# SparklingH/BloomScene

Hardware: AMD Instinct MI355X
Metric: Msplats/s fwd+bwd @1M Gaussians 1920x1080 SH3; fraction of HBM roofline (higher is better)
Workload: dtype f32; 1 GPU; c3: 1000000 Gaussians, SH deg 3, 1920x1080, fwd+bwd colour+depth targets, synthetic scene A seed 0; gaussians=1000000, width=1920, height=1080, sh_degree=3, num_rendered=4386625, visible=1000000, parallelism=view-parallel x1, exact_exp=0, strict_gradients=0, prewarm_steps=282

## Files before the change

### bloomscene_amd/_capi.py

```python
from __future__ import annotations

import ctypes as C
import os
import subprocess

_HERE = os.path.dirname(os.path.abspath(__file__))
LIB_PATH = os.path.join(_HERE, "libbloomscene_rast.so")
CSRC = os.path.join(_HERE, "csrc")

ALLOC_FN = C.CFUNCTYPE(C.c_void_p, C.c_void_p, C.c_size_t)

_F = C.c_void_p
ABI_VERSION = 4
OLDER_ABI_ACCEPTED = frozenset({2, 3})


class StageProfile(C.Structure):
    _fields_ = [("name", C.c_char_p), ("total_ms", C.c_double), ("launches", C.c_int)]


SIGNATURES = {
    "bsr_version": (C.c_int, []),
    "bsr_last_error": (C.c_char_p, []),
    "bsr_mark_visible": (C.c_int, [C.c_int, _F, _F, _F, _F, C.c_void_p]),
    "bsr_forward": (C.c_int, [ALLOC_FN, C.c_void_p, ALLOC_FN, C.c_void_p, ALLOC_FN, C.c_void_p,
                              C.c_int, C.c_int, C.c_int, _F, C.c_int, C.c_int, _F, _F, _F, _F, _F, C.c_float, _F, _F,
                              _F, _F, _F, C.c_float, C.c_float, C.c_int, _F, _F, _F, C.c_int, C.c_void_p,
                              C.POINTER(C.c_int)]),
    "bsr_forward_ex": (C.c_int, [ALLOC_FN, C.c_void_p, ALLOC_FN, C.c_void_p, ALLOC_FN, C.c_void_p,
                                 C.c_int, C.c_int, C.c_int, _F, C.c_int, C.c_int, _F, _F, _F, _F, _F, C.c_float, _F, _F,
                                 _F, _F, _F, C.c_float, C.c_float, C.c_int, _F, _F, _F, C.c_int, C.c_void_p,
                                 C.POINTER(C.c_int)] + [C.c_uint]),
    "bsr_forward_views": (C.c_int, [ALLOC_FN, C.c_void_p, ALLOC_FN, C.c_void_p, ALLOC_FN, C.c_void_p,
                                    C.c_int, C.c_int, C.c_int, C.c_int, _F, C.c_int, C.c_int, _F, _F, _F, _F, _F,
                                    C.c_float, _F, _F, _F, _F, _F, C.c_float, C.c_float, C.c_int, _F, _F, _F, C.c_int,
                                    C.c_void_p, C.POINTER(C.c_int), C.c_uint]),
    "bsr_visible_filter": (C.c_int, [C.c_int, C.c_int, C.c_int, C.c_int, _F, _F, C.c_float, _F, _F, _F, _F,
                                     C.c_float, C.c_float, C.c_int, _F, C.c_int, C.c_void_p]),
    "bsr_visible_scratch_bytes": (C.c_size_t, [C.c_int]),
    "bsr_visible_filter_indices": (C.c_int, [C.c_int, C.c_int, C.c_int, C.c_int, _F, _F, C.c_float, _F, _F, _F, _F,
                                             C.c_float, C.c_float, C.c_int, _F, _F, _F, C.POINTER(C.c_int), C.c_int,
                                             C.c_void_p]),
    "bsr_visible_filter_views": (C.c_int, [C.c_int, C.c_int, C.c_int, C.c_int, _F, _F, C.c_float, _F, _F, _F, _F,
                                           C.c_float, C.c_float, _F, C.c_int, C.c_void_p]),
    "bsr_visible_groups_scratch_bytes": (C.c_size_t, [C.c_int, C.c_int]),
    "bsr_visible_filter_groups": (C.c_int, [C.c_int, C.c_int, C.c_int, C.c_int, C.c_int, _F, _F, C.c_float, _F, _F, _F, _F,
                                            C.c_float, C.c_float, _F, _F, _F, _F, C.c_int, C.c_void_p]),
    "bsr_pack_rows": (C.c_int, [C.c_int, C.c_int, C.c_int, C.POINTER(C.c_void_p), C.POINTER(C.c_int), _F, C.c_int, _F, C.c_int,
                                C.c_void_p]),
    "bsr_gather_rows": (C.c_int, [C.c_int, C.c_int, C.c_int, C.POINTER(C.c_void_p), C.POINTER(C.c_int), _F, C.c_int,
                                  C.POINTER(C.c_void_p), C.c_int, C.c_void_p]),
    "bsr_backward": (C.c_int, [C.c_int, C.c_int, C.c_int, C.c_int, _F, C.c_int, C.c_int, _F, _F, _F, _F, C.c_float,
                               _F, _F, _F, _F, _F, C.c_float, C.c_float, _F, _F, _F, _F, _F, _F, _F, _F, _F, _F, _F,
                               _F, _F, _F, _F, C.c_int, C.c_void_p]),
    "bsr_backward_depth": (C.c_int, [C.c_int, C.c_int, C.c_int, C.c_int, _F, C.c_int, C.c_int, _F, _F, _F, _F, C.c_float,
                                     _F, _F, _F, _F, _F, C.c_float, C.c_float, _F, _F, _F, _F, _F, _F, _F, _F, _F, _F,
                                     _F, _F, _F, _F, _F, _F, C.c_int, C.c_void_p]),
    "bsr_backward_ex": (C.c_int, [C.c_int, C.c_int, C.c_int, C.c_int, _F, C.c_int, C.c_int, _F, _F, _F, _F, C.c_float,
                                  _F, _F, _F, _F, _F, C.c_float, C.c_float, _F, _F, _F, _F, _F, _F, _F, _F, _F, _F,
                                  _F, _F, _F, _F, _F, _F, C.c_int, C.c_void_p, C.c_uint]),
    "bsr_read_counts": (C.c_int, [_F, C.c_int, C.c_int, C.c_void_p, C.POINTER(C.c_int), C.POINTER(C.c_int)]),
    "bsr_check_deferred": (C.c_int, []),
    "bsr_geometry_bytes": (C.c_size_t, [C.c_int]),
    "bsr_binning_bytes": (C.c_size_t, [C.c_int]),
    "bsr_image_bytes": (C.c_size_t, [C.c_int, C.c_int]),
    "bsr_transmittance_offset": (C.c_size_t, [C.c_void_p]),
    "bsr_profile_enable": (C.c_int, [C.c_int]),
    "bsr_profile_only": (C.c_int, [C.c_char_p]),
    "bsr_profile_reset": (C.c_int, []),
    "bsr_profile_read": (C.c_int, [C.POINTER(StageProfile), C.c_int]),
    "bsr_anchor_scratch_bytes": (C.c_size_t, [C.c_int, C.c_int]),
    "bsr_anchor_select": (C.c_int, [C.c_int, C.c_int, _F, _F, _F, C.POINTER(C.c_int), C.c_void_p]),
    "bsr_anchor_expand": (C.c_int, [C.c_int, C.c_int, C.c_int] + [_F] * 12 + [C.c_void_p]),
    "bsr_anchor_expand_backward": (C.c_int, [C.c_int, C.c_int, C.c_int] + [_F] * 16 + [C.c_void_p]),
    "bsr_anchor_gaussian_bytes": (C.c_size_t, [C.c_int]),
    "bsr_anchor_gradient_bytes": (C.c_size_t, [C.c_int]),
    "bsr_anchor_render_forward": (C.c_int, [C.c_int, C.c_int] + [_F] * 8 + [ALLOC_FN, C.c_void_p] * 4
                                  + [_F, C.c_int, C.c_int, C.c_float, _F, _F, _F, C.c_float, C.c_float, _F, _F, C.c_int,
                                     C.c_void_p, C.POINTER(C.c_int), C.POINTER(C.c_int), C.c_uint]),
    "bsr_anchor_render_backward": (C.c_int, [C.c_int, C.c_int, C.c_int, C.c_int] + [_F] * 6 + [_F, _F, _F]
                                   + [_F, C.c_int, C.c_int, C.c_float, _F, _F, _F, C.c_float, C.c_float]
                                   + [_F] * 3 + [_F] * 5 + [_F] + [_F] * 6 + [C.c_int, C.c_void_p, C.c_uint]),
    "bsr_grid_backward_scratch_bytes": (C.c_size_t, [C.c_int, C.c_int, C.c_int]),
    "bsr_grid_encode_forward": (C.c_int, [C.c_int] * 5 + [_F] * 6 + [C.c_void_p]),
    "bsr_grid_encode_backward": (C.c_int, [C.c_int] * 5 + [_F] * 7 + [C.c_void_p, C.c_void_p]),
    "bsr_knn_scratch_bytes": (C.c_size_t, [C.c_int]),
    "bsr_knn_mean_dist": (C.c_int, [C.c_int, _F, _F, C.c_void_p, C.c_void_p]),
    "bsr_scatter_max": (C.c_int, [C.c_int] * 4 + [_F, _F, _F, C.c_longlong, C.c_longlong, _F, _F, C.c_void_p]),
    "bsr_voxel_isin_scratch_bytes": (C.c_size_t, [C.c_int]),
    "bsr_voxel_isin": (C.c_int, [C.c_int, C.c_int, _F, _F, _F, C.c_void_p, C.c_void_p]),
    "bsr_entropy_scratch_bytes": (C.c_size_t, [C.c_int] * 3),
    "bsr_entropy_forward": (C.c_int, [C.c_int] * 3 + [_F, C.c_longlong] * 3 + [_F, C.c_int, _F, _F, _F] + [_F] * 4
                            + [C.c_void_p, C.c_void_p]),
    "bsr_entropy_backward": (C.c_int, [C.c_int] * 3 + [_F, C.c_longlong] * 3 + [_F, C.c_int, _F, _F, _F] + [_F, C.c_int]
                             + [_F] * 5 + [C.c_void_p, C.c_void_p]),
    "bsr_photometric_scratch_bytes": (C.c_size_t, [C.c_int] * 4),
    "bsr_photometric_forward": (C.c_int, [C.c_int] * 4 + [_F, _F, C.c_float, _F, _F, _F, C.c_void_p, C.c_void_p]),
    "bsr_photometric_backward": (C.c_int, [C.c_int] * 4 + [_F, _F, _F, C.c_float, _F, _F, C.c_void_p]),
    "bsr_depth_prior_scratch_bytes": (C.c_size_t, [C.c_int] * 2),
    "bsr_depth_prior_forward": (C.c_int, [C.c_int] * 2 + [_F] * 3 + [C.c_longlong] * 3 + [C.c_int] + [C.c_float] * 3 + [C.c_int]
                                + [_F] * 4 + [C.c_void_p]),
    "bsr_depth_prior_backward": (C.c_int, [C.c_int] * 2 + [_F] * 3 + [C.c_longlong] * 3 + [C.c_int] + [C.c_float] * 3 + [C.c_int]
                                 + [_F] * 4 + [C.c_void_p]),
    "bsr_anchor_heads_scratch_bytes": (C.c_size_t, [C.c_int] * 3),
    "bsr_anchor_heads_forward": (C.c_int, [C.c_int] * 3 + [_F, C.c_longlong, _F, _F, _F, C.c_void_p] + [_F] * 4 + [C.c_void_p]),
    "bsr_anchor_heads_backward": (C.c_int, [C.c_int] * 3 + [_F, C.c_longlong, _F, _F, _F, C.c_void_p] + [_F] * 7
                                  + [C.c_void_p, C.c_void_p, C.c_void_p]),
    "bsr_context_scratch_bytes": (C.c_size_t, [C.c_int] * 5),
    "bsr_context_head_forward": (C.c_int, [C.c_int] * 5 + [_F, C.c_longlong, C.c_void_p] + [C.c_float] * 3 + [_F, C.c_longlong] * 3
                                 + [_F] * 3 + [_F] * 2 + [_F] * 3 + [_F, C.c_void_p]),
    "bsr_context_head_backward": (C.c_int, [C.c_int] * 5 + [_F, C.c_longlong, C.c_void_p] + [C.c_float] * 3 + [_F] * 3 + [_F] * 5
                                  + [_F, C.c_void_p, C.c_void_p, C.c_void_p]),
    "bsr_context_quantise_forward": (C.c_int, [C.c_int] * 5 + [_F, C.c_longlong, C.c_void_p] + [C.c_float] * 3
                                     + [_F, C.c_longlong] * 3 + [_F] * 3 + [_F] + [_F] * 3 + [C.c_void_p]),
    "bsr_anchor_visible_forward": (C.c_int, [C.c_int] * 4 + [_F] * 5 + [C.c_longlong] + [_F] * 3 + [_F] * 7 + [C.c_void_p]),
    "bsr_anchor_visible_backward": (C.c_int, [C.c_int] * 4 + [_F] * 3 + [_F] * 5 + [_F] * 5 + [C.c_void_p]),
    "bsr_anchor_accumulate_scratch_bytes": (C.c_size_t, [C.c_int] * 2),
    "bsr_anchor_accumulate": (C.c_int, [C.c_int] * 4 + [_F] * 4 + [C.c_int] + [_F] * 5 + [C.c_void_p, C.c_void_p]),
    "bsr_codec_stream_bound": (C.c_size_t, [C.c_longlong, C.c_int]),
    "bsr_codec_scratch_bytes": (C.c_size_t, [C.c_longlong, C.c_int]),
    "bsr_codec_encode_gaussian": (C.c_int, [C.c_int] * 3 + [_F, C.c_longlong] * 3 + [_F, C.c_int, _F, C.c_float, C.c_int]
                                  + [_F, C.c_size_t, _F, C.c_void_p, C.c_void_p]),
    "bsr_codec_decode_gaussian": (C.c_int, [C.c_int] * 3 + [_F, C.c_size_t] + [_F, C.c_longlong] * 2
                                  + [_F, C.c_int, _F, C.c_float, _F, _F, C.c_void_p]),
    "bsr_codec_encode_table": (C.c_int, [C.c_int] * 2 + [_F, _F, C.c_longlong, C.c_int, _F, C.c_size_t, _F, C.c_void_p,
                                                         C.c_void_p]),
    "bsr_codec_decode_table": (C.c_int, [C.c_int] * 2 + [_F, C.c_size_t, _F, C.c_longlong, _F, _F, C.c_void_p]),
}

HeadsPointers = C.c_void_p * 12
ContextPointers = C.c_void_p * 4

_lib = None
_allow_older_abi = False


def build(force: bool = False) -> str:
    cmd = ["make", "-C", CSRC, "-j8"] + (["-B"] if force else [])
    subprocess.check_call(cmd, stdout=subprocess.DEVNULL)
    return LIB_PATH


def lib():
    global _lib
    if _lib is None:
        if not os.path.exists(LIB_PATH):
            raise RuntimeError(
                f"{LIB_PATH} not found: build it with `make -C {CSRC}` (or __graft_entry__.build()). "
                "bloomscene_amd has no CPU fallback.")
        handle = C.CDLL(LIB_PATH)
        handle.bsr_version.restype = C.c_int
        older = handle.bsr_version() in OLDER_ABI_ACCEPTED and _allow_older_abi
        if handle.bsr_version() != ABI_VERSION and not older:
            raise RuntimeError(f"{LIB_PATH} is ABI version {handle.bsr_version()}, this binding needs {ABI_VERSION}: "
                               f"rebuild it (make -C {CSRC})")
        for name, (res, args) in SIGNATURES.items():
            if older and not hasattr(handle, name):
                continue
            fn = getattr(handle, name)
            fn.restype = res
            fn.argtypes = args
        _lib = handle
    return _lib


def use_library(path: str, allow_older_abi: bool = False):
    global LIB_PATH, _allow_older_abi
    if _lib is not None:
        raise RuntimeError("use_library() must be called before the library is first used")
    LIB_PATH = os.path.abspath(path)
    _allow_older_abi = bool(allow_older_abi)


def last_error() -> str:
    return lib().bsr_last_error().decode("utf-8", "replace")


def check(rc: int, what: str):
    if rc != 0:
        raise RuntimeError(f"{what} failed: {last_error()}")


def profile_enable(on):
    lib().bsr_profile_enable(int(on))


def profile_only(stage=None):
    lib().bsr_profile_only(stage.encode() if stage else None)


def profile_reset():
    lib().bsr_profile_reset()


def profile_read():
    arr = (StageProfile * 16)()
    n = lib().bsr_profile_read(arr, 16)
    return {arr[i].name.decode(): (arr[i].total_ms, arr[i].launches) for i in range(n)}
```

### bloomscene_amd/csrc/api.hip

```cpp
#include "../../include/bloomscene_rast.h"
#include "common.h"
#include "errors.h"
#include "host_state.h"
#include "launch.h"
#include "profiler.h"
#include "scratch.h"

#include <cstring>

using namespace bsr;

static constexpr unsigned BSR_KNOWN_FLAGS = BSR_FLAG_EXACT_EXP | BSR_FLAG_EXACT_GRAD | BSR_FLAG_NO_READBACK | BSR_FLAG_TEST_MASK;

static bool is_capturing(hipStream_t s)
{
	hipStreamCaptureStatus cs = hipStreamCaptureStatusNone;
	if (hipStreamIsCapturing(s, &cs) != hipSuccess) { (void)hipGetLastError(); cs = hipStreamCaptureStatusNone; }
	return cs != hipStreamCaptureStatusNone;
}

static int check_common(int P, int width, int height, const float* means3D, const float* scales, const float* rotations,
                        const float* cov3D_precomp, const float* viewmatrix, const float* projmatrix)
{
	if (P < 0 || width <= 0 || height <= 0) return fail("invalid sizes: P=%d width=%d height=%d", P, width, height);
	if ((width + BSR_TILE - 1) / BSR_TILE > 65535 || (height + BSR_TILE - 1) / BSR_TILE > 65535)
		return fail("image too large for 16-bit tile coordinates");
	if (P > 0 && !means3D) return fail("means3D is null");
	if (!viewmatrix || !projmatrix) return fail("viewmatrix/projmatrix is null");
	const bool has_sr = scales != nullptr && rotations != nullptr;
	const bool has_any_sr = scales != nullptr || rotations != nullptr;
	if (P > 0 && ((!has_sr && !cov3D_precomp) || (has_any_sr && cov3D_precomp)))
		return fail("Please provide exactly one of either scale/rotation pair or precomputed 3D covariance!");
	return 0;
}

static int check_forward_args(bsr_alloc_fn geometryBuffer, bsr_alloc_fn binningBuffer, bsr_alloc_fn imageBuffer, int P,
                              int D, int M, const float* background, int width, int height, const float* means3D,
                              const float* shs, const float* colors_precomp, const float* opacities, const float* scales,
                              const float* rotations, const float* cov3D_precomp, const float* viewmatrix,
                              const float* projmatrix, const float* cam_pos, const float* out_color,
                              const float* out_depth)
{
	if (check_common(P, width, height, means3D, scales, rotations, cov3D_precomp, viewmatrix, projmatrix)) return 1;
	if (!geometryBuffer || !binningBuffer || !imageBuffer) return fail("scratch allocation callback is null");
	if (!out_color || !out_depth || !background) return fail("out_color/out_depth/background is null");
	if (!opacities) return fail("opacities is null");
	if ((shs == nullptr) == (colors_precomp == nullptr))
		return fail("Please provide excatly one of either SHs or precomputed colors!");
	if (shs && (!cam_pos || M <= 0)) return fail("SH colours need cam_pos and M > 0");
	if (shs && D >= 0 && (D + 1) * (D + 1) > M && D <= 3)
		return fail("sh_degree %d needs %d coefficients per Gaussian, shs holds %d", D, (D + 1) * (D + 1), M);
	return 0;
}

struct ForwardCall {
	hipStream_t s;
	unsigned flags;
	int debug;
	bool no_readback;
	int V, P, width, height, gx, gy, T, n_wg;
	size_t P_rows;
	GeomState geom;
	ImgState img;
	bsr_alloc_fn binningBuffer;
	void* binning_user;
	const float* background;
	float *out_color, *out_depth;
	size_t cap;
};

static int run_tail(ForwardCall& c, size_t capacity, bool rerun, long long kept_hint)
{
	hipStream_t s = c.s;
	const unsigned flags = c.flags;
	const int V = c.V, T = c.T, debug = c.debug;
	const GeomState& geom = c.geom;
	const ImgState& img = c.img;
	char* bin_p = c.binningBuffer(c.binning_user, BinState::bytes(capacity, V == 1));
	if (!bin_p) return fail("scratch allocation callback returned null");
	const BinState bin = BinState::carve(bin_p, capacity, V == 1);
	c.cap = capacity;
	if (rerun) {
		HIP_TRY(hipMemsetAsync(img.flags + 1, 0, sizeof(int), s));
		HIP_TRY(hipMemsetAsync(img.flags + 4, 0, 2 * sizeof(int), s));
	}
	const int* n_ptr = img.flags + 2;
	const BinPlan plan = binning_plan((int)c.P_rows, T, (int)capacity, kept_hint);
	BinElem* elems_sorted = nullptr;
	BinElem* elems_free = nullptr;
	{
		StageTimer t("binning", s);
		launch_binning(plan, (int)c.P_rows, T, c.gx, n_ptr, (int)capacity, geom, bin.elems_a, bin.elems_b, bin.hist, BSR_HIST_BLOCKS_MAX,
		               img.tile_range, img.big_tiles, img.flags, &elems_sorted, &elems_free, s);
	}
	STAGE_CHECK("binning", debug, s);
	{
		StageTimer t("sort_tiles", s);
		const uint32_t* digit_total1 = geom.hist1 + BSR_RADIX_BINS_ * hist1_columns((size_t)c.n_wg);
		launch_sort_tiles(plan, T, (int)capacity, n_ptr, (int)capacity, img.tile_range, img.big_tiles, img.flags,
		                  digit_total1, elems_sorted, elems_free, bin.point_list,
		                  ((flags & BSR_FLAG_TEST_SORT_INT) ? 1 : 0) | ((flags & BSR_FLAG_TEST_SORT_NETWORK) ? 2 : 0),
		                  (flags & BSR_FLAG_TEST_SMALL_GRIDS) != 0, s);
	}
	STAGE_CHECK("sort_tiles", debug, s);
	{
		StageTimer t("render_fwd", s);
		int* const masks_flag = (V == 1 && c.P <= (1 << 24) && !(flags & BSR_FLAG_TEST_NO_HALF_MASKS)) ? img.flags + 6 : nullptr;
		launch_render_fwd(c.gx, c.gy, V, c.width, c.height, n_ptr, (int)capacity, img.tile_range, bin.point_list, masks_flag, geom.rec,
		                  c.background, V > 1 ? nullptr : img.final_T, V > 1 ? nullptr : img.n_contrib, c.out_color, c.out_depth,
		                  (flags & BSR_FLAG_EXACT_EXP) != 0, c.no_readback, img.flags + BSR_POOL_FWD, s);
	}
	return 0;
}

static int forward_impl(int V, bsr_alloc_fn geometryBuffer, void* geometry_user, bsr_alloc_fn binningBuffer,
                        void* binning_user, bsr_alloc_fn imageBuffer, void* image_user, int P, int D, int M,
                        const float* background, int width,
                int height, const float* means3D, const float* shs, const float* colors_precomp,
                const float* opacities, const float* scales, float scale_modifier, const float* rotations,
                const float* cov3D_precomp, const float* viewmatrix, const float* projmatrix, const float* cam_pos,
                float tan_fovx, float tan_fovy, int prefiltered, float* out_color, float* out_depth, int* radii,
                int debug, void* stream, int* num_rendered, unsigned flags)
{
	g_err[0] = 0;
	hipStream_t s = (hipStream_t)stream;
	if (flags & ~BSR_KNOWN_FLAGS) {
		if (num_rendered) *num_rendered = 0;
		return fail("forward: unknown flag bits 0x%x", flags & ~BSR_KNOWN_FLAGS);
	}
	const bool no_readback = (flags & BSR_FLAG_NO_READBACK) != 0;
	const long long given_capacity = (no_readback && num_rendered) ? (long long)*num_rendered : 0;
	if (num_rendered) *num_rendered = 0;
	if (no_readback) {
		if (V != 1) return fail("BSR_FLAG_NO_READBACK is for single-view calls");
		if (prefiltered) return fail("BSR_FLAG_NO_READBACK cannot be combined with prefiltered (its violation flag is part of the read-back)");
		if (!num_rendered || given_capacity <= 0)
			return fail("BSR_FLAG_NO_READBACK: *num_rendered must hold the capacity (tile instances, > 0) on entry");
	}
	{
		SyncCache* sc0 = sync_cache();
		if (!sc0) return 1;
		if (sc0->pending && is_capturing(s))
			return fail("forward during stream capture while the overflow check of this thread's previous BSR_FLAG_NO_READBACK "
			            "forward is pending: call bsr_check_deferred() before hipStreamBeginCapture");
		if (check_deferred(sc0)) return 1;
	}
	if (no_readback) *num_rendered = (int)given_capacity;
	if (P == 0) {
		if (width <= 0 || height <= 0 || !out_color || !out_depth) return fail("invalid image outputs");
		HIP_TRY(hipMemsetAsync(out_color, 0, (size_t)V * 3 * width * height * sizeof(float), s));
		HIP_TRY(hipMemsetAsync(out_depth, 0, (size_t)V * width * height * sizeof(float), s));
		return 0;
	}
	if (check_forward_args(geometryBuffer, binningBuffer, imageBuffer, P, D, M, background, width, height, means3D, shs,
	                       colors_precomp, opacities, scales, rotations, cov3D_precomp, viewmatrix, projmatrix, cam_pos,
	                       out_color, out_depth))
		return 1;
	const int gx = (width + BSR_TILE - 1) / BSR_TILE, gy = (height + BSR_TILE - 1) / BSR_TILE;
	if ((long long)V * gy > 65535 || (long long)V * gx * gy > 0x3fffffff) return fail("too many views for one call");
	const int T = gx * gy * V;
	const size_t N = (size_t)width * height * (size_t)V;
	const int n_wg = ((P + 255) / 256) * V;
	const size_t P_rows = V == 1 ? (size_t)P : (size_t)n_wg * 256;
	if (P_rows > 0x7fffffffu) return fail("too many (view, Gaussian) pairs for one call");

	char* geom_p = geometryBuffer(geometry_user, GeomState::bytes(P_rows));
	char* img_p = imageBuffer(image_user, ImgState::bytes(N, (size_t)T));
	if (!geom_p || !img_p) return fail("scratch allocation callback returned null");
	ForwardCall c = {s, flags, debug, no_readback, V, P, width, height, gx, gy, T, n_wg, P_rows,
	                 GeomState::carve(geom_p, P_rows), ImgState::carve(img_p, N, (size_t)T),
	                 binningBuffer, binning_user, background, out_color, out_depth, 0};
	const GeomState& geom = c.geom;
	const ImgState& img = c.img;

	if (prefiltered) HIP_TRY(hipMemsetAsync(img.flags, 0, sizeof(int), s));

	{
		PreArgs a;
		memset(&a, 0, sizeof(a));
		a.P = P; a.D = D; a.M = M;
		a.means3D = means3D; a.scales = scales; a.scale_modifier = scale_modifier; a.rotations = rotations;
		a.opacities = opacities; a.shs = shs; a.cov3D_precomp = cov3D_precomp; a.colors_precomp = colors_precomp;
		a.viewmatrix = viewmatrix; a.projmatrix = projmatrix; a.cam_pos = cam_pos;
		a.W = width; a.H = height; a.tan_fovx = tan_fovx; a.tan_fovy = tan_fovy;
		a.focal_y = height / (2.0f * tan_fovy);
		a.focal_x = width / (2.0f * tan_fovx);
		a.gx = gx; a.gy = gy; a.prefiltered = prefiltered; a.radii = radii; a.geom = geom;
		a.flags = img.flags;
		a.n_views = V;
		if (V > 1)
			HIP_TRY(hipMemsetAsync(geom.hist1, 0, BSR_RADIX_BINS_ * hist1_columns((size_t)n_wg) * sizeof(uint32_t), s));
		{
			StageTimer t("preprocess", s);
			launch_preprocess(a, false, s);
		}
		STAGE_CHECK("preprocess", debug, s);
	}
	SyncCache* sc = sync_cache();
	if (!sc) return 1;
	const bool capturing = no_readback && is_capturing(s);
	{
		StageTimer t("scan_wg", s);
		launch_scans(n_wg, geom.wg_kept, geom.wg_area, img.flags, geom.hist1, capturing ? nullptr : sc->pinned_dev, s);
	}
	STAGE_CHECK("scan_wg", debug, s);

	const CallShape shape{P, width, height, V};
	if (no_readback) {
		if (!capturing) {
			HIP_TRY(hipEventRecord(sc->deferred, s));
			sc->pending = true;
			sc->pending_capacity = (size_t)given_capacity;
			sc->pending_shape = shape;
		}
		if (run_tail(c, (size_t)given_capacity, false, sc->nr_shape == shape ? (long long)sc->nr_kept : 0)) return 1;
		STAGE_CHECK("render_fwd", debug, s);
		return 0;
	}
	const bool guess = sc->can_guess(shape);
	HIP_TRY(hipEventRecord(sc->copied, s));
	if (guess && run_tail(c, sc->guessed_capacity(), false, (long long)sc->last_kept)) return 1;
	HIP_TRY(hipEventSynchronize(sc->copied));
	const int h_flag = prefiltered ? sc->pinned[0] : 0;
	const uint32_t h_kept = (uint32_t)sc->pinned[2], h_R = (uint32_t)sc->pinned[3];
	if (h_flag) return fail("Point is filtered although prefiltered is set. This shouldn't happen!");
	if (h_R > 0x7fffffffu) return fail("too many tile instances (%u)", h_R);
	const int R = (int)h_R;
	if (num_rendered) *num_rendered = R;
	sc->remember(shape, h_R, h_kept);
	if (!guess || (size_t)h_kept > c.cap || (V == 1 && !backward_fits(c.cap, (size_t)R, (size_t)h_kept))) {
		if (run_tail(c, (size_t)R, guess, (long long)h_kept)) return 1;
	}
	STAGE_CHECK("render_fwd", debug, s);
	return 0;
}

extern "C" {

int bsr_version(void) { return BSR_VERSION; }

size_t bsr_geometry_bytes(int P) { return GeomState::bytes((size_t)(P > 0 ? P : 0)); }
size_t bsr_binning_bytes(int R) { return BinState::bytes((size_t)(R > 0 ? R : 0), true); }
size_t bsr_transmittance_offset(const void* image_buffer)
{
	return (size_t)((const char*)ImgState::carve((char*)image_buffer, 0, 0).final_T - (const char*)image_buffer);
}
size_t bsr_image_bytes(int W, int H)
{
	const size_t gx = (W + BSR_TILE - 1) / BSR_TILE, gy = (H + BSR_TILE - 1) / BSR_TILE;
	return ImgState::bytes((size_t)W * H, gx * gy);
}

int bsr_read_counts(const char* image_buffer, int width, int height, void* stream, int* kept, int* num_rendered)
{
	g_err[0] = 0;
	if (!image_buffer || width <= 0 || height <= 0) return fail("bsr_read_counts: invalid image buffer / size");
	const size_t gx = (width + BSR_TILE - 1) / BSR_TILE, gy = (height + BSR_TILE - 1) / BSR_TILE;
	ImgState img = ImgState::carve(const_cast<char*>(image_buffer), (size_t)width * height, gx * gy);
	uint32_t k = 0, r = 0;
	if (read_u32_blocking((const uint32_t*)(img.flags + 2), &k, (hipStream_t)stream)) return 1;
	if (read_u32_blocking((const uint32_t*)(img.flags + 3), &r, (hipStream_t)stream)) return 1;
	if (kept) *kept = (int)k;
	if (num_rendered) *num_rendered = (int)r;
	return 0;
}

int bsr_mark_visible(int P, const float* means3D, const float* viewmatrix, const float* projmatrix, uint8_t* present,
                     void* stream)
{
	(void)projmatrix;
	g_err[0] = 0;
	hipStream_t s = (hipStream_t)stream;
	if (P <= 0) return 0;
	if (!means3D || !viewmatrix || !present) return fail("bsr_mark_visible: null pointer");
	{
		StageTimer t("mark_visible", s);
		launch_mark_visible(P, means3D, viewmatrix, present, s);
	}
	STAGE_CHECK("mark_visible", 0, s);
	return 0;
}

int bsr_visible_filter(int P, int M, int width, int height, const float* means3D, const float* scales,
                       float scale_modifier, const float* rotations, const float* cov3D_precomp,
                       const float* viewmatrix, const float* projmatrix, float tan_fovx, float tan_fovy,
                       int prefiltered, int* radii, int debug, void* stream)
{
	(void)M;
	g_err[0] = 0;
	hipStream_t s = (hipStream_t)stream;
	if (check_common(P, width, height, means3D, scales, rotations, cov3D_precomp, viewmatrix, projmatrix)) return 1;
	if (P == 0) return 0;
	if (!radii) return fail("radii is null");
	int* d_flag = nullptr;
	SyncCache* sc = nullptr;
	if (prefiltered) {
		sc = sync_cache();
		if (!sc) return 1;
		sc->pinned[5] = 0;
		d_flag = sc->pinned_dev + 5;
	}
	PreArgs a;
	memset(&a, 0, sizeof(a));
	a.P = P; a.D = 0; a.M = 0;
	a.means3D = means3D; a.scales = scales; a.scale_modifier = scale_modifier; a.rotations = rotations;
	a.cov3D_precomp = cov3D_precomp; a.viewmatrix = viewmatrix; a.projmatrix = projmatrix;
	a.W = width; a.H = height; a.tan_fovx = tan_fovx; a.tan_fovy = tan_fovy;
	a.focal_y = height / (2.0f * tan_fovy);
	a.focal_x = width / (2.0f * tan_fovx);
	a.gx = (width + BSR_TILE - 1) / BSR_TILE; a.gy = (height + BSR_TILE - 1) / BSR_TILE;
	a.prefiltered = prefiltered; a.radii = radii; a.flags = d_flag;
	{
		StageTimer t("visible_filter", s);
		launch_preprocess(a, true, s);
	}
	STAGE_CHECK("visible_filter", debug, s);
	if (prefiltered) {
		HIP_TRY(hipStreamSynchronize(s));
		if (sc->pinned[5]) return fail("Point is filtered although prefiltered is set. This shouldn't happen!");
	}
	return 0;
}

int bsr_visible_filter_views(int P, int n_views, int width, int height, const float* means3D, const float* scales,
                             float scale_modifier, const float* rotations, const float* cov3D_precomp,
                             const float* viewmatrices, const float* projmatrices, float tan_fovx, float tan_fovy,
                             int* radii, int debug, void* stream)
{
	g_err[0] = 0;
	hipStream_t s = (hipStream_t)stream;
	if (n_views < 0) return fail("n_views must be >= 0");
	if (check_common(P, width, height, means3D, scales, rotations, cov3D_precomp, viewmatrices, projmatrices)) return 1;
	if (P == 0 || n_views == 0) return 0;
	if (!radii) return fail("radii is null");
	{
		StageTimer t("visible_filter_views", s);
		launch_visible_filter_views(P, n_views, means3D, scales, scale_modifier, rotations, cov3D_precomp, viewmatrices,
		                            projmatrices, width, height, tan_fovx, tan_fovy, radii, nullptr, 0, nullptr,
		                            nullptr, nullptr, s);
	}
	STAGE_CHECK("visible_filter_views", debug, s);
	return 0;
}

size_t bsr_visible_groups_scratch_bytes(int P, int n_groups)
{
	if (P <= 0 || n_groups <= 0) return 0;
	return sizeof(uint32_t) * (size_t)n_groups * (((size_t)P + 255) / 256);
}

int bsr_visible_filter_groups(int P, int n_views, int n_groups, int width, int height, const float* means3D,
                              const float* scales, float scale_modifier, const float* rotations,
                              const float* cov3D_precomp, const float* viewmatrices, const float* projmatrices,
                              float tan_fovx, float tan_fovy, const int* group_of_view, uint8_t* group_mask,
                              uint32_t* group_counts, void* count_scratch, int debug, void* stream)
{
// ... 16 lines not shown
		                            group_mask, wg_counts, group_counts, s);
	}
	STAGE_CHECK("visible_filter_groups", debug, s);
	return 0;
}

static int gather_impl(const char* who, int R, int P, int n_src, const float* const* src, const int* widths,
                       const int64_t* idx, int idx_stride, float* dst_packed, float* const* dst_each, int debug,
                       void* stream)
{
	g_err[0] = 0;
	hipStream_t s = (hipStream_t)stream;
	if (R < 0 || P < 0 || n_src < 1 || n_src > BSR_PACK_MAX_SRC) return fail("%s: need R >= 0, P >= 0 and 1 <= n_src <= 8", who);
	if (!src || !widths) return fail("%s: NULL table", who);
	int row = 0;
	for (int k = 0; k < n_src; k++) {
		if (widths[k] < 1 || !src[k]) return fail("%s: every source needs a pointer and a width >= 1", who);
		row += widths[k];
	}
	if (row > 4096) return fail("%s: more than 4096 floats per row", who);
	if (R == 0) return 0;
	if (!idx || idx_stride < 1 || (!dst_packed && !dst_each)) return fail("%s: NULL buffer", who);
	if (!dst_packed)
		for (int k = 0; k < n_src; k++)
			if (!dst_each[k]) return fail("%s: NULL destination", who);
	{
		StageTimer t(who, s);
		launch_pack_rows(R, P, n_src, src, widths, idx, idx_stride, dst_packed, dst_each, s);
	}
	STAGE_CHECK(who, debug, s);
	return 0;
}

int bsr_pack_rows(int R, int P, int n_src, const float* const* src, const int* widths, const int64_t* idx, int idx_stride,
                  float* dst, int debug, void* stream)
{
	return gather_impl("pack_rows", R, P, n_src, src, widths, idx, idx_stride, dst, nullptr, debug, stream);
}

int bsr_gather_rows(int R, int P, int n_src, const float* const* src, const int* widths, const int64_t* idx,
                    int idx_stride, float* const* dst, int debug, void* stream)
{
	return gather_impl("gather_rows", R, P, n_src, src, widths, idx, idx_stride, nullptr, dst, debug, stream);
}

int bsr_forward(bsr_alloc_fn geometryBuffer, void* geometry_user, bsr_alloc_fn binningBuffer, void* binning_user,
                bsr_alloc_fn imageBuffer, void* image_user, int P, int D, int M, const float* background, int width,
                int height, const float* means3D, const float* shs, const float* colors_precomp,
                const float* opacities, const float* scales, float scale_modifier, const float* rotations,
                const float* cov3D_precomp, const float* viewmatrix, const float* projmatrix, const float* cam_pos,
                float tan_fovx, float tan_fovy, int prefiltered, float* out_color, float* out_depth, int* radii,
                int debug, void* stream, int* num_rendered)
{
	return bsr_forward_ex(geometryBuffer, geometry_user, binningBuffer, binning_user, imageBuffer, image_user, P, D, M,
	                      background, width, height, means3D, shs, colors_precomp, opacities, scales, scale_modifier,
	                      rotations, cov3D_precomp, viewmatrix, projmatrix, cam_pos, tan_fovx, tan_fovy, prefiltered,
	                      out_color, out_depth, radii, debug, stream, num_rendered, 0u);
}

int bsr_forward_ex(bsr_alloc_fn geometryBuffer, void* geometry_user, bsr_alloc_fn binningBuffer, void* binning_user,
                   bsr_alloc_fn imageBuffer, void* image_user, int P, int D, int M, const float* background, int width,
                   int height, const float* means3D, const float* shs, const float* colors_precomp,
                   const float* opacities, const float* scales, float scale_modifier, const float* rotations,
                   const float* cov3D_precomp, const float* viewmatrix, const float* projmatrix, const float* cam_pos,
                   float tan_fovx, float tan_fovy, int prefiltered, float* out_color, float* out_depth, int* radii,
                   int debug, void* stream, int* num_rendered, unsigned flags)
{
	return forward_impl(1, geometryBuffer, geometry_user, binningBuffer, binning_user, imageBuffer, image_user, P, D, M,
	                    background, width, height, means3D, shs, colors_precomp, opacities, scales, scale_modifier,
	                    rotations, cov3D_precomp, viewmatrix, projmatrix, cam_pos, tan_fovx, tan_fovy, prefiltered,
	                    out_color, out_depth, radii, debug, stream, num_rendered, flags);
}

int bsr_forward_views(bsr_alloc_fn geometryBuffer, void* geometry_user, bsr_alloc_fn binningBuffer, void* binning_user,
                      bsr_alloc_fn imageBuffer, void* image_user, int P, int D, int M, int n_views,
                      const float* background, int width, int height, const float* means3D, const float* shs,
                      const float* colors_precomp, const float* opacities, const float* scales, float scale_modifier,
                      const float* rotations, const float* cov3D_precomp, const float* viewmatrices,
                      const float* projmatrices, const float* cam_positions, float tan_fovx, float tan_fovy,
                      int prefiltered, float* out_color, float* out_depth, int* radii, int debug, void* stream,
                      int* num_rendered, unsigned flags)
{
	g_err[0] = 0;
	if (num_rendered) *num_rendered = 0;
	if (n_views < 0) return fail("n_views must be >= 0");
	if (n_views == 0) return 0;
	return forward_impl(n_views, geometryBuffer, geometry_user, binningBuffer, binning_user, imageBuffer, image_user, P, D,
	                    M, background, width, height, means3D, shs, colors_precomp, opacities, scales, scale_modifier,
	                    rotations, cov3D_precomp, viewmatrices, projmatrices, cam_positions, tan_fovx, tan_fovy,
	                    prefiltered, out_color, out_depth, radii, debug, stream, num_rendered, flags);
}

int bsr_backward_ex(int P, int D, int M, int R, const float* background, int width, int height,
                    const float* means3D, const float* shs, const float* colors_precomp, const float* scales,
                    float scale_modifier, const float* rotations, const float* cov3D_precomp,
                    const float* viewmatrix, const float* projmatrix, const float* campos, float tan_fovx,
                    float tan_fovy, const int* radii, char* geom_buffer, char* binning_buffer, char* image_buffer,
                    const float* out_depth, const float* dL_dpix, const float* dL_depths, float* dL_dmean2D,
                    float* dL_dconic, float* dL_dopacity, float* dL_dcolor, float* dL_dmean3D, float* dL_dcov3D,
                    float* dL_dsh, float* dL_dscale, float* dL_drot, int debug, void* stream, unsigned flags)
{
	g_err[0] = 0;
	(void)colors_precomp;
	if (P > 0 && out_depth && !dL_depths)
		return fail("bsr_backward_ex: out_depth selects the depth-gradient extension, which needs dL_depths");
	hipStream_t s = (hipStream_t)stream;
	if (flags & ~BSR_KNOWN_FLAGS) return fail("backward: unknown flag bits 0x%x", flags & ~BSR_KNOWN_FLAGS);
	if (P == 0) return 0;
	if (check_common(P, width, height, means3D, scales, rotations, cov3D_precomp, viewmatrix, projmatrix)) return 1;
	if (!geom_buffer || !image_buffer || (R > 0 && !binning_buffer)) return fail("scratch buffer is null");
	if (!dL_dpix || !background) return fail("dL_dpix/background is null");
	if (!dL_dmean2D || !dL_dopacity || !dL_dmean3D) return fail("gradient output is null");
	if (!shs && !dL_dcolor) return fail("dL_dcolor is null but colors_precomp is the colour input");
	if (!scales && !dL_dcov3D) return fail("dL_dcov3D is null but cov3D_precomp is the covariance input");
	if (shs && (M <= 0 || !dL_dsh || !campos)) return fail("SH backward needs M > 0, dL_dsh and campos");
	if (shs && (D < 0 || (D + 1) * (D + 1) > M))
		return fail("sh_degree %d needs %d coefficients per Gaussian, shs holds %d", D, (D + 1) * (D + 1), M);
	if (scales && (!dL_dscale || !dL_drot)) return fail("dL_dscale/dL_drot is null");

	const int gx = (width + BSR_TILE - 1) / BSR_TILE, gy = (height + BSR_TILE - 1) / BSR_TILE;
	const int T = gx * gy;
	const size_t N = (size_t)width * height;
	GeomState geom = GeomState::carve(geom_buffer, (size_t)P);
	ImgState img = ImgState::carve(image_buffer, N, (size_t)T);
	BinState bin = BinState::carve(binning_buffer, (size_t)(R > 0 ? R : 0), true);

	float4* slab = bin.slab;

	if (R > 0) {
		{
			StageTimer t("render_bwd", s);
			RenderBwdArgs w;
			w.gx = gx; w.gy = gy; w.W = width; w.H = height;
			w.tile_range = img.tile_range; w.point_list = bin.point_list; w.rec = geom.rec; w.wg_base = geom.wg_kept;
			w.bg = background; w.final_T = img.final_T; w.n_contrib = img.n_contrib; w.dL_dpix = dL_dpix;
			w.out_depth = out_depth; w.dL_depths = out_depth ? dL_depths : nullptr;
			w.masks_flag = img.flags + 6; w.slab = slab;
			w.strict = (flags & BSR_FLAG_EXACT_GRAD) != 0; w.capacity = R;
			launch_render_bwd(w, s);
		}
		STAGE_CHECK("render_bwd", debug, s);
	}
	BwdArgs a;
	memset(&a, 0, sizeof(a));
	a.P = P; a.D = D; a.M = M;
	a.means3D = means3D; a.radii = radii; a.shs = shs; a.scales = scales; a.rotations = rotations;
	a.scale_modifier = scale_modifier; a.cov3D_precomp = cov3D_precomp; a.viewmatrix = viewmatrix;
	a.projmatrix = projmatrix; a.campos = campos; a.tan_fovx = tan_fovx; a.tan_fovy = tan_fovy;
	a.focal_y = height / (2.0f * tan_fovy);
	a.focal_x = width / (2.0f * tan_fovx);
	a.geom = geom;
	a.slab = slab; a.depth_grad = out_depth != nullptr;
	a.kept_ptr = img.flags + 2; a.capacity = R;
	a.dL_dmean2D = dL_dmean2D; a.dL_dconic = dL_dconic; a.dL_dopacity = dL_dopacity; a.dL_dcolor = dL_dcolor;
	a.dL_dmean3D = dL_dmean3D; a.dL_dcov3D = dL_dcov3D; a.dL_dsh = dL_dsh; a.dL_dscale = dL_dscale; a.dL_drot = dL_drot;
	{
		StageTimer t("preprocess_bwd", s);
		launch_preprocess_bwd(a, s);
	}
	STAGE_CHECK("preprocess_bwd", debug, s);
	return 0;
}

int bsr_backward(int P, int D, int M, int R, const float* background, int width, int height, const float* means3D,
                 const float* shs, const float* colors_precomp, const float* scales, float scale_modifier,
                 const float* rotations, const float* cov3D_precomp, const float* viewmatrix, const float* projmatrix,
                 const float* campos, float tan_fovx, float tan_fovy, const int* radii, char* geom_buffer,
                 char* binning_buffer, char* image_buffer, const float* dL_dpix, const float* dL_depths,
                 float* dL_dmean2D, float* dL_dconic, float* dL_dopacity, float* dL_dcolor, float* dL_dmean3D,
                 float* dL_dcov3D, float* dL_dsh, float* dL_dscale, float* dL_drot, int debug, void* stream)
{
	(void)dL_depths;
	return bsr_backward_ex(P, D, M, R, background, width, height, means3D, shs, colors_precomp, scales, scale_modifier,
	                       rotations, cov3D_precomp, viewmatrix, projmatrix, campos, tan_fovx, tan_fovy, radii, geom_buffer,
	                       binning_buffer, image_buffer, nullptr, dL_dpix, nullptr, dL_dmean2D, dL_dconic, dL_dopacity,
	                       dL_dcolor, dL_dmean3D, dL_dcov3D, dL_dsh, dL_dscale, dL_drot, debug, stream, 0u);
}

int bsr_backward_depth(int P, int D, int M, int R, const float* background, int width, int height,
                       const float* means3D, const float* shs, const float* colors_precomp, const float* scales,
                       float scale_modifier, const float* rotations, const float* cov3D_precomp,
                       const float* viewmatrix, const float* projmatrix, const float* campos, float tan_fovx,
                       float tan_fovy, const int* radii, char* geom_buffer, char* binning_buffer, char* image_buffer,
                       const float* out_depth, const float* dL_dpix, const float* dL_depths, float* dL_dmean2D,
                       float* dL_dconic, float* dL_dopacity, float* dL_dcolor, float* dL_dmean3D, float* dL_dcov3D,
                       float* dL_dsh, float* dL_dscale, float* dL_drot, int debug, void* stream)
{
	if (P > 0 && (!out_depth || !dL_depths)) return fail("bsr_backward_depth needs out_depth and dL_depths");
	return bsr_backward_ex(P, D, M, R, background, width, height, means3D, shs, colors_precomp, scales, scale_modifier,
	                       rotations, cov3D_precomp, viewmatrix, projmatrix, campos, tan_fovx, tan_fovy, radii, geom_buffer,
	                       binning_buffer, image_buffer, out_depth, dL_dpix, dL_depths, dL_dmean2D, dL_dconic, dL_dopacity,
	                       dL_dcolor, dL_dmean3D, dL_dcov3D, dL_dsh, dL_dscale, dL_drot, debug, stream, 0u);
}

}
```

### bloomscene_amd/csrc/binning.hip

```cpp
#include "tile_sort.h"
#include "launch.h"

namespace bsr {

struct AllValid { __device__ __forceinline__ bool operator()(int) const { return true; } };
template <typename Valid = AllValid>
__device__ __forceinline__ uint32_t block_exclusive_scan(int n, uint32_t* data, uint32_t* s_wave, bool write, Valid valid = Valid())
{
	const int tid = threadIdx.x, lane = tid & 63, wave = tid >> 6;
	uint32_t carry = 0u;
	uint32_t nx[4];
#pragma unroll
	for (int k = 0; k < 4; k++) nx[k] = (tid * 4 + k < n && valid(tid * 4 + k)) ? data[tid * 4 + k] : 0u;
	int set = 0;
	for (int base = 0; base < n; base += 4096, set ^= 16) {
		const int i = base + tid * 4;
		uint32_t v[4];
#pragma unroll
		for (int k = 0; k < 4; k++) v[k] = nx[k];
#pragma unroll
		for (int k = 0; k < 4; k++) nx[k] = (i + 4096 + k < n && valid(i + 4096 + k)) ? data[i + 4096 + k] : 0u;
		const uint32_t mine = v[0] + v[1] + v[2] + v[3];
		const uint32_t incl = wave_inclusive_sum_dpp(mine);
		if (lane == 63) s_wave[set + wave] = incl;
		__syncthreads();
		uint32_t wave_off = 0u, total = 0u;
#pragma unroll
		for (int w = 0; w < 16; w++) {
			const uint32_t t = s_wave[set + w];
			wave_off += w < wave ? t : 0u;
			total += t;
		}
		uint32_t run = carry + wave_off + incl - mine;
		if (write) {
#pragma unroll
			for (int k = 0; k < 4; k++) {
				if (i + k < n) data[i + k] = run;
				run += v[k];
			}
		}
		carry += total;
	}
	__syncthreads();
	return carry;
}

struct Hist1ColumnValid {
	int per, n_wg;
	__device__ __forceinline__ bool operator()(int col) const { return hist1_wg_of_column(col, per) < n_wg; }
};
__global__ void __launch_bounds__(1024) k_scans(int n_wg, uint32_t* __restrict__ wg_kept,
                                                uint32_t* __restrict__ wg_area, int* __restrict__ flags,
                                                uint32_t* __restrict__ hist1, int* __restrict__ host_counts)
{
	__shared__ uint32_t s_w[32];
	if (blockIdx.x == BSR_RADIX_BINS) {
		const uint32_t kept = block_exclusive_scan(n_wg, wg_kept, s_w, true);
		const uint32_t area = block_exclusive_scan(n_wg, wg_area, s_w, false);
		if (threadIdx.x == 0) {
			flags[2] = (int)kept;
			flags[3] = (int)area;
			flags[1] = flags[4] = flags[5] = 0;
			flags[6] = flags[7] = 0;
			flags[BSR_POOL_FWD] = flags[BSR_POOL_BWD] = 0;
			if (host_counts != nullptr) {
				host_counts[0] = flags[0];
				host_counts[1] = 0;
				host_counts[2] = (int)kept;
				host_counts[3] = (int)area;
				__threadfence_system();
			}
		}
		return;
	}
	const int per = (n_wg + 7) >> 3, n_col = 8 * per;
	const uint32_t total = block_exclusive_scan(n_col, hist1 + (size_t)blockIdx.x * n_col, s_w, true,
	                                            Hist1ColumnValid{per, n_wg});
	if (threadIdx.x == 0) hist1[(size_t)BSR_RADIX_BINS * n_col + blockIdx.x] = total;
}

struct RadixPartition { int n, chunk, n_blocks; };
__device__ __forceinline__ RadixPartition radix_partition(const int* __restrict__ n_ptr, int capacity,
                                                          int hist_blocks_max)
{
	RadixPartition p;
	p.n = *n_ptr;
	if (p.n > capacity || p.n < 0) p.n = -1;
	int chunk = ((max(p.n, 0) + hist_blocks_max - 1) / hist_blocks_max + 255) / 256 * 256;
	p.chunk = chunk < 1024 ? 1024 : chunk;
	p.n_blocks = (max(p.n, 0) + p.chunk - 1) / p.chunk;
	return p;
}

__global__ void __launch_bounds__(256) k_radix_rowscan(const int* __restrict__ n_ptr, int capacity, int hist_blocks_max,
                                                       uint32_t* __restrict__ hist,
                                                       uint32_t* __restrict__ digit_total)
{
	__shared__ uint32_t s_wave[4];
	__shared__ uint32_t s_carry;
	const RadixPartition part = radix_partition(n_ptr, capacity, hist_blocks_max);
	if (part.n <= 0) return;
	const int n_blocks = part.n_blocks;
	const int tid = threadIdx.x, lane = tid & 63, wave = tid >> 6;
	uint32_t* row = hist + (size_t)blockIdx.x * n_blocks;
	if (tid == 0) s_carry = 0;
	__syncthreads();
	for (int base = 0; base < n_blocks; base += 256) {
		const int i = base + tid;
		const uint32_t v = (i < n_blocks) ? row[i] : 0u;
		uint32_t incl = v;
#pragma unroll
		for (int d = 1; d < 64; d <<= 1) {
			const uint32_t t = __shfl_up(incl, d, 64);
			if (lane >= d) incl += t;
		}
		if (lane == 63) s_wave[wave] = incl;
		__syncthreads();
		const uint32_t w0 = s_wave[0], w1 = s_wave[1], w2 = s_wave[2], w3 = s_wave[3];
		const uint32_t carry = s_carry;
		if (i < n_blocks) row[i] = carry + (wave > 0 ? w0 : 0u) + (wave > 1 ? w1 : 0u) + (wave > 2 ? w2 : 0u) + incl - v;
		__syncthreads();
		if (tid == 0) s_carry = carry + w0 + w1 + w2 + w3;
		__syncthreads();
	}
	if (tid == 0) digit_total[blockIdx.x] = s_carry;
}

__global__ void __launch_bounds__(256) k_emit_scatter(int P, int gx, const int* __restrict__ n_ptr, int capacity,
                                                      const ushort4* __restrict__ rect,
                                                      const uint64_t* __restrict__ kept_mask,
                                                      const float* __restrict__ depth,
                                                      const uint32_t* __restrict__ hist1,
                                                      uint32_t* __restrict__ digit_base, BinElem* __restrict__ elems,
                                                      uint32_t* __restrict__ zero_me, int n_zero, int compact)
{
	__shared__ uint32_t s_off[BSR_RADIX_BINS];
	__shared__ uint32_t s_scan[4];
	{
		const int n = *n_ptr;
		if (n <= 0 || n > capacity) return;
	}
	const int tid = threadIdx.x, lane = tid & 63, wave = tid >> 6;
	const int n_wg = (int)gridDim.x, per = (n_wg + 7) >> 3, n_col = 8 * per;
	const int idx = blockIdx.x * 256 + tid;
	for (int i = idx; i < n_zero; i += n_wg * 256) zero_me[i] = 0u;
	const bool in_range = idx < P;
	const int ld = in_range ? idx : 0;
	const uint32_t v = hist1[(size_t)BSR_RADIX_BINS * n_col + tid];
	const uint32_t col = hist1[(size_t)tid * n_col + hist1_column((int)blockIdx.x, per)];
	const ushort4 r = rect[ld];
	const uint64_t mask = kept_mask[ld];
	const uint32_t depth_bits = __float_as_uint(depth[ld]);
	{
		const uint32_t incl = wave_inclusive_sum_dpp(v);
		if (lane == 63) s_scan[wave] = incl;
		__syncthreads();
		const uint32_t base = (wave > 0 ? s_scan[0] : 0u) + (wave > 1 ? s_scan[1] : 0u) + (wave > 2 ? s_scan[2] : 0u) + incl - v;
		s_off[tid] = base + col;
		if (blockIdx.x == 0) digit_base[tid] = base;
	}
	__syncthreads();
	if (!in_range) return;
	if (r.z <= r.x || r.w <= r.y) return;
	const uint32_t area = (uint32_t)(r.z - r.x) * (uint32_t)(r.w - r.y);
	if (kept_count(area, mask) == 0) return;
	uint32_t k = 0;
	for (int y = r.y; y < r.w; y++)
		for (int x = r.x; x < r.z; x++, k++) {
			if (!tile_kept(area, mask, k)) continue;
			const uint32_t tile = (uint32_t)(y * gx + x);
			const uint32_t pos = atomicAdd(&s_off[tile & (BSR_RADIX_BINS - 1)], 1u);
			store_elem_m(elems, pos, BinElem{tile, (uint32_t)idx, depth_bits}, compact);
		}
}

__global__ void __launch_bounds__(256) k_radix_hist(const int* __restrict__ n_ptr, int capacity, int hist_blocks_max,
                                                    int shift, const BinElem* __restrict__ elems,
                                                    uint32_t* __restrict__ hist)
{
	__shared__ uint32_t s_hist[BSR_RADIX_BINS];
	const RadixPartition part = radix_partition(n_ptr, capacity, hist_blocks_max);
	if ((int)blockIdx.x >= part.n_blocks) return;
	const int n = part.n, chunk = part.chunk, n_blocks = part.n_blocks;
	const int tid = threadIdx.x;
	s_hist[tid] = 0;
	__syncthreads();
	const int beg = blockIdx.x * chunk, end = min(n, beg + chunk);
	for (int i = beg + tid; i < end; i += 1024) {
		uint32_t t[4];
#pragma unroll
		for (int k = 0; k < 4; k++) t[k] = (i + 256 * k < end) ? elems[i + 256 * k].x : 0u;
#pragma unroll
		for (int k = 0; k < 4; k++)
			if (i + 256 * k < end) atomicAdd(&s_hist[(t[k] >> shift) & (BSR_RADIX_BINS - 1)], 1u);
	}
	__syncthreads();
	hist[(size_t)tid * n_blocks + blockIdx.x] = s_hist[tid];
}

__global__ void __launch_bounds__(256) k_radix_scatter(const int* __restrict__ n_ptr, int capacity,
                                                       int hist_blocks_max, int shift,
                                                       const BinElem* __restrict__ elems_in,
                                                       BinElem* __restrict__ elems_out,
                                                       const uint32_t* __restrict__ hist,
                                                       const uint32_t* __restrict__ digit_total)
{
	__shared__ uint32_t s_off[BSR_RADIX_BINS];
	__shared__ uint32_t s_wcnt[4][BSR_RADIX_BINS];
	__shared__ uint32_t s_scan[4];
	const RadixPartition part = radix_partition(n_ptr, capacity, hist_blocks_max);
	if ((int)blockIdx.x >= part.n_blocks) return;
	const int n = part.n, chunk = part.chunk, n_blocks = part.n_blocks;
	const int tid = threadIdx.x, lane = tid & 63, wave = tid >> 6;
	const int beg = blockIdx.x * chunk, end = min(n, beg + chunk);
	const uint32_t row_prefix = hist[(size_t)tid * n_blocks + blockIdx.x];
	BinElem e_next = BinElem{0u, 0u, 0u};
// ... 156 lines not shown
			const uint32_t first = s_tot[j * 16 + wave] + c[j];
			tile_range[(j << 10) + tid] = make_uint2(first, first + tile_count[(j << 10) + tid]);
		}
	if (__syncthreads_or(any_big)) {
		__shared__ int s_cls[3];
		if (tid < 3) s_cls[tid] = 0;
		__syncthreads();
		for (int j = 0; j < chunks; j++) {
			const int t = (j << 10) + tid;
			const uint32_t cc = t < T ? tile_count[t] : 0u;
			const int cls = cc > 8192u ? 2 : (cc > 4096u ? 1 : (cc > (uint32_t)BSR_SORT_SMALL_N ? 0 : -1));
#pragma unroll
			for (int c3 = 0; c3 < 3; c3++) {
				const uint64_t b = wave_ballot(cls == c3);
				if (b == 0ull) continue;
				int base = 0;
				if (lane == 0) base = atomicAdd(&s_cls[c3], __popcll(b));
				base = __shfl(base, 0);
				if (cls == c3) big_tiles[(size_t)c3 * T + base + __popcll(b & ((1ull << lane) - 1ull))] = (uint32_t)t;
			}
		}
		__syncthreads();
		if (tid < 3) flags[tid == 0 ? 1 : 3 + tid] = s_cls[tid];
	}
}

#define BSR_SLICE_REGS 16
__global__ void __launch_bounds__(256) k_tile_scatter(int T, int n_slices, const int* __restrict__ n_ptr, int capacity,
                                                      const uint32_t* __restrict__ digit_total1,
                                                      const BinElem* __restrict__ elems_in,
                                                      BinElem* __restrict__ elems_out,
                                                      const uint2* __restrict__ tile_range,
                                                      uint32_t* __restrict__ tile_cursor, int compact)
{
	__shared__ uint32_t s_hist[BSR_RADIX_BINS];
	__shared__ uint32_t s_off[BSR_RADIX_BINS];
	__shared__ uint32_t s_scan[4];
	__shared__ uint32_t s_base[2];
	{
		const int n = *n_ptr;
		if (n <= 0 || n > capacity) return;
	}
	const int tid = threadIdx.x;
	const int d1 = (int)blockIdx.x / n_slices, s = (int)blockIdx.x % n_slices;
	s_hist[tid] = 0;
	const BucketSlice sl = bucket_slice(digit_total1[tid], d1, s, n_slices, s_scan, s_base);
	if (sl.beg >= sl.end) return;
	const bool in_regs = sl.end - sl.beg <= 256 * BSR_SLICE_REGS;
	BinElem e[BSR_SLICE_REGS];
	if (in_regs) {
#pragma unroll
		for (int k = 0; k < BSR_SLICE_REGS; k++) {
			const int i = sl.beg + tid + 256 * k;
			e[k] = i < sl.end ? load_elem_m(elems_in, (size_t)i, compact) : BinElem{0u, 0u, 0u};
		}
#pragma unroll
		for (int k = 0; k < BSR_SLICE_REGS; k++)
			if (sl.beg + tid + 256 * k < sl.end) atomicAdd(&s_hist[(e[k].x >> BSR_RADIX_BITS) & (BSR_RADIX_BINS - 1)], 1u);
	} else {
		slice_histogram(elems_in, sl, s_hist, compact);
	}
	__syncthreads();
	{
		const uint32_t c = s_hist[tid];
		const uint32_t t = ((uint32_t)tid << BSR_RADIX_BITS) | (uint32_t)d1;
		uint32_t off = 0;
		if (c != 0u && t < (uint32_t)T) off = tile_range[t].x + atomicAdd(&tile_cursor[t], c);
		s_off[tid] = off;
	}
	__syncthreads();
	if (in_regs) {
#pragma unroll
		for (int k = 0; k < BSR_SLICE_REGS; k++)
			if (sl.beg + tid + 256 * k < sl.end) {
				const uint32_t pos = atomicAdd(&s_off[(e[k].x >> BSR_RADIX_BITS) & (BSR_RADIX_BINS - 1)], 1u);
				store_elem_m(elems_out, pos, e[k], compact);
			}
		return;
	}
	for (int i = sl.beg + tid; i < sl.end; i += 1024) {
		BinElem f[4];
#pragma unroll
		for (int k = 0; k < 4; k++)
			if (i + 256 * k < sl.end) f[k] = load_elem_m(elems_in, (size_t)(i + 256 * k), compact);
#pragma unroll
		for (int k = 0; k < 4; k++)
			if (i + 256 * k < sl.end) {
				const uint32_t pos = atomicAdd(&s_off[(f[k].x >> BSR_RADIX_BITS) & (BSR_RADIX_BINS - 1)], 1u);
				store_elem_m(elems_out, pos, f[k], compact);
			}
	}
}

__device__ __forceinline__ int first_not_below_row16(const BinElem* __restrict__ elems_sorted, int n, uint32_t t,
                                                     int lane)
{
	const int j = lane & 15, sh = lane & 48;
	int lo = 0, hi = n;
	while (hi > lo) {
		const int width = hi - lo;
		if (width <= 16) {
			const bool below = j < width && elems_sorted[lo + j].x < t;
			lo += __popc((uint32_t)(wave_ballot(below) >> sh) & 0xffffu);
			break;
		}
		const int p = lo + (int)(((uint64_t)width * (uint32_t)(j + 1)) / 17u);
		const bool below = elems_sorted[p].x < t;
		const int c = __popc((uint32_t)(wave_ballot(below) >> sh) & 0xffffu);
		const int new_lo = c > 0 ? lo + (int)(((uint64_t)width * (uint32_t)c) / 17u) + 1 : lo;
		const int new_hi = c < 16 ? lo + (int)(((uint64_t)width * (uint32_t)(c + 1)) / 17u) : hi;
		lo = new_lo;
		hi = new_hi;
	}
	return lo;
}

__global__ void __launch_bounds__(256) k_tile_ranges(int T, const int* __restrict__ n_ptr, int capacity,
                                                     const BinElem* __restrict__ elems_sorted,
                                                     uint2* __restrict__ tile_range,
                                                     uint32_t* __restrict__ big_tiles, int* __restrict__ flags)
{
	int n = *n_ptr;
	if (n > capacity) return;
	if (n < 0) n = 0;
	const int lane = threadIdx.x & 63, row = lane >> 4;
	const int wave = (int)blockIdx.x * 4 + ((int)threadIdx.x >> 6);
	const int t = wave * 3 + row;
	bool big = false;
	int cnt_t = 0;
	{
		const int lo = (t <= T) ? first_not_below_row16(elems_sorted, n, (uint32_t)t, lane) : n;
		const int hi = __shfl_down(lo, 16, 64);
		const bool owner = row < 3 && (lane & 15) == 0;
		if (owner && t < T) {
			tile_range[t] = make_uint2((uint32_t)lo, (uint32_t)hi);
			cnt_t = hi - lo;
			big = cnt_t > BSR_SORT_SMALL;
		}
	}
	int cls = -1;
	if (big) cls = cnt_t > 8192 ? 2 : (cnt_t > 4096 ? 1 : 0);
#pragma unroll
	for (int k = 0; k < 3; k++) {
		const uint64_t b = __ballot(cls == k);
		if (b == 0) continue;
		int base = 0;
		if (lane == 0) base = atomicAdd(&flags[k == 0 ? 1 : 3 + k], __popcll(b));
		base = __shfl(base, 0);
		if (cls == k) big_tiles[(size_t)k * T + base + __popcll(b & ((1ull << lane) - 1ull))] = (uint32_t)t;
	}
}

void launch_scans(int n_wg, uint32_t* wg_kept, uint32_t* wg_area, int* flags, uint32_t* hist1, int* host_counts,
                  hipStream_t s)
{
	hipLaunchKernelGGL(k_scans, dim3(BSR_RADIX_BINS + 1), dim3(1024), 0, s, n_wg, wg_kept, wg_area, flags, hist1,
	                   host_counts);
}

#ifndef BSR_BUCKET_MAX_PER_TILE
#define BSR_BUCKET_MAX_PER_TILE 850
#endif
#ifndef BSR_BKT_SMALL_PER_TILE
#define BSR_BKT_SMALL_PER_TILE 400
#endif
#ifndef BSR_BKT_BIG_PER_TILE
#define BSR_BKT_BIG_PER_TILE 1400
#endif
BinPlan binning_plan(int P, int T, int capacity, long long kept_hint)
{
	int bits = 0;
	while ((1 << bits) < T) bits++;
	const bool tile_owned = bits <= 2 * BSR_RADIX_BITS && 2 * (size_t)T <= (size_t)BSR_RADIX_BINS * BSR_HIST_BLOCKS_MAX;
	const int compact = (tile_owned && P <= (1 << 24)) ? 1 : 0;
	if (!tile_owned) return BinPlan{BinPlan::RADIX, 0, compact};
	const long long kept = kept_hint > 0 ? kept_hint : (long long)capacity * 7 / 10;
	if (P <= (1 << 24) && T <= 8192 && kept <= (long long)BSR_BUCKET_MAX_PER_TILE * T)
		return kept <= (long long)BSR_BKT_SMALL_PER_TILE * T ? BinPlan{BinPlan::BUCKET, 512, compact}
		                                                     : BinPlan{BinPlan::BUCKET, 1024, compact};
	if (P <= (1 << 24) && T <= 8192 && BSR_BUCKET_MAX_PER_TILE > 0 && kept <= (long long)BSR_BKT_BIG_PER_TILE * T)
		return BinPlan{BinPlan::BUCKET, 2048, compact};
	return BinPlan{BinPlan::CHAIN, 0, compact};
}

void launch_binning(const BinPlan& plan, int P, int T, int gx, const int* n_ptr, int capacity, const GeomState& geom,
                    BinElem* elems_a, BinElem* elems_b, uint32_t* hist, int hist_blocks_max, uint2* tile_range,
                    uint32_t* big_tiles, int* flags, BinElem** elems_sorted, BinElem** elems_free, hipStream_t s)
{
	const int compact = plan.compact;
	const int n_wg = (P + 255) / 256, n_col = 8 * ((n_wg + 7) >> 3);
	uint32_t* const digit_total1 = geom.hist1 + (size_t)BSR_RADIX_BINS * n_col;
	uint32_t* tile_count = hist;
	uint32_t* tile_cursor = hist + T;
	hipLaunchKernelGGL(k_emit_scatter, dim3((P + 255) / 256), dim3(256), 0, s, P, gx, n_ptr, capacity, geom.rect,
	                   geom.kept_mask, geom.depth, geom.hist1, digit_total1 + BSR_RADIX_BINS, elems_a, tile_count,
	                   plan.form == BinPlan::CHAIN ? 2 * T : 0, compact);
	switch (plan.form) {
	case BinPlan::BUCKET:
		*elems_sorted = elems_a;
		*elems_free = elems_b;
		return;
	case BinPlan::CHAIN: {
		int n_slices = capacity / (BSR_RADIX_BINS * 3072) + 1;
		n_slices = n_slices > 256 ? 256 : n_slices;
		hipLaunchKernelGGL(k_tile_count, dim3(BSR_RADIX_BINS * n_slices), dim3(256), 0, s, T, n_slices, n_ptr, capacity,
		                   digit_total1, elems_a, tile_count, compact);
		if (T <= 8192)
			hipLaunchKernelGGL(k_tile_starts<8>, dim3(1), dim3(1024), 0, s, T, n_ptr, capacity, tile_count, tile_range,
			                   big_tiles, flags);
		else
			hipLaunchKernelGGL(k_tile_starts<64>, dim3(1), dim3(1024), 0, s, T, n_ptr, capacity, tile_count, tile_range,
			                   big_tiles, flags);
		hipLaunchKernelGGL(k_tile_scatter, dim3(BSR_RADIX_BINS * n_slices), dim3(256), 0, s, T, n_slices, n_ptr, capacity,
		                   digit_total1, elems_a, elems_b, tile_range, tile_cursor, compact);
		*elems_sorted = elems_b;
		*elems_free = elems_a;
		return;
	}
	case BinPlan::RADIX:
		break;
	}
	int bits = 0;
	while ((1 << bits) < T) bits++;
	int max_blocks = (capacity + 1023) / 1024;
	if (max_blocks > hist_blocks_max) max_blocks = hist_blocks_max;
	if (max_blocks < 1) max_blocks = 1;
	uint32_t* digit_total = hist + (size_t)BSR_RADIX_BINS * hist_blocks_max;
	BinElem* ei = elems_a; BinElem* eo = elems_b;
	for (int shift = BSR_RADIX_BITS; shift < bits; shift += BSR_RADIX_BITS) {
		hipLaunchKernelGGL(k_radix_hist, dim3(max_blocks), dim3(256), 0, s, n_ptr, capacity, hist_blocks_max, shift, ei,
		                   hist);
		hipLaunchKernelGGL(k_radix_rowscan, dim3(BSR_RADIX_BINS), dim3(256), 0, s, n_ptr, capacity, hist_blocks_max, hist,
		                   digit_total);
		hipLaunchKernelGGL(k_radix_scatter, dim3(max_blocks), dim3(256), 0, s, n_ptr, capacity, hist_blocks_max, shift, ei,
		                   eo, hist, digit_total);
		BinElem* tt = ei; ei = eo; eo = tt;
	}
	hipLaunchKernelGGL(k_tile_ranges, dim3((T / 3 + 1 + 3) / 4), dim3(256), 0, s, T, n_ptr, capacity, ei, tile_range,
	                   big_tiles, flags);
	*elems_sorted = ei;
	*elems_free = eo;
}

}
```

### bloomscene_amd/csrc/common.h

```cpp
#pragma once
#include <hip/hip_runtime.h>
#include <stdint.h>

#define BSR_TILE 16
#define BSR_BLOCK 256
#define BSR_NEAR 0.2f
#define BSR_PACK_MAX_SRC 8

namespace bsr {

struct Carver;
#define BSR_REC 4
struct GeomState {
	float4* rec;
	uint32_t* inst_offset;
	uint32_t* wg_kept;
	uint32_t* wg_area;
	uint32_t* hist1;
	uint64_t* kept_mask;
	ushort4* rect;
	uint8_t* clamped;
	float* depth;
	static GeomState layout(Carver& c, size_t P);
	static size_t bytes(size_t P);
	static GeomState carve(char* p, size_t P);
};
struct BinElem {
	uint32_t x;
	uint32_t y;
	uint32_t z;
};
typedef float bsr_f32x4 __attribute__((ext_vector_type(4)));
typedef float bsr_f32x2 __attribute__((ext_vector_type(2)));
typedef bsr_f32x4 bsr_f32x4_a4 __attribute__((aligned(4)));
typedef bsr_f32x2 bsr_f32x2_a4 __attribute__((aligned(4)));
__host__ __device__ __forceinline__ constexpr int slab_row_floats(bool depth_grad) { return depth_grad ? 10 : 9; }
#define BSR_SLAB_ROW_BYTES 40
#define BSR_SLAB_TAIL_BYTES 16
typedef uint32_t bsr_u32x3 __attribute__((ext_vector_type(3)));
typedef bsr_u32x3 bsr_u32x3_a4 __attribute__((aligned(4)));
__device__ __forceinline__ BinElem load_elem(const BinElem* p)
{
	const bsr_u32x3 v = *reinterpret_cast<const bsr_u32x3_a4*>(p);
	return BinElem{v.x, v.y, v.z};
}
__device__ __forceinline__ void store_elem(BinElem* p, const BinElem e)
{
	*reinterpret_cast<bsr_u32x3_a4*>(p) = bsr_u32x3{e.x, e.y, e.z};
}
__device__ __forceinline__ BinElem load_elem_m(const BinElem* base, size_t i, int compact)
{
	if (compact) {
		const uint2 v = reinterpret_cast<const uint2*>(base)[i];
		return BinElem{(v.x >> 24) << 8, v.x & 0x00ffffffu, v.y};
	}
	return load_elem(base + i);
}
__device__ __forceinline__ void store_elem_m(BinElem* base, size_t i, const BinElem e, int compact)
{
	if (compact) reinterpret_cast<uint2*>(base)[i] = make_uint2(((e.x >> 8) << 24) | e.y, e.z);
	else store_elem(base + i, e);
}
__device__ __forceinline__ uint32_t elem_tile_m(const BinElem* base, size_t i, int compact)
{
	return compact ? (reinterpret_cast<const uint2*>(base)[i].x >> 24) << 8 : base[i].x;
}
__device__ __forceinline__ uint64_t elem_key_m(const BinElem* base, size_t i, int compact)
{
	if (compact) {
		const uint2 v = reinterpret_cast<const uint2*>(base)[i];
		return ((uint64_t)v.y << 32) | (uint64_t)(v.x & 0x00ffffffu);
	}
	const BinElem e = load_elem(base + i);
	return ((uint64_t)e.z << 32) | (uint64_t)e.y;
}
#define BSR_HIST_BLOCKS_MAX 2048
struct BinState {
	uint32_t* point_list;
	BinElem* elems_a;
	BinElem* elems_b;
	float4* slab;
	uint32_t* hist;
	static BinState layout(Carver& c, size_t R, bool with_slab);
	static size_t bytes(size_t R, bool with_slab);
	static BinState carve(char* p, size_t R, bool with_slab);
};
struct ImgState {
	float* final_T;
	uint32_t* n_contrib;
	uint2* tile_range;
	int* flags;
	uint32_t* big_tiles;
	static ImgState layout(Carver& c, size_t N, size_t T);
	static size_t bytes(size_t N, size_t T);
	static ImgState carve(char* p, size_t N, size_t T);
};

struct PreArgs {
	int P, D, M;
	const float* means3D;
	const float* scales;
	float scale_modifier;
	const float* rotations;
	const float* opacities;
	const float* shs;
	const float* cov3D_precomp;
	const float* colors_precomp;
	const float* viewmatrix;
	const float* projmatrix;
	const float* cam_pos;
	int W, H;
	float tan_fovx, tan_fovy, focal_x, focal_y;
	int gx, gy;
	int prefiltered;
	int* radii;
	int n_views;
	GeomState geom;
	int* flags;
};

struct BwdArgs {
	int P, D, M;
	const float* means3D;
	const int* radii;
	const float* shs;
	const float* scales;
	const float* rotations;
	float scale_modifier;
	const float* cov3D_precomp;
	const float* viewmatrix;
	const float* projmatrix;
	const float* campos;
	float tan_fovx, tan_fovy, focal_x, focal_y;
	GeomState geom;
	const float4* slab;
	int depth_grad;
	const int* kept_ptr;
	int capacity;
	float* dL_dmean2D;
	float* dL_dconic;
	float* dL_dopacity;
	float* dL_dcolor;
	float* dL_dmean3D;
	float* dL_dcov3D;
	float* dL_dsh;
	float* dL_dscale;
	float* dL_drot;
};

int fail(const char* fmt, ...);

int read_u32_blocking(const uint32_t* dev, uint32_t* out, hipStream_t s);

static inline size_t align_up(size_t x, size_t a) { return (x + a - 1) & ~(a - 1); }

__device__ __forceinline__ float bsr_expf(float x)
{
	if (x != x) return x;
	if (x < -104.0f) return 0.0f;
	if (x > 88.72284f) return __builtin_inff();
	const float k = __builtin_rintf(x * 1.44269504088896341f);
	float r = __builtin_fmaf(-k, 0.693359375f, x);
	r = __builtin_fmaf(-k, -2.12194440e-4f, r);
	float p = 1.0f / 5040.0f;
	p = __builtin_fmaf(p, r, 1.0f / 720.0f);
	p = __builtin_fmaf(p, r, 1.0f / 120.0f);
	p = __builtin_fmaf(p, r, 1.0f / 24.0f);
	p = __builtin_fmaf(p, r, 1.0f / 6.0f);
	p = __builtin_fmaf(p, r, 0.5f);
	p = __builtin_fmaf(p, r, 1.0f);
	p = __builtin_fmaf(p, r, 1.0f);
	return __builtin_ldexpf(p, (int)k);
}

__device__ __forceinline__ uint64_t wave_ballot(bool p) { return __builtin_amdgcn_ballot_w64(p); }

__device__ __forceinline__ uint32_t wave_inclusive_sum_dpp(uint32_t x)
{
	x += (uint32_t)__builtin_amdgcn_update_dpp(0, (int)x, 0x111, 0xf, 0xf, false);
	x += (uint32_t)__builtin_amdgcn_update_dpp(0, (int)x, 0x112, 0xf, 0xf, false);
	x += (uint32_t)__builtin_amdgcn_update_dpp(0, (int)x, 0x114, 0xf, 0xf, false);
	x += (uint32_t)__builtin_amdgcn_update_dpp(0, (int)x, 0x118, 0xf, 0xf, false);
	x += (uint32_t)__builtin_amdgcn_update_dpp(0, (int)x, 0x142, 0xa, 0xf, false);
	x += (uint32_t)__builtin_amdgcn_update_dpp(0, (int)x, 0x143, 0xc, 0xf, false);
	return x;
}

__device__ __forceinline__ float bsr_expf_walk(float x)
{
	const float k = __builtin_rintf(x * 1.44269504088896341f);
	float r = __builtin_fmaf(-k, 0.693359375f, x);
	r = __builtin_fmaf(-k, -2.12194440e-4f, r);
	float p = 1.0f / 5040.0f;
	p = __builtin_fmaf(p, r, 1.0f / 720.0f);
	p = __builtin_fmaf(p, r, 1.0f / 120.0f);
	p = __builtin_fmaf(p, r, 1.0f / 24.0f);
	p = __builtin_fmaf(p, r, 1.0f / 6.0f);
	p = __builtin_fmaf(p, r, 0.5f);
	p = __builtin_fmaf(p, r, 1.0f);
	p = __builtin_fmaf(p, r, 1.0f);
	return __builtin_ldexpf(p, (int)k);
}

__device__ __forceinline__ uint32_t kept_rank(uint32_t area, uint64_t mask, uint32_t k)
{
	return area > 64u ? k : (uint32_t)__popcll(mask & ((1ull << k) - 1ull));
}
__device__ __forceinline__ bool tile_kept(uint32_t area, uint64_t mask, uint32_t k)
{
	return area > 64u || ((mask >> k) & 1ull);
}
__device__ __forceinline__ uint32_t kept_count(uint32_t area, uint64_t mask)
{
	return area > 64u ? area : (uint32_t)__popcll(mask);
}

__host__ __device__ __forceinline__ float rank_sort_scale(float zmin, float zmax, int nb)
{
	const float s = zmax > zmin ? ((float)nb - 0.5f) / (zmax - zmin) : 0.0f;
	return s < 3.0e38f ? s : 0.0f;
}
__host__ __device__ __forceinline__ uint32_t rank_sort_bucket(float z, float zmin, float scale, int nb)
{
	const uint32_t b = (uint32_t)((z - zmin) * scale);
	return b < (uint32_t)nb ? b : (uint32_t)(nb - 1);
}

__device__ __forceinline__ int hist1_column(int wg, int per) { return (wg & 7) * per + (wg >> 3); }
__device__ __forceinline__ int hist1_wg_of_column(int c, int per) { return (c % per) * 8 + c / per; }

__device__ __forceinline__ void cov3d_from_scale_rot(const float* scale, float mod, const float4 q, float* cov3D)
{
	const float s0 = mod * scale[0], s1 = mod * scale[1], s2 = mod * scale[2];
	const float r = q.x, x = q.y, y = q.z, z = q.w;
	const float m00 = s0 * (1.f - 2.f * (y * y + z * z)), m01 = s1 * (2.f * (x * y - r * z)), m02 = s2 * (2.f * (x * z + r * y));
	const float m10 = s0 * (2.f * (x * y + r * z)), m11 = s1 * (1.f - 2.f * (x * x + z * z)), m12 = s2 * (2.f * (y * z - r * x));
	const float m20 = s0 * (2.f * (x * z - r * y)), m21 = s1 * (2.f * (y * z + r * x)), m22 = s2 * (1.f - 2.f * (x * x + y * y));
	cov3D[0] = m00 * m00 + m01 * m01 + m02 * m02;
	cov3D[1] = m10 * m00 + m11 * m01 + m12 * m02;
	cov3D[2] = m20 * m00 + m21 * m01 + m22 * m02;
	cov3D[3] = m10 * m10 + m11 * m11 + m12 * m12;
	cov3D[4] = m20 * m10 + m21 * m11 + m22 * m12;
	cov3D[5] = m20 * m20 + m21 * m21 + m22 * m22;
}


__device__ __forceinline__ int xcd_tile(int b, int n_tiles)
{
	const int per = (n_tiles + 7) >> 3;
	return (b & 7) * per + (b >> 3);
}

#ifndef BSR_POOL_K
#define BSR_POOL_K 64
#endif
#ifndef BSR_POOL_E
#define BSR_POOL_E 48
#endif
#define BSR_FLAGS_BYTES 512
#define BSR_POOL_FWD 64
#define BSR_POOL_BWD 96
__host__ __device__ __forceinline__ int pool_tiles_per_band(int n_tiles)
{
	const int per = (n_tiles + 7) >> 3;
	return per >= 8 * BSR_POOL_K ? BSR_POOL_K : 0;
}
static inline int pooled_grid(int n_tiles)
{
	const int per = (n_tiles + 7) >> 3;
	return 8 * (per + (pool_tiles_per_band(n_tiles) ? BSR_POOL_E : 0));
}
__device__ __forceinline__ int pooled_tile(int b, int n_tiles, int* pool_ctr, int* s_slot)
{
	const int per = (n_tiles + 7) >> 3;
	const int k = pool_tiles_per_band(n_tiles), own = per - k;
	const int i = b >> 3;
	int tile;
	if (i < own) {
		tile = (b & 7) * per + i;
	} else {
		if (threadIdx.x == 0) {
			const int j = atomicAdd(pool_ctr, 1);
			if (j == 8 * (k + BSR_POOL_E) - 1) *pool_ctr = 0;
			*s_slot = j;
		}
		__syncthreads();
		const int j = __builtin_amdgcn_readfirstlane(*s_slot);
		tile = j < 8 * k ? (j & 7) * per + own + (j >> 3) : n_tiles;
	}
	tile = __builtin_amdgcn_readfirstlane(tile);
// ... 5 lines not shown
```

### bloomscene_amd/csrc/launch.h

```cpp
#pragma once
#include "common.h"

namespace bsr {

struct BinPlan {
	enum Form { RADIX, CHAIN, BUCKET } form;
	int area, compact;
};

struct RenderBwdArgs {
	int gx, gy, W, H;
	const uint2* tile_range;
	const uint32_t* point_list;
	const float4* rec;
	const uint32_t* wg_base;
	const float* bg;
	const float* final_T;
	const uint32_t* n_contrib;
	const float* dL_dpix;
	const float* out_depth;
	const float* dL_depths;
	int* masks_flag;
	float4* slab;
	bool strict;
	int capacity;
};

void launch_preprocess(const PreArgs& a, bool filter_only, hipStream_t s);
void launch_mark_visible(int P, const float* means3D, const float* vm, uint8_t* present, hipStream_t s);
void launch_visible_filter_views(int P, int V, const float* means3D, const float* scales, float scale_modifier,
                                 const float* rotations, const float* cov3D_precomp, const float* viewmatrices,
                                 const float* projmatrices, int W, int H, float tan_fovx, float tan_fovy, int* radii,
                                 const int* group_of_view, int n_groups, uint8_t* group_mask, uint32_t* wg_counts,
                                 uint32_t* group_counts, hipStream_t s);
void launch_pack_rows(int R, int P, int n_src, const float* const* src, const int* widths, const int64_t* idx,
                      int idx_stride, float* dst_packed, float* const* dst_each, hipStream_t s);
void launch_scans(int n_wg, uint32_t* wg_kept, uint32_t* wg_area, int* flags, uint32_t* hist1, int* host_counts,
                  hipStream_t s);
BinPlan binning_plan(int P, int T, int capacity, long long kept_hint);
void launch_binning(const BinPlan& plan, int P, int T, int gx, const int* n_ptr, int capacity, const GeomState& geom,
                    BinElem* elems_a, BinElem* elems_b, uint32_t* hist, int hist_blocks_max, uint2* tile_range,
                    uint32_t* big_tiles, int* flags, BinElem** elems_sorted, BinElem** elems_free, hipStream_t s);
void launch_sort_tiles(const BinPlan& plan, int T, int n_bound, const int* n_ptr, int capacity, uint2* tile_range,
                       const uint32_t* big_tiles, const int* flags, const uint32_t* digit_total1, const BinElem* elems,
                       BinElem* elems_free, uint32_t* point_list, int force_int, int small_grids, hipStream_t s);
void launch_render_fwd(int gx, int gy, int n_views, int W, int H, const int* n_ptr, int capacity, const uint2* tile_range,
                       uint32_t* point_list, int* masks_flag,
                       const float4* rec, const float* bg, float* final_T, uint32_t* n_contrib, float* out_color,
                       float* out_depth, bool exact_exp, bool nan_on_overflow, int* pool_ctr, hipStream_t s);
void launch_render_bwd(const RenderBwdArgs& a, hipStream_t s);
void launch_render_bwd_strict(const RenderBwdArgs& a, hipStream_t s);
void launch_preprocess_bwd(const BwdArgs& a, hipStream_t s);

}
```

### bloomscene_amd/csrc/preprocess.hip

```cpp
#include "common.h"
#include "sh.h"
#include "tile_common.h"
#include "launch.h"

namespace bsr {

struct Cov2DTerms {
	float t0[3], t1[3];
	float tx, ty, tz;
	float xmul, ymul;
};

__device__ __forceinline__ void cov2d_terms(const float3 mean, float focal_x, float focal_y, float tan_fovx,
                                            float tan_fovy, const float* __restrict__ vm, Cov2DTerms& o)
{
	float tx = vm[0] * mean.x + vm[4] * mean.y + vm[8] * mean.z + vm[12];
	float ty = vm[1] * mean.x + vm[5] * mean.y + vm[9] * mean.z + vm[13];
	const float tz = vm[2] * mean.x + vm[6] * mean.y + vm[10] * mean.z + vm[14];
	const float limx = 1.3f * tan_fovx;
	const float limy = 1.3f * tan_fovy;
	const float txtz = tx / tz;
	const float tytz = ty / tz;
	tx = fminf(limx, fmaxf(-limx, txtz)) * tz;
	ty = fminf(limy, fmaxf(-limy, tytz)) * tz;
// ... 19 lines not shown
	const float A20 = t.t0[0] * c[2] + t.t0[1] * c[4] + t.t0[2] * c[5];
	const float A01 = t.t1[0] * c[0] + t.t1[1] * c[1] + t.t1[2] * c[2];
	const float A11 = t.t1[0] * c[1] + t.t1[1] * c[3] + t.t1[2] * c[4];
	const float A21 = t.t1[0] * c[2] + t.t1[1] * c[4] + t.t1[2] * c[5];
	a = A00 * t.t0[0] + A10 * t.t0[1] + A20 * t.t0[2];
	b = A01 * t.t0[0] + A11 * t.t0[1] + A21 * t.t0[2];
	cc = A01 * t.t1[0] + A11 * t.t1[1] + A21 * t.t1[2];
	a += 0.3f;
	cc += 0.3f;
}

__device__ __forceinline__ float ndc2pix(float v, int S) { return (float)(((v + 1.0) * S - 1.0) * 0.5); }

__device__ __forceinline__ void get_rect(float px, float py, int max_radius, int gx, int gy, int* rmin, int* rmax)
{
	rmin[0] = min(gx, max(0, (int)((px - max_radius) / BSR_TILE)));
	rmin[1] = min(gy, max(0, (int)((py - max_radius) / BSR_TILE)));
	rmax[0] = min(gx, max(0, (int)((px + max_radius + BSR_TILE - 1) / BSR_TILE)));
	rmax[1] = min(gy, max(0, (int)((py + max_radius + BSR_TILE - 1) / BSR_TILE)));
}


template <bool FILTER_ONLY, int COLOR = 0>
__global__ void __launch_bounds__(256) k_preprocess(const PreArgs a)
{
	const int idx = blockIdx.x * 256 + threadIdx.x;
	const bool in_range = idx < a.P;
	if (FILTER_ONLY && !in_range) return;
	const int view = (int)blockIdx.y;
	const int wg = view * (int)gridDim.x + (int)blockIdx.x;
	const int id = wg * 256 + (int)threadIdx.x;
	const int ty_off = view * a.gy;

	__shared__ uint32_t s_hist[256];
	if (!FILTER_ONLY) {
		s_hist[threadIdx.x] = 0;
		__syncthreads();
	}

	int radius_out = 0;
	ushort4 rect_out = make_ushort4(0, 0, 0, 0);
	uint64_t kept_mask = 0;
	float4 rq0 = make_float4(0.f, 0.f, 0.f, 0.f), rq1 = rq0, rq2 = rq0;

	const int ld = in_range ? idx : 0;
	float3 p = make_float3(a.means3D[3 * ld], a.means3D[3 * ld + 1], a.means3D[3 * ld + 2]);
	const float* vm = a.viewmatrix + 16 * view;
	const float* pm = a.projmatrix + 16 * view;
	float pvz = vm[2] * p.x + vm[6] * p.y + vm[10] * p.z + vm[14];
	const bool alive = in_range && !(pvz <= BSR_NEAR);
	if (in_range && !alive && a.prefiltered) a.flags[0] = 1;

	bool vis = false;
	float cov3D[6] = {0.f, 0.f, 0.f, 0.f, 0.f, 0.f};
	float conic_a = 0.f, conic_b = 0.f, conic_c = 0.f, pix_x = 0.f, pix_y = 0.f;
	int rmin[2] = {0, 0}, rmax[2] = {0, 0};
	if (alive) {
		const float hx = pm[0] * p.x + pm[4] * p.y + pm[8] * p.z + pm[12];
		const float hy = pm[1] * p.x + pm[5] * p.y + pm[9] * p.z + pm[13];
		const float hw = pm[3] * p.x + pm[7] * p.y + pm[11] * p.z + pm[15];
		const float p_w = 1.0f / (hw + 0.0000001f);
		const float projx = hx * p_w, projy = hy * p_w;

		if (a.cov3D_precomp != nullptr) {
#pragma unroll
			for (int k = 0; k < 6; k++) cov3D[k] = a.cov3D_precomp[(size_t)idx * 6 + k];
		} else {
			const float sc[3] = {a.scales[3 * idx], a.scales[3 * idx + 1], a.scales[3 * idx + 2]};
			const float4 q = reinterpret_cast<const float4*>(a.rotations)[idx];
			cov3d_from_scale_rot(sc, a.scale_modifier, q, cov3D);
		}

		Cov2DTerms tt;
		cov2d_terms(p, a.focal_x, a.focal_y, a.tan_fovx, a.tan_fovy, vm, tt);
		float ca, cb, cc;
		cov2d_eval(tt, cov3D, ca, cb, cc);

		const float det = (ca * cc - cb * cb);
		if (det != 0.0f) {
			const float det_inv = 1.f / det;
			conic_a = cc * det_inv;
			conic_b = -cb * det_inv;
			conic_c = ca * det_inv;
			const float mid = 0.5f * (ca + cc);
			const float lambda1 = mid + sqrtf(fmaxf(0.1f, mid * mid - det));
			const float lambda2 = mid - sqrtf(fmaxf(0.1f, mid * mid - det));
			const float my_radius = ceilf(3.f * sqrtf(fmaxf(lambda1, lambda2)));
			pix_x = ndc2pix(projx, a.W);
			pix_y = ndc2pix(projy, a.H);
			get_rect(pix_x, pix_y, (int)my_radius, a.gx, a.gy, rmin, rmax);
			if ((rmax[0] - rmin[0]) * (rmax[1] - rmin[1]) != 0) {
				radius_out = (int)my_radius;
				vis = true;
			}
		}
	}
	if (in_range && a.radii) a.radii[(size_t)view * a.P + idx] = radius_out;
	if (FILTER_ONLY) return;
	if (!vis && (in_range || a.n_views > 1)) a.geom.rect[id] = make_ushort4(0, 0, 0, 0);

	int li = (int)threadIdx.x;
	{
		constexpr int PACK_MAX = 128, NF = 21;
		__shared__ uint32_t s_pack[NF][PACK_MAX];
		__shared__ uint32_t s_nvis[4];
		const int lane = threadIdx.x & 63, wave = threadIdx.x >> 6;
		const uint64_t vm_mask = wave_ballot(vis);
		if (lane == 0) s_nvis[wave] = (uint32_t)__popcll(vm_mask);
		__syncthreads();
		const uint32_t v0 = s_nvis[0], v1 = s_nvis[1], v2 = s_nvis[2], v3 = s_nvis[3];
		const int n_vis = (int)(v0 + v1 + v2 + v3);
		const int waves_now = (v0 != 0) + (v1 != 0) + (v2 != 0) + (v3 != 0);
		if (n_vis <= PACK_MAX && ((n_vis + 63) >> 6) < waves_now) {
			if (vis) {
				const int slot = (int)((wave > 0 ? v0 : 0u) + (wave > 1 ? v1 : 0u) + (wave > 2 ? v2 : 0u)) +
				                 __popcll(vm_mask & ((1ull << lane) - 1ull));
				s_pack[0][slot] = (uint32_t)threadIdx.x;
				s_pack[1][slot] = __float_as_uint(p.x); s_pack[2][slot] = __float_as_uint(p.y); s_pack[3][slot] = __float_as_uint(p.z);
#pragma unroll
				for (int k = 0; k < 6; k++) s_pack[4 + k][slot] = __float_as_uint(cov3D[k]);
				s_pack[10][slot] = __float_as_uint(conic_a); s_pack[11][slot] = __float_as_uint(conic_b); s_pack[12][slot] = __float_as_uint(conic_c);
				s_pack[13][slot] = (uint32_t)radius_out;
				s_pack[14][slot] = __float_as_uint(pix_x); s_pack[15][slot] = __float_as_uint(pix_y);
				s_pack[16][slot] = (uint32_t)rmin[0]; s_pack[17][slot] = (uint32_t)rmin[1];
				s_pack[18][slot] = (uint32_t)rmax[0]; s_pack[19][slot] = (uint32_t)rmax[1];
				s_pack[20][slot] = __float_as_uint(pvz);
			}
			__syncthreads();
			const int t = (int)threadIdx.x;
			vis = t < n_vis;
			radius_out = 0;
			if (vis) {
				li = (int)s_pack[0][t];
				p = make_float3(__uint_as_float(s_pack[1][t]), __uint_as_float(s_pack[2][t]), __uint_as_float(s_pack[3][t]));
#pragma unroll
				for (int k = 0; k < 6; k++) cov3D[k] = __uint_as_float(s_pack[4 + k][t]);
				conic_a = __uint_as_float(s_pack[10][t]); conic_b = __uint_as_float(s_pack[11][t]); conic_c = __uint_as_float(s_pack[12][t]);
				radius_out = (int)s_pack[13][t];
				pix_x = __uint_as_float(s_pack[14][t]); pix_y = __uint_as_float(s_pack[15][t]);
				rmin[0] = (int)s_pack[16][t]; rmin[1] = (int)s_pack[17][t];
				rmax[0] = (int)s_pack[18][t]; rmax[1] = (int)s_pack[19][t];
				pvz = __uint_as_float(s_pack[20][t]);
			}
		}
	}
	const int gi = (int)blockIdx.x * 256 + li;
	const int gid = wg * 256 + li;

	if (vis) {
		rect_out = make_ushort4((unsigned short)rmin[0], (unsigned short)(rmin[1] + ty_off),
		                        (unsigned short)rmax[0], (unsigned short)(rmax[1] + ty_off));
		float rgb[3];
		uint8_t clamp_bits = 0;
		if (COLOR == 1) {
			sh3_to_rgb_stream(p, a.cam_pos + 3 * view, a.shs + (size_t)gi * 48, rgb, clamp_bits);
		} else if (COLOR == 0 && a.colors_precomp == nullptr) {
			sh_to_rgb(a.D, a.M, p, a.cam_pos + 3 * view, a.shs + (size_t)gi * a.M * 3, rgb, clamp_bits);
		} else {
			rgb[0] = a.colors_precomp[3 * gi];
			rgb[1] = a.colors_precomp[3 * gi + 1];
			rgb[2] = a.colors_precomp[3 * gi + 2];
		}
		const float opacity = a.opacities[gi];
		const float power_cut = -logf(255.0f * opacity) - 1.0e-3f;
		rq0 = make_float4(pix_x, pix_y, -0.5f * conic_a, -conic_b);
		rq1 = make_float4(-0.5f * conic_c, power_cut, opacity, pvz);
		a.geom.clamped[gid] = clamp_bits;
		const uint32_t area = (uint32_t)(rmax[0] - rmin[0]) * (uint32_t)(rmax[1] - rmin[1]);
		const bool pd = (conic_a > 0.0f) && (conic_c > 0.0f) && (conic_a * conic_c - conic_b * conic_b > 0.0f);
		const float rb_c = -conic_b / conic_c, rb_a = -conic_b / conic_a;
		if (area <= 64u) {
			int x0 = rmin[0], x1 = rmax[0], y0 = rmin[1], y1 = rmax[1];
			const float tq = -(power_cut - (1.0e-3f + 1.0e-4f * fabsf(power_cut)));
			const float cdet = conic_a * conic_c - conic_b * conic_b;
			if (pd) {
				if (tq < 0.0f) {
					x1 = x0;
				} else {
					const float hx = sqrtf(2.0f * tq * conic_c / cdet) * 1.0001f + 0.01f;
					const float hy = sqrtf(2.0f * tq * conic_a / cdet) * 1.0001f + 0.01f;
					if (hx == hx && hy == hy) {
						x0 = max(x0, (int)ceilf((pix_x - hx - 15.0f) * (1.0f / BSR_TILE)));
						x1 = min(x1, (int)floorf((pix_x + hx) * (1.0f / BSR_TILE)) + 1);
						y0 = max(y0, (int)ceilf((pix_y - hy - 15.0f) * (1.0f / BSR_TILE)));
						y1 = min(y1, (int)floorf((pix_y + hy) * (1.0f / BSR_TILE)) + 1);
					}
				}
			}
			const int w = rmax[0] - rmin[0];
			for (int y = y0; y < y1; y++)
				for (int x = x0; x < x1; x++) {
#ifdef BSR_PRE_KNOCK_CULL
					if (true) {
#else
					if (box_may_hit<15>(pix_x, pix_y, conic_a, conic_b, conic_c, power_cut, rb_c, rb_a, pd,
					                    (float)(x * BSR_TILE), (float)(y * BSR_TILE))) {
#endif
						kept_mask |= (1ull << (uint32_t)((y - rmin[1]) * w + (x - rmin[0])));
						atomicAdd(&s_hist[(uint32_t)((y + ty_off) * a.gx + x) & 255u], 1u);
					}
				}
		} else {
			for (int y = rmin[1]; y < rmax[1]; y++)
				for (int x = rmin[0]; x < rmax[0]; x++)
					atomicAdd(&s_hist[(uint32_t)((y + ty_off) * a.gx + x) & 255u], 1u);
		}
		rq2 = make_float4(rgb[0], rgb[1], rgb[2], __uint_as_float((uint32_t)(kept_mask >> 32)));
	}
	{
		__shared__ uint32_t s_wave[4];
		__shared__ uint32_t s_area[4];
		const int lane = threadIdx.x & 63, wave = threadIdx.x >> 6;
		const uint32_t area_all = (uint32_t)(rect_out.z - rect_out.x) * (uint32_t)(rect_out.w - rect_out.y);
		const uint32_t n_inst = area_all ? kept_count(area_all, kept_mask) : 0u;
		const uint32_t incl = wave_inclusive_sum_dpp(n_inst);
		const uint32_t area_sum = wave_inclusive_sum_dpp(area_all);
		if (lane == 63) {
			s_wave[wave] = incl;
			s_area[wave] = area_sum;
		}
		__syncthreads();
		const uint32_t w0 = s_wave[0], w1 = s_wave[1], w2 = s_wave[2], w3 = s_wave[3];
		{
			const int per = ((int)(gridDim.x * gridDim.y) + 7) >> 3;
			if (a.n_views <= 1 || s_hist[threadIdx.x] != 0u)
				a.geom.hist1[(size_t)threadIdx.x * (8 * per) + hist1_column(wg, per)] = s_hist[threadIdx.x];
		}
		if (threadIdx.x == 0) {
			a.geom.wg_kept[wg] = w0 + w1 + w2 + w3;
			a.geom.wg_area[wg] = s_area[0] + s_area[1] + s_area[2] + s_area[3];
		}
		if (vis) {
			const uint32_t off = (wave > 0 ? w0 : 0u) + (wave > 1 ? w1 : 0u) + (wave > 2 ? w2 : 0u) + incl - n_inst;
			a.geom.rect[gid] = rect_out;
			a.geom.depth[gid] = rq1.w;
			a.geom.inst_offset[gid] = off;
			a.geom.kept_mask[gid] = kept_mask;
			{
				float4* rec = a.geom.rec + (size_t)gid * BSR_REC;
				rec[0] = rq0;
				rec[1] = rq1;
				rec[2] = rq2;
				rec[3] = make_float4(
				    __uint_as_float(off), __uint_as_float((uint32_t)rect_out.x | ((uint32_t)rect_out.y << 16)),
				    __uint_as_float((uint32_t)(rect_out.z - rect_out.x) | ((uint32_t)(rect_out.w - rect_out.y) << 16)),
				    __uint_as_float((uint32_t)kept_mask));
			}
		}
	}
}

__global__ void __launch_bounds__(256) k_mark_visible(int P, const float* __restrict__ means3D,
                                                      const float* __restrict__ vm, uint8_t* __restrict__ present)
{
	const int idx = blockIdx.x * 256 + threadIdx.x;
	if (idx >= P) return;
	const float pvz = vm[2] * means3D[3 * idx] + vm[6] * means3D[3 * idx + 1] + vm[10] * means3D[3 * idx + 2] + vm[14];
	present[idx] = !(pvz <= BSR_NEAR);
}

struct FilterWaveLds {
	float g[9][64];
	uint32_t q[128];
	uint32_t seen[2][64];
};

__device__ __forceinline__ void filter_wave_sync()
{
	__builtin_amdgcn_fence(__ATOMIC_RELEASE, "wavefront");
	__builtin_amdgcn_wave_barrier();
	__builtin_amdgcn_fence(__ATOMIC_ACQUIRE, "wavefront");
}

__global__ void __launch_bounds__(256) k_visible_filter_views(int P, int V, const float* __restrict__ means3D,
                                                              const float* __restrict__ scales, float scale_modifier,
                                                              const float* __restrict__ rotations,
                                                              const float* __restrict__ cov3D_precomp,
                                                              const float* __restrict__ viewmatrices,
                                                              const float* __restrict__ projmatrices, int W, int H,
                                                              float focal_x, float focal_y, float tan_fovx,
                                                              float tan_fovy, int gx, int gy, int* __restrict__ radii,
                                                              const int* __restrict__ group_of_view, int n_groups,
                                                              uint8_t* __restrict__ group_mask,
                                                              uint32_t* __restrict__ wg_counts)
{
	__shared__ FilterWaveLds lds_all[4];
	FilterWaveLds& L = lds_all[threadIdx.x >> 6];
	const int lane = threadIdx.x & 63;
	const int idx = blockIdx.x * 256 + threadIdx.x;
	const int wave_base = idx - lane;
	const bool valid = idx < P;
	const bool groups_only = (radii == nullptr && group_mask != nullptr);

	float3 p = make_float3(0.f, 0.f, 0.f);
	float cov3D[6] = {0.f, 0.f, 0.f, 0.f, 0.f, 0.f};
	if (valid) {
		p = make_float3(means3D[3 * idx], means3D[3 * idx + 1], means3D[3 * idx + 2]);
		if (cov3D_precomp != nullptr) {
#pragma unroll
			for (int k = 0; k < 6; k++) cov3D[k] = cov3D_precomp[(size_t)idx * 6 + k];
		} else {
			const float sc[3] = {scales[3 * idx], scales[3 * idx + 1], scales[3 * idx + 2]};
			const float4 q = reinterpret_cast<const float4*>(rotations)[idx];
			cov3d_from_scale_rot(sc, scale_modifier, q, cov3D);
		}
	}
	L.g[0][lane] = p.x; L.g[1][lane] = p.y; L.g[2][lane] = p.z;
#pragma unroll
	for (int k = 0; k < 6; k++) L.g[3 + k][lane] = cov3D[k];
	L.seen[0][lane] = 0u; L.seen[1][lane] = 0u;
	const float sF = sqrtf(cov3D[0] * cov3D[0] + cov3D[3] * cov3D[3] + cov3D[5] * cov3D[5] +
	                       2.0f * (cov3D[1] * cov3D[1] + cov3D[2] * cov3D[2] + cov3D[4] * cov3D[4]));
	const float limx = 1.3f * tan_fovx, limy = 1.3f * tan_fovy;
	const float K = focal_x * focal_x * (1.0f + limx * limx) + focal_y * focal_y * (1.0f + limy * limy);
	const float xmax = 16.0f * (float)gx, ymax = 16.0f * (float)gy;
	filter_wave_sync();

	auto drain = [&](uint32_t base, uint32_t n) {
		if ((uint32_t)lane < n) {
			const uint32_t e = L.q[base + lane];
			const int src = (int)(e & 63u), v = (int)(e >> 6);
			const float3 pp = make_float3(L.g[0][src], L.g[1][src], L.g[2][src]);
			float cc3[6];
#pragma unroll
			for (int k = 0; k < 6; k++) cc3[k] = L.g[3 + k][src];
			const float* vm = viewmatrices + 16 * v;
			const float* pm = projmatrices + 16 * v;
			int radius_out = 0;
			const float pvz = vm[2] * pp.x + vm[6] * pp.y + vm[10] * pp.z + vm[14];
			if (!(pvz <= BSR_NEAR)) {
				const float hx = pm[0] * pp.x + pm[4] * pp.y + pm[8] * pp.z + pm[12];
				const float hy = pm[1] * pp.x + pm[5] * pp.y + pm[9] * pp.z + pm[13];
				const float hw = pm[3] * pp.x + pm[7] * pp.y + pm[11] * pp.z + pm[15];
				const float p_w = 1.0f / (hw + 0.0000001f);
				const float projx = hx * p_w, projy = hy * p_w;
				Cov2DTerms tt;
				cov2d_terms(pp, focal_x, focal_y, tan_fovx, tan_fovy, vm, tt);
				float ca, cb, cc;
				cov2d_eval(tt, cc3, ca, cb, cc);
				const float det = (ca * cc - cb * cb);
				if (det != 0.0f) {
					const float mid = 0.5f * (ca + cc);
					const float lambda1 = mid + sqrtf(fmaxf(0.1f, mid * mid - det));
					const float lambda2 = mid - sqrtf(fmaxf(0.1f, mid * mid - det));
					const float my_radius = ceilf(3.f * sqrtf(fmaxf(lambda1, lambda2)));
					const float pix_x = ndc2pix(projx, W), pix_y = ndc2pix(projy, H);
					int rmin[2], rmax[2];
					get_rect(pix_x, pix_y, (int)my_radius, gx, gy, rmin, rmax);
					if ((rmax[0] - rmin[0]) * (rmax[1] - rmin[1]) != 0) radius_out = (int)my_radius;
				}
			}
			if (radii != nullptr) radii[(size_t)v * P + wave_base + src] = radius_out;
			if (group_mask != nullptr && radius_out > 0) {
				const int g = group_of_view[v] & 63;
				atomicOr(&L.seen[g >> 5][src], 1u << (g & 31));
			}
		}
		filter_wave_sync();
	};

	uint32_t count = 0;
	for (int v = 0; v < V; v++) {
		const float* vm = viewmatrices + 16 * v;
		const float* pm = projmatrices + 16 * v;
		bool cand = valid;
		if (groups_only) {
			const int g = group_of_view[v] & 63;
			cand = cand && !((L.seen[g >> 5][lane] >> (g & 31)) & 1u);
		}
		const float pvz = vm[2] * p.x + vm[6] * p.y + vm[10] * p.z + vm[14];
		cand = cand && !(pvz <= BSR_NEAR);
		{
			const float hx = pm[0] * p.x + pm[4] * p.y + pm[8] * p.z + pm[12];
			const float hy = pm[1] * p.x + pm[5] * p.y + pm[9] * p.z + pm[13];
			const float hw = pm[3] * p.x + pm[7] * p.y + pm[11] * p.z + pm[15];
			const float p_w = __builtin_amdgcn_rcpf(hw + 0.0000001f);
			const float pxf = ((hx * p_w + 1.0f) * (float)W - 1.0f) * 0.5f;
			const float pyf = ((hy * p_w + 1.0f) * (float)H - 1.0f) * 0.5f;
			const float wF2 = vm[0] * vm[0] + vm[1] * vm[1] + vm[2] * vm[2] + vm[4] * vm[4] + vm[5] * vm[5] +
			                  vm[6] * vm[6] + vm[8] * vm[8] + vm[9] * vm[9] + vm[10] * vm[10];
			const float itz = __builtin_amdgcn_rcpf(pvz);
			const float B = (K * wF2) * sF * (itz * itz);
			const float rb = 3.01f * __builtin_amdgcn_sqrtf(1.5015f * B + 1.0f) + 2.0f;
			const float slx = 2.0f + 1.0e-5f * fabsf(pxf), sly = 2.0f + 1.0e-5f * fabsf(pyf);
			const bool outside = (pxf + rb < -slx) || (pxf - rb > xmax + slx) || (pyf + rb < -sly) || (pyf - rb > ymax + sly);
			cand = cand && !outside;
		}
		if (radii != nullptr && valid && !cand) radii[(size_t)v * P + idx] = 0;
		const unsigned long long m = __ballot(cand);
		if (m != 0ull) {
			if (cand) L.q[count + __builtin_amdgcn_mbcnt_hi((uint32_t)(m >> 32), __builtin_amdgcn_mbcnt_lo((uint32_t)m, 0u))] =
				((uint32_t)v << 6) | (uint32_t)lane;
			count += (uint32_t)__popcll(m);
			filter_wave_sync();
			if (count >= 64u) {
				count -= 64u;
				drain(count, 64u);
			}
		}
	}
	if (count != 0u) drain(0u, count);

	if (group_mask != nullptr) {
		__shared__ uint32_t s_cnt[4][64];
		const unsigned long long seen = (unsigned long long)L.seen[0][lane] | ((unsigned long long)L.seen[1][lane] << 32);
		for (int g = 0; g < n_groups; g++) {
			const bool bit = valid && ((seen >> g) & 1ull);
			if (valid) group_mask[(size_t)g * P + idx] = (uint8_t)bit;
			if (wg_counts != nullptr) {
				const unsigned long long mb = __ballot(bit);
				if (lane == 0) s_cnt[threadIdx.x >> 6][g] = (uint32_t)__popcll(mb);
			}
		}
		if (wg_counts != nullptr) {
			__syncthreads();
			if ((int)threadIdx.x < n_groups)
				wg_counts[(size_t)threadIdx.x * gridDim.x + blockIdx.x] =
				    s_cnt[0][threadIdx.x] + s_cnt[1][threadIdx.x] + s_cnt[2][threadIdx.x] + s_cnt[3][threadIdx.x];
		}
	}
}

__global__ void __launch_bounds__(256) k_sum_group_counts(int n_wg, const uint32_t* __restrict__ wg_counts,
                                                          uint32_t* __restrict__ group_counts)
{
	__shared__ uint32_t part[256];
	uint32_t acc = 0;
	for (int i = threadIdx.x; i < n_wg; i += 256) acc += wg_counts[(size_t)blockIdx.x * n_wg + i];
	part[threadIdx.x] = acc;
	__syncthreads();
	for (int h = 128; h > 0; h >>= 1) {
		if ((int)threadIdx.x < h) part[threadIdx.x] += part[threadIdx.x + h];
		__syncthreads();
	}
	if (threadIdx.x == 0) group_counts[blockIdx.x] = part[0];
}

void launch_visible_filter_views(int P, int V, const float* means3D, const float* scales, float scale_modifier,
                                 const float* rotations, const float* cov3D_precomp, const float* viewmatrices,
                                 const float* projmatrices, int W, int H, float tan_fovx, float tan_fovy, int* radii,
                                 const int* group_of_view, int n_groups, uint8_t* group_mask, uint32_t* wg_counts,
                                 uint32_t* group_counts, hipStream_t s)
{
	const int n_wg = (P + 255) / 256;
	hipLaunchKernelGGL(k_visible_filter_views, dim3(n_wg), dim3(256), 0, s, P, V, means3D, scales,
	                   scale_modifier, rotations, cov3D_precomp, viewmatrices, projmatrices, W, H,
	                   W / (2.0f * tan_fovx), H / (2.0f * tan_fovy), tan_fovx, tan_fovy, (W + BSR_TILE - 1) / BSR_TILE,
	                   (H + BSR_TILE - 1) / BSR_TILE, radii, group_of_view, n_groups, group_mask,
	                   group_counts != nullptr ? wg_counts : nullptr);
	if (group_counts != nullptr && n_groups > 0)
		hipLaunchKernelGGL(k_sum_group_counts, dim3(n_groups), dim3(256), 0, s, n_wg, wg_counts, group_counts);
}

void launch_preprocess(const PreArgs& a, bool filter_only, hipStream_t s)
{
	const int blocks = (a.P + 255) / 256;
	if (filter_only)
		hipLaunchKernelGGL((k_preprocess<true, 0>), dim3(blocks), dim3(256), 0, s, a);
	else if (a.colors_precomp == nullptr && a.D == 3 && a.M == 16)
		hipLaunchKernelGGL((k_preprocess<false, 1>), dim3(blocks, a.n_views > 1 ? a.n_views : 1), dim3(256), 0, s, a);
	else if (a.colors_precomp != nullptr)
		hipLaunchKernelGGL((k_preprocess<false, 2>), dim3(blocks, a.n_views > 1 ? a.n_views : 1), dim3(256), 0, s, a);
	else
		hipLaunchKernelGGL((k_preprocess<false, 0>), dim3(blocks, a.n_views > 1 ? a.n_views : 1), dim3(256), 0, s, a);
}

void launch_mark_visible(int P, const float* means3D, const float* vm, uint8_t* present, hipStream_t s)
{
	hipLaunchKernelGGL(k_mark_visible, dim3((P + 255) / 256), dim3(256), 0, s, P, means3D, vm, present);
}

}
```

### bloomscene_amd/csrc/preprocess_bwd.hip

```cpp
#include "common.h"
#include "sh.h"
#include "launch.h"

namespace bsr {


template <int N>
__device__ __forceinline__ void store_sh_grad(float* __restrict__ dst, int M, const float* v)
{
	const int total = M * 3;
	if ((M & 3) == 0) {
		float4* d4 = reinterpret_cast<float4*>(dst);
		constexpr int NV = (N + 3) / 4;
#pragma unroll
		for (int i = 0; i < NV; i++) {
			float4 o;
			o.x = (i * 4 + 0 < N) ? v[i * 4 + 0] : 0.f;
			o.y = (i * 4 + 1 < N) ? v[i * 4 + 1] : 0.f;
			o.z = (i * 4 + 2 < N) ? v[i * 4 + 2] : 0.f;
			o.w = (i * 4 + 3 < N) ? v[i * 4 + 3] : 0.f;
			if (i * 4 < total) d4[i] = o;
		}
		for (int i = NV; i < (total >> 2); i++) d4[i] = make_float4(0.f, 0.f, 0.f, 0.f);
	} else {
#pragma unroll
		for (int i = 0; i < N; i++)
			if (i < total) dst[i] = v[i];
		for (int i = N; i < total; i++) dst[i] = 0.f;
	}
}

__device__ __forceinline__ void zero_sh_grad(float* __restrict__ dst, int M)
{
	const int total = M * 3;
	if ((M & 3) == 0) {
		float4* d4 = reinterpret_cast<float4*>(dst);
		for (int i = 0; i < (total >> 2); i++) d4[i] = make_float4(0.f, 0.f, 0.f, 0.f);
	} else {
		for (int i = 0; i < total; i++) dst[i] = 0.f;
	}
}

template <int DEG>
__device__ __forceinline__ void sh_bwd_deg(const BwdArgs& a, int idx, const float3 m, const float* dcolor, float* dmean)
{
	constexpr int NC = (DEG + 1) * (DEG + 1);
	const float ox = m.x - a.campos[0], oy = m.y - a.campos[1], oz = m.z - a.campos[2];
	const float len = sqrtf((ox * ox + oy * oy) + oz * oz);
	const float x = ox / len, y = oy / len, z = oz / len;
	const uint8_t cl = a.geom.clamped[idx];
	float dL_dRGB[3] = {dcolor[0], dcolor[1], dcolor[2]};
	dL_dRGB[0] *= (cl & 1) ? 0.f : 1.f;
	dL_dRGB[1] *= (cl & 2) ? 0.f : 1.f;
	dL_dRGB[2] *= (cl & 4) ? 0.f : 1.f;
	{
		float dsh[NC * 3];
		sh_coef_grad<DEG>(x, y, z, dL_dRGB, dsh);
		store_sh_grad<NC * 3>(a.dL_dsh + (size_t)idx * a.M * 3, a.M, dsh);
	}
	__builtin_amdgcn_sched_barrier(0);
	float dL_ddir[3];
	{
		float c[NC * 3];
		load_sh<NC>(a.shs + (size_t)idx * a.M * 3, a.M, c);
		sh_dir_grad<DEG>(c, x, y, z, dL_dRGB, dL_ddir);
	}
	const float sum2 = ox * ox + oy * oy + oz * oz;
	const float invsum32 = 1.0f / sqrtf(sum2 * sum2 * sum2);
	dmean[0] += ((+sum2 - ox * ox) * dL_ddir[0] - oy * ox * dL_ddir[1] - oz * ox * dL_ddir[2]) * invsum32;
	dmean[1] += (-ox * oy * dL_ddir[0] + (sum2 - oy * oy) * dL_ddir[1] - oz * oy * dL_ddir[2]) * invsum32;
	dmean[2] += (-ox * oz * dL_ddir[0] - oy * oz * dL_ddir[1] + (sum2 - oz * oz) * dL_ddir[2]) * invsum32;
}

template <int DEG, int ROW_F4>
__device__ __forceinline__ void sh_bwd_coop_half(const BwdArgs& a, int idx, bool visible, const float3 m, const float* dcolor,
                                                 float* dmean, ShTile<ROW_F4, 32>& tile, int lane, int g0, int n_valid)
{
	constexpr int NC = (DEG + 1) * (DEG + 1);
	constexpr int N = NC * 3;
	constexpr int STRIDE = ShTile<ROW_F4, 32>::STRIDE;
	const float ox = m.x - a.campos[0], oy = m.y - a.campos[1], oz = m.z - a.campos[2];
	const float len = sqrtf((ox * ox + oy * oy) + oz * oz);
	const float x = visible ? ox / len : 0.f, y = visible ? oy / len : 0.f, z = visible ? oz / len : 0.f;
	const uint8_t cl = visible ? a.geom.clamped[idx] : (uint8_t)7;
	float dL_dRGB[3] = {0.f, 0.f, 0.f};
	if (visible) {
		dL_dRGB[0] = dcolor[0] * ((cl & 1) ? 0.f : 1.f);
		dL_dRGB[1] = dcolor[1] * ((cl & 2) ? 0.f : 1.f);
		dL_dRGB[2] = dcolor[2] * ((cl & 4) ? 0.f : 1.f);
	}
	const int half = lane >> 5;
	float4* const row = &tile.rows[(lane & 31) * STRIDE];
	{
		float b[NC];
		sh_coef_basis<DEG>(x, y, z, b);
#pragma unroll
		for (int h = 0; h < 2; h++) {
			if (half == h) {
#pragma unroll
				for (int i = 0; i < ROW_F4; i++) {
					float4 o;
					o.x = (i * 4 + 0 < N) ? b[(i * 4 + 0 < N) ? (i * 4 + 0) / 3 : 0] * dL_dRGB[(i * 4 + 0) % 3] : 0.f;
					o.y = (i * 4 + 1 < N) ? b[(i * 4 + 1 < N) ? (i * 4 + 1) / 3 : 0] * dL_dRGB[(i * 4 + 1) % 3] : 0.f;
					o.z = (i * 4 + 2 < N) ? b[(i * 4 + 2 < N) ? (i * 4 + 2) / 3 : 0] * dL_dRGB[(i * 4 + 2) % 3] : 0.f;
					o.w = (i * 4 + 3 < N) ? b[(i * 4 + 3 < N) ? (i * 4 + 3) / 3 : 0] * dL_dRGB[(i * 4 + 3) % 3] : 0.f;
					row[i] = o;
				}
			}
			__builtin_amdgcn_fence(__ATOMIC_RELEASE, "wavefront");
			__builtin_amdgcn_wave_barrier();
			__builtin_amdgcn_fence(__ATOMIC_ACQUIRE, "wavefront");
			sh_tile_store<ROW_F4, 32>(tile, a.dL_dsh, g0 + 32 * h, min(32, max(0, n_valid - 32 * h)), lane);
			__builtin_amdgcn_fence(__ATOMIC_RELEASE, "wavefront");
			__builtin_amdgcn_wave_barrier();
			__builtin_amdgcn_fence(__ATOMIC_ACQUIRE, "wavefront");
		}
	}
	const uint64_t vis_mask = __ballot(visible);
	if (vis_mask == 0ull) return;
	float dL_ddir[3] = {0.f, 0.f, 0.f};
#pragma unroll
	for (int h = 0; h < 2; h++) {
		if (((vis_mask >> (32 * h)) & 0xffffffffull) == 0ull) continue;
		sh_tile_load<ROW_F4, 32>(tile, a.shs, g0 + 32 * h, min(32, max(0, n_valid - 32 * h)), lane);
		__builtin_amdgcn_fence(__ATOMIC_RELEASE, "wavefront");
		__builtin_amdgcn_wave_barrier();
		__builtin_amdgcn_fence(__ATOMIC_ACQUIRE, "wavefront");
		if (visible && half == h) {
			const float* const c = reinterpret_cast<const float*>(row);
			float dx0, dy0, dz0, dx1, dy1, dz1, dx2, dy2, dz2;
			sh_dir_grad_channel<DEG, 0>(c, x, y, z, dx0, dy0, dz0);
			__builtin_amdgcn_sched_barrier(0);
			sh_dir_grad_channel<DEG, 1>(c, x, y, z, dx1, dy1, dz1);
			__builtin_amdgcn_sched_barrier(0);
			sh_dir_grad_channel<DEG, 2>(c, x, y, z, dx2, dy2, dz2);
			dL_ddir[0] = (dx0 * dL_dRGB[0] + dx1 * dL_dRGB[1]) + dx2 * dL_dRGB[2];
			dL_ddir[1] = (dy0 * dL_dRGB[0] + dy1 * dL_dRGB[1]) + dy2 * dL_dRGB[2];
			dL_ddir[2] = (dz0 * dL_dRGB[0] + dz1 * dL_dRGB[1]) + dz2 * dL_dRGB[2];
		}
		__builtin_amdgcn_fence(__ATOMIC_RELEASE, "wavefront");
		__builtin_amdgcn_wave_barrier();
		__builtin_amdgcn_fence(__ATOMIC_ACQUIRE, "wavefront");
	}
	if (visible) {
		const float sum2 = ox * ox + oy * oy + oz * oz;
		const float invsum32 = 1.0f / sqrtf(sum2 * sum2 * sum2);
		dmean[0] += ((+sum2 - ox * ox) * dL_ddir[0] - oy * ox * dL_ddir[1] - oz * ox * dL_ddir[2]) * invsum32;
		dmean[1] += (-ox * oy * dL_ddir[0] + (sum2 - oy * oy) * dL_ddir[1] - oz * oy * dL_ddir[2]) * invsum32;
		dmean[2] += (-ox * oz * dL_ddir[0] - oy * oz * dL_ddir[1] + (sum2 - oz * oz) * dL_ddir[2]) * invsum32;
	}
}

template <int ROW_F4>
__global__ void __launch_bounds__(256, (ROW_F4 == 12 ? 6 : 4)) k_preprocess_bwd(const BwdArgs a)
{
	const int idx = blockIdx.x * 256 + threadIdx.x;
	const bool in_range = idx < a.P;
	const bool overflow = __builtin_amdgcn_readfirstlane(*a.kept_ptr) > a.capacity;
	const ushort4 rc = (in_range && !overflow) ? a.geom.rect[idx] : make_ushort4(0, 0, 0, 0);
	const bool visible = in_range && !overflow && (a.radii ? (a.radii[idx] > 0) : (rc.z > rc.x && rc.w > rc.y));

	constexpr int STAGE_F4 = (ROW_F4 > 0 && 32 * (ROW_F4 + 1) > 192) ? 32 * (ROW_F4 + 1) : 192;
	__shared__ float4 s_stage[4][STAGE_F4];
	float g[9] = {0.f, 0.f, 0.f, 0.f, 0.f, 0.f, 0.f, 0.f, 0.f};
	float g_z = 0.f;
	{
		const uint32_t rowf = (uint32_t)slab_row_floats(a.depth_grad != 0);
		const uint32_t stage_rows = (uint32_t)(STAGE_F4 * 4) / rowf;
		const int lane = threadIdx.x & 63;
		float4* const stage = s_stage[threadIdx.x >> 6];
		const float* const stage_f = reinterpret_cast<const float*>(stage);
		const uint32_t area = (uint32_t)(rc.z - rc.x) * (uint32_t)(rc.w - rc.y);
		const uint32_t n_inst = area ? kept_count(area, a.geom.kept_mask[idx]) : 0u;
		const uint32_t off = n_inst ? a.geom.wg_kept[idx >> 8] + a.geom.inst_offset[idx] : 0u;
		const uint32_t incl = wave_inclusive_sum_dpp(n_inst);
		const uint32_t excl = incl - n_inst;
		const uint32_t total = (uint32_t)__builtin_amdgcn_readlane((int)incl, 63);
		const uint64_t has = wave_ballot(n_inst != 0u);
		if (has != 0ull) {
			const uint32_t run0 = (uint32_t)__builtin_amdgcn_readlane((int)(off - excl), (int)__builtin_ctzll(has));
			const float* const src = reinterpret_cast<const float*>(a.slab) + (size_t)run0 * rowf;
			for (uint32_t c0 = 0; c0 < total; c0 += stage_rows) {
				const uint32_t n_rows = min(stage_rows, total - c0);
				const uint32_t n_f4 = (n_rows * rowf + 3u) >> 2;
				const bsr_f32x4_a4* const s = reinterpret_cast<const bsr_f32x4_a4*>(src + (size_t)c0 * rowf);
				for (uint32_t i0 = 0; i0 < n_f4; i0 += 256) {
					const uint32_t i = i0 + (uint32_t)lane;
					bsr_f32x4 v0, v1, v2, v3;
					if (i < n_f4) v0 = s[i];
					if (i + 64 < n_f4) v1 = s[i + 64];
					if (i + 128 < n_f4) v2 = s[i + 128];
					if (i + 192 < n_f4) v3 = s[i + 192];
					if (i < n_f4) stage[i] = make_float4(v0.x, v0.y, v0.z, v0.w);
					if (i + 64 < n_f4) stage[i + 64] = make_float4(v1.x, v1.y, v1.z, v1.w);
					if (i + 128 < n_f4) stage[i + 128] = make_float4(v2.x, v2.y, v2.z, v2.w);
					if (i + 192 < n_f4) stage[i + 192] = make_float4(v3.x, v3.y, v3.z, v3.w);
				}
				__builtin_amdgcn_fence(__ATOMIC_RELEASE, "wavefront");
				__builtin_amdgcn_wave_barrier();
				__builtin_amdgcn_fence(__ATOMIC_ACQUIRE, "wavefront");
				const uint32_t k0 = max(excl, c0), k1 = min(incl, c0 + n_rows);
				for (uint32_t k = k0; k < k1; k++) {
					const float* row = stage_f + (k - c0) * rowf;
					g[0] += row[0]; g[1] += row[1]; g[2] += row[2]; g[3] += row[3];
					g[4] += row[4]; g[5] += row[5]; g[6] += row[6]; g[7] += row[7];
					g[8] += row[8];
					if (a.depth_grad) g_z += row[9];
				}
				__builtin_amdgcn_fence(__ATOMIC_RELEASE, "wavefront");
				__builtin_amdgcn_wave_barrier();
				__builtin_amdgcn_fence(__ATOMIC_ACQUIRE, "wavefront");
			}
		}
	}
	if (in_range) {
		a.dL_dmean2D[3 * idx] = g[0];
		a.dL_dmean2D[3 * idx + 1] = g[1];
		a.dL_dmean2D[3 * idx + 2] = 0.f;
		if (a.dL_dconic) reinterpret_cast<float4*>(a.dL_dconic)[idx] = make_float4(g[2], g[3], 0.f, g[4]);
		a.dL_dopacity[idx] = g[5];
		if (a.dL_dcolor) {
			a.dL_dcolor[3 * idx] = g[6];
			a.dL_dcolor[3 * idx + 1] = g[7];
			a.dL_dcolor[3 * idx + 2] = g[8];
		}
	}

	float dmean[3] = {0.f, 0.f, 0.f};
	float dcov[6] = {0.f, 0.f, 0.f, 0.f, 0.f, 0.f};
	float dscale[3] = {0.f, 0.f, 0.f};
	float drot[4] = {0.f, 0.f, 0.f, 0.f};

	const int li = in_range ? idx : 0;
	const float3 m = make_float3(a.means3D[3 * li], a.means3D[3 * li + 1], a.means3D[3 * li + 2]);
	if (visible) {
		const float* vm = a.viewmatrix;

		float V[6];
		float sc_in[3] = {0.f, 0.f, 0.f};
		float4 q_in = make_float4(0.f, 0.f, 0.f, 0.f);
		if (a.cov3D_precomp) {
#pragma unroll
			for (int k = 0; k < 6; k++) V[k] = a.cov3D_precomp[(size_t)idx * 6 + k];
		} else {
			sc_in[0] = a.scales[3 * idx]; sc_in[1] = a.scales[3 * idx + 1]; sc_in[2] = a.scales[3 * idx + 2];
			q_in = reinterpret_cast<const float4*>(a.rotations)[idx];
			cov3d_from_scale_rot(sc_in, a.scale_modifier, q_in, V);
		}
		const float dcx = g[2], dcy = g[3], dcw = g[4];

		float tx = vm[0] * m.x + vm[4] * m.y + vm[8] * m.z + vm[12];
		float ty = vm[1] * m.x + vm[5] * m.y + vm[9] * m.z + vm[13];
		const float tz_ = vm[2] * m.x + vm[6] * m.y + vm[10] * m.z + vm[14];
		const float limx = 1.3f * a.tan_fovx;
		const float limy = 1.3f * a.tan_fovy;
		const float txtz = tx / tz_;
		const float tytz = ty / tz_;
		tx = fminf(limx, fmaxf(-limx, txtz)) * tz_;
		ty = fminf(limy, fmaxf(-limy, tytz)) * tz_;
		const float x_grad_mul = (txtz < -limx || txtz > limx) ? 0.0f : 1.0f;
		const float y_grad_mul = (tytz < -limy || tytz > limy) ? 0.0f : 1.0f;
		const float h_x = a.focal_x, h_y = a.focal_y;
		const float J00 = h_x / tz_;
		const float J02 = -(h_x * tx) / (tz_ * tz_);
		const float J11 = h_y / tz_;
		const float J12 = -(h_y * ty) / (tz_ * tz_);
		const float T00 = vm[0] * J00 + vm[2] * J02, T01 = vm[4] * J00 + vm[6] * J02, T02 = vm[8] * J00 + vm[10] * J02;
		const float T10 = vm[1] * J11 + vm[2] * J12, T11 = vm[5] * J11 + vm[6] * J12, T12 = vm[9] * J11 + vm[10] * J12;
		const float V00 = V[0], V01 = V[1], V02 = V[2], V11 = V[3], V12 = V[4], V22 = V[5];
		const float A00 = T00 * V00 + T01 * V01 + T02 * V02;
		const float A10 = T00 * V01 + T01 * V11 + T02 * V12;
		const float A20 = T00 * V02 + T01 * V12 + T02 * V22;
		const float A01 = T10 * V00 + T11 * V01 + T12 * V02;
		const float A11 = T10 * V01 + T11 * V11 + T12 * V12;
		const float A21 = T10 * V02 + T11 * V12 + T12 * V22;
		float ca = A00 * T00 + A10 * T01 + A20 * T02;
		const float cb = A01 * T00 + A11 * T01 + A21 * T02;
		float cc = A01 * T10 + A11 * T11 + A21 * T12;
		ca += 0.3f;
		cc += 0.3f;
		const float a_ = ca, b_ = cb, c_ = cc;
		const float denom = a_ * c_ - b_ * b_;
		float dL_da = 0, dL_db = 0, dL_dc = 0;
		const float denom2inv = 1.0f / ((denom * denom) + 0.0000001f);
		if (denom2inv != 0) {
			dL_da = denom2inv * (-c_ * c_ * dcx + 2 * b_ * c_ * dcy + (denom - a_ * c_) * dcw);
			dL_dc = denom2inv * (-a_ * a_ * dcw + 2 * a_ * b_ * dcy + (denom - a_ * c_) * dcx);
			dL_db = denom2inv * 2 * (b_ * c_ * dcx - (denom + 2 * b_ * b_) * dcy + a_ * b_ * dcw);
			dcov[0] = (T00 * T00 * dL_da + T00 * T10 * dL_db + T10 * T10 * dL_dc);
			dcov[3] = (T01 * T01 * dL_da + T01 * T11 * dL_db + T11 * T11 * dL_dc);
			dcov[5] = (T02 * T02 * dL_da + T02 * T12 * dL_db + T12 * T12 * dL_dc);
			dcov[1] = 2 * T00 * T01 * dL_da + (T00 * T11 + T01 * T10) * dL_db + 2 * T10 * T11 * dL_dc;
			dcov[2] = 2 * T00 * T02 * dL_da + (T00 * T12 + T02 * T10) * dL_db + 2 * T10 * T12 * dL_dc;
			dcov[4] = 2 * T02 * T01 * dL_da + (T01 * T12 + T02 * T11) * dL_db + 2 * T11 * T12 * dL_dc;
		}
		const float dL_dT00 = 2 * (T00 * V00 + T01 * V01 + T02 * V02) * dL_da + (T10 * V00 + T11 * V01 + T12 * V02) * dL_db;
		const float dL_dT01 = 2 * (T00 * V01 + T01 * V11 + T02 * V12) * dL_da + (T10 * V01 + T11 * V11 + T12 * V12) * dL_db;
		const float dL_dT02 = 2 * (T00 * V02 + T01 * V12 + T02 * V22) * dL_da + (T10 * V02 + T11 * V12 + T12 * V22) * dL_db;
		const float dL_dT10 = 2 * (T10 * V00 + T11 * V01 + T12 * V02) * dL_dc + (T00 * V00 + T01 * V01 + T02 * V02) * dL_db;
		const float dL_dT11 = 2 * (T10 * V01 + T11 * V11 + T12 * V12) * dL_dc + (T00 * V01 + T01 * V11 + T02 * V12) * dL_db;
		const float dL_dT12 = 2 * (T10 * V02 + T11 * V12 + T12 * V22) * dL_dc + (T00 * V02 + T01 * V12 + T02 * V22) * dL_db;
		const float dL_dJ00 = vm[0] * dL_dT00 + vm[4] * dL_dT01 + vm[8] * dL_dT02;
		const float dL_dJ02 = vm[2] * dL_dT00 + vm[6] * dL_dT01 + vm[10] * dL_dT02;
		const float dL_dJ11 = vm[1] * dL_dT10 + vm[5] * dL_dT11 + vm[9] * dL_dT12;
		const float dL_dJ12 = vm[2] * dL_dT10 + vm[6] * dL_dT11 + vm[10] * dL_dT12;
		const float tz = 1.f / tz_;
		const float tz2 = tz * tz;
		const float tz3 = tz2 * tz;
		const float dL_dtx = x_grad_mul * -h_x * tz2 * dL_dJ02;
		const float dL_dty = y_grad_mul * -h_y * tz2 * dL_dJ12;
		const float dL_dtz = -h_x * tz2 * dL_dJ00 - h_y * tz2 * dL_dJ11 + (2 * h_x * tx) * tz3 * dL_dJ02 + (2 * h_y * ty) * tz3 * dL_dJ12;
		dmean[0] = vm[0] * dL_dtx + vm[1] * dL_dty + vm[2] * dL_dtz;
		dmean[1] = vm[4] * dL_dtx + vm[5] * dL_dty + vm[6] * dL_dtz;
		dmean[2] = vm[8] * dL_dtx + vm[9] * dL_dty + vm[10] * dL_dtz;

		const float* proj = a.projmatrix;
		const float m_homw = proj[3] * m.x + proj[7] * m.y + proj[11] * m.z + proj[15];
		const float m_w = 1.0f / (m_homw + 0.0000001f);
		const float mul1 = (proj[0] * m.x + proj[4] * m.y + proj[8] * m.z + proj[12]) * m_w * m_w;
		const float mul2 = (proj[1] * m.x + proj[5] * m.y + proj[9] * m.z + proj[13]) * m_w * m_w;
		const float g2x = g[0], g2y = g[1];
		const float pdx = (proj[0] * m_w - proj[3] * mul1) * g2x + (proj[1] * m_w - proj[3] * mul2) * g2y;
		const float pdy = (proj[4] * m_w - proj[7] * mul1) * g2x + (proj[5] * m_w - proj[7] * mul2) * g2y;
		const float pdz = (proj[8] * m_w - proj[11] * mul1) * g2x + (proj[9] * m_w - proj[11] * mul2) * g2y;
		dmean[0] += pdx;
		dmean[1] += pdy;
		dmean[2] += pdz;

		if (ROW_F4 == 0 && a.shs) {
			if (a.D <= 0) sh_bwd_deg<0>(a, idx, m, &g[6], dmean);
			else if (a.D == 1) sh_bwd_deg<1>(a, idx, m, &g[6], dmean);
			else if (a.D == 2) sh_bwd_deg<2>(a, idx, m, &g[6], dmean);
			else sh_bwd_deg<3>(a, idx, m, &g[6], dmean);
		}

		if (a.scales) {
			const float4 q = q_in;
			const float r = q.x, x = q.y, y = q.z, z = q.w;
			const float s[3] = {a.scale_modifier * sc_in[0], a.scale_modifier * sc_in[1], a.scale_modifier * sc_in[2]};
			const float Rm[3][3] = {
			    {1.f - 2.f * (y * y + z * z), 2.f * (x * y - r * z), 2.f * (x * z + r * y)},
			    {2.f * (x * y + r * z), 1.f - 2.f * (x * x + z * z), 2.f * (y * z - r * x)},
			    {2.f * (x * z - r * y), 2.f * (y * z + r * x), 1.f - 2.f * (x * x + y * y)}};
			float M2[3][3];
#pragma unroll
			for (int c = 0; c < 3; c++)
#pragma unroll
				for (int k = 0; k < 3; k++) M2[c][k] = 2.0f * (s[k] * Rm[c][k]);
			const float dS[3][3] = {{dcov[0], 0.5f * dcov[1], 0.5f * dcov[2]},
			                        {0.5f * dcov[1], dcov[3], 0.5f * dcov[4]},
			                        {0.5f * dcov[2], 0.5f * dcov[4], dcov[5]}};
			float dM[3][3];
#pragma unroll
			for (int c = 0; c < 3; c++)
#pragma unroll
				for (int rr = 0; rr < 3; rr++) dM[c][rr] = M2[0][rr] * dS[c][0] + M2[1][rr] * dS[c][1] + M2[2][rr] * dS[c][2];
#pragma unroll
			for (int i = 0; i < 3; i++) dscale[i] = (Rm[0][i] * dM[0][i] + Rm[1][i] * dM[1][i]) + Rm[2][i] * dM[2][i];
			float G[3][3];
#pragma unroll
			for (int i = 0; i < 3; i++)
#pragma unroll
				for (int j = 0; j < 3; j++) G[i][j] = dM[j][i] * s[i];
			drot[0] = 2 * z * (G[0][1] - G[1][0]) + 2 * y * (G[2][0] - G[0][2]) + 2 * x * (G[1][2] - G[2][1]);
			drot[1] = 2 * y * (G[1][0] + G[0][1]) + 2 * z * (G[2][0] + G[0][2]) + 2 * r * (G[1][2] - G[2][1]) - 4 * x * (G[2][2] + G[1][1]);
			drot[2] = 2 * x * (G[1][0] + G[0][1]) + 2 * r * (G[2][0] - G[0][2]) + 2 * z * (G[1][2] + G[2][1]) - 4 * y * (G[2][2] + G[0][0]);
			drot[3] = 2 * r * (G[0][1] - G[1][0]) + 2 * x * (G[2][0] + G[0][2]) + 2 * y * (G[1][2] + G[2][1]) - 4 * z * (G[1][1] + G[0][0]);
		}
	} else if (ROW_F4 == 0 && in_range && a.shs && a.dL_dsh) {
		zero_sh_grad(a.dL_dsh + (size_t)idx * a.M * 3, a.M);
	}

	if (in_range) {
		if (a.dL_dcov3D) {
#pragma unroll
			for (int k = 0; k < 6; k++) a.dL_dcov3D[(size_t)idx * 6 + k] = dcov[k];
		}
		if (a.scales) {
			a.dL_dscale[3 * idx] = dscale[0];
			a.dL_dscale[3 * idx + 1] = dscale[1];
			a.dL_dscale[3 * idx + 2] = dscale[2];
			reinterpret_cast<float4*>(a.dL_drot)[idx] = make_float4(drot[0], drot[1], drot[2], drot[3]);
		}
	}

	__builtin_amdgcn_sched_barrier(0);
	if (ROW_F4 > 0) {
		const int lane = threadIdx.x & 63, wave = threadIdx.x >> 6;
		const int g0 = blockIdx.x * 256 + wave * 64;
		const int n_valid = min(64, max(0, a.P - g0));
		constexpr int RF = ROW_F4 > 0 ? ROW_F4 : 1, RF12 = ROW_F4 >= 12 ? ROW_F4 : 12;
		static_assert(sizeof(ShTile<RF, 32>) <= sizeof(s_stage[0]), "the SH tile lives in the staging area");
		ShTile<RF, 32>& tile = *reinterpret_cast<ShTile<RF, 32>*>(&s_stage[wave][0]);
		if (a.D <= 0) sh_bwd_coop_half<0, RF>(a, idx, visible, m, &g[6], dmean, tile, lane, g0, n_valid);
		else if (a.D == 1) sh_bwd_coop_half<1, RF>(a, idx, visible, m, &g[6], dmean, tile, lane, g0, n_valid);
		else if (ROW_F4 < 12) {  }
		else if (a.D == 2) sh_bwd_coop_half<2, RF12>(a, idx, visible, m, &g[6], dmean, *reinterpret_cast<ShTile<RF12, 32>*>(&tile), lane, g0, n_valid);
		else sh_bwd_coop_half<3, RF12>(a, idx, visible, m, &g[6], dmean, *reinterpret_cast<ShTile<RF12, 32>*>(&tile), lane, g0, n_valid);
	}
	if (!in_range) return;

	if (a.depth_grad && visible) {
		dmean[0] += a.viewmatrix[2] * g_z;
		dmean[1] += a.viewmatrix[6] * g_z;
		dmean[2] += a.viewmatrix[10] * g_z;
	}
	if (overflow) dmean[0] = dmean[1] = dmean[2] = __builtin_nanf("");
	a.dL_dmean3D[3 * idx] = dmean[0];
	a.dL_dmean3D[3 * idx + 1] = dmean[1];
	a.dL_dmean3D[3 * idx + 2] = dmean[2];
}

void launch_preprocess_bwd(const BwdArgs& a, hipStream_t s)
{
	const dim3 grid((a.P + 255) / 256), block(256);
	if (a.shs && a.M == 16)
		hipLaunchKernelGGL(k_preprocess_bwd<12>, grid, block, 0, s, a);
	else if (a.shs && a.M == 4)
		hipLaunchKernelGGL(k_preprocess_bwd<3>, grid, block, 0, s, a);
	else if (!a.shs)
		hipLaunchKernelGGL(k_preprocess_bwd<-1>, grid, block, 0, s, a);
	else
		hipLaunchKernelGGL(k_preprocess_bwd<0>, grid, block, 0, s, a);
}

}
```

### bloomscene_amd/csrc/scratch.h

```cpp
#pragma once
#include "common.h"

namespace bsr {

static constexpr size_t BSR_RADIX_BINS_ = 256;

struct Carver {
	char* base;
	size_t off = 0;
	template <class T> T* take(size_t n)
	{
		T* r = base ? (T*)(base + off) : nullptr;
		off += align_up(n * sizeof(T), 256);
		return r;
	}
};

static inline size_t hist1_columns(size_t n_wg) { return (n_wg + 7) / 8 * 8; }

inline GeomState GeomState::layout(Carver& c, size_t P)
{
	const size_t n_wg = (P + 255) / 256;
	GeomState g;
	g.rec = c.take<float4>(P * BSR_REC);
	g.inst_offset = c.take<uint32_t>(P);
	g.wg_kept = c.take<uint32_t>(n_wg);
	g.wg_area = c.take<uint32_t>(n_wg);
	g.hist1 = c.take<uint32_t>(BSR_RADIX_BINS_ * hist1_columns(n_wg) + 512);
	g.kept_mask = c.take<uint64_t>(P);
	g.rect = c.take<ushort4>(P);
	g.clamped = c.take<uint8_t>(P);
	g.depth = c.take<float>(P);
	return g;
}
inline size_t GeomState::bytes(size_t P) { Carver c{nullptr}; layout(c, P); return c.off + 256; }
inline GeomState GeomState::carve(char* p, size_t P) { Carver c{(char*)align_up((size_t)p, 256)}; return layout(c, P); }

inline BinState BinState::layout(Carver& c, size_t R, bool with_slab)
{
	BinState b;
	b.point_list = c.take<uint32_t>(R);
	Carver pingpong = c, slab = c;
	b.elems_a = pingpong.take<BinElem>(R);
	b.elems_b = pingpong.take<BinElem>(R);
	b.slab = (float4*)slab.take<char>(with_slab ? R * BSR_SLAB_ROW_BYTES + BSR_SLAB_TAIL_BYTES : 0);
	c.off = pingpong.off > slab.off ? pingpong.off : slab.off;
	b.hist = c.take<uint32_t>(BSR_RADIX_BINS_ * (BSR_HIST_BLOCKS_MAX + 1));
	return b;
}
inline size_t BinState::bytes(size_t R, bool with_slab) { Carver c{nullptr}; layout(c, R, with_slab); return c.off + 256; }
inline BinState BinState::carve(char* p, size_t R, bool with_slab) { Carver c{(char*)align_up((size_t)p, 256)}; return layout(c, R, with_slab); }

static inline bool backward_fits(size_t cap, size_t R, size_t kept)
{
	Carver c{nullptr};
	c.take<uint32_t>(R);
	c.take<char>(kept * BSR_SLAB_ROW_BYTES + BSR_SLAB_TAIL_BYTES);
	return c.off <= BinState::bytes(cap, true) - 256;
}

inline ImgState ImgState::layout(Carver& c, size_t N, size_t T)
{
	ImgState i;
	i.final_T = c.take<float>(N);
	i.n_contrib = c.take<uint32_t>(N);
	i.tile_range = c.take<uint2>(T);
	i.flags = c.take<int>(BSR_FLAGS_BYTES / sizeof(int));
	i.big_tiles = c.take<uint32_t>(3 * T);
	return i;
}
inline size_t ImgState::bytes(size_t N, size_t T) { Carver c{nullptr}; layout(c, N, T); return c.off + 256; }
inline ImgState ImgState::carve(char* p, size_t N, size_t T) { Carver c{(char*)align_up((size_t)p, 256)}; return layout(c, N, T); }

}
```

### bloomscene_amd/csrc/sh.h

```cpp
#pragma once
#include "common.h"

namespace bsr {

__device__ static const float SH_C0 = 0.28209479177387814f;
__device__ static const float SH_C1 = 0.4886025119029199f;
__device__ static const float SH_C2[5] = {1.0925484305920792f, -1.0925484305920792f, 0.31539156525252005f,
                                          -1.0925484305920792f, 0.5462742152960396f};
__device__ static const float SH_C3[7] = {-0.5900435899266435f, 2.890611442640554f, -0.4570457994644658f,
                                          0.3731763325901154f,  -0.4570457994644658f, 1.445305721320277f,
                                          -0.5900435899266435f};

template <int NC>
__device__ __forceinline__ void load_sh(const float* __restrict__ sh, int M, float* c)
{
	if ((M & 3) == 0) {
		const float4* s4 = reinterpret_cast<const float4*>(sh);
		constexpr int NV = (NC * 3 + 3) / 4;
#pragma unroll
		for (int i = 0; i < NV; i++) {
			if (i * 4 < M * 3) {
				const float4 v = s4[i];
				if (i * 4 + 0 < NC * 3) c[i * 4 + 0] = v.x;
				if (i * 4 + 1 < NC * 3) c[i * 4 + 1] = v.y;
				if (i * 4 + 2 < NC * 3) c[i * 4 + 2] = v.z;
				if (i * 4 + 3 < NC * 3) c[i * 4 + 3] = v.w;
			}
		}
	} else {
#pragma unroll
		for (int i = 0; i < NC * 3; i++) c[i] = sh[i];
	}
}

template <int DEG>
__device__ __forceinline__ void sh_eval(const float* c, float x, float y, float z, float* res)
{
#pragma unroll
	for (int ch = 0; ch < 3; ch++) {
#define SH(k) c[(k) * 3 + ch]
		float r = SH_C0 * SH(0);
		if (DEG > 0) {
			r = r - SH_C1 * y * SH(1) + SH_C1 * z * SH(2) - SH_C1 * x * SH(3);
			if (DEG > 1) {
				const float xx = x * x, yy = y * y, zz = z * z;
				const float xy = x * y, yz = y * z, xz = x * z;
				r = r + SH_C2[0] * xy * SH(4) + SH_C2[1] * yz * SH(5) + SH_C2[2] * (2.0f * zz - xx - yy) * SH(6) +
				    SH_C2[3] * xz * SH(7) + SH_C2[4] * (xx - yy) * SH(8);
				if (DEG > 2) {
					r = r + SH_C3[0] * y * (3.0f * xx - yy) * SH(9) + SH_C3[1] * xy * z * SH(10) +
					    SH_C3[2] * y * (4.0f * zz - xx - yy) * SH(11) +
					    SH_C3[3] * z * (2.0f * zz - 3.0f * xx - 3.0f * yy) * SH(12) +
					    SH_C3[4] * x * (4.0f * zz - xx - yy) * SH(13) + SH_C3[5] * z * (xx - yy) * SH(14) +
					    SH_C3[6] * x * (xx - 3.0f * yy) * SH(15);
				}
			}
		}
#undef SH
		res[ch] = r + 0.5f;
	}
}

__device__ __forceinline__ float sh3_basis(int k, float x, float y, float z, float xx, float yy, float zz, float xy,
                                           float yz, float xz)
{
	switch (k) {
	case 0: return SH_C0;
	case 1: return SH_C1 * y;
	case 2: return SH_C1 * z;
	case 3: return SH_C1 * x;
	case 4: return SH_C2[0] * xy;
	case 5: return SH_C2[1] * yz;
	case 6: return SH_C2[2] * (2.0f * zz - xx - yy);
	case 7: return SH_C2[3] * xz;
	case 8: return SH_C2[4] * (xx - yy);
	case 9: return SH_C3[0] * y * (3.0f * xx - yy);
	case 10: return SH_C3[1] * xy * z;
	case 11: return SH_C3[2] * y * (4.0f * zz - xx - yy);
	case 12: return SH_C3[3] * z * (2.0f * zz - 3.0f * xx - 3.0f * yy);
	case 13: return SH_C3[4] * x * (4.0f * zz - xx - yy);
	case 14: return SH_C3[5] * z * (xx - yy);
	default: return SH_C3[6] * x * (xx - 3.0f * yy);
	}
}

__device__ __forceinline__ void sh_eval3_stream(const float* __restrict__ sh, float x, float y, float z, float* res)
{
	const float xx = x * x, yy = y * y, zz = z * z;
	const float xy = x * y, yz = y * z, xz = x * z;
	const float4* s4 = reinterpret_cast<const float4*>(sh);
	float r[3] = {0.f, 0.f, 0.f};
#ifndef BSR_SH_GROUP
#define BSR_SH_GROUP 6
#endif
	constexpr int GS = BSR_SH_GROUP;
	static_assert(12 % GS == 0, "twelve 16-byte loads");
#pragma unroll
	for (int g = 0; g < 12 / GS; g++) {
		if (g > 0) asm volatile("" : "+v"(s4), "+v"(r[0]), "+v"(r[1]), "+v"(r[2]));
		float v[4 * GS];
#pragma unroll
		for (int i = 0; i < GS; i++) {
			const float4 q = s4[GS * g + i];
			v[4 * i + 0] = q.x; v[4 * i + 1] = q.y; v[4 * i + 2] = q.z; v[4 * i + 3] = q.w;
		}
#pragma unroll
		for (int j = 0; j < 4 * GS; j++) {
			const int p = 4 * GS * g + j, k = p / 3, ch = p % 3;
			const float b = sh3_basis(k, x, y, z, xx, yy, zz, xy, yz, xz);
			if (k == 0) r[ch] = b * v[j];
			else if (k == 1 || k == 3) r[ch] = r[ch] - b * v[j];
			else r[ch] = r[ch] + b * v[j];
		}
	}
#pragma unroll
	for (int ch = 0; ch < 3; ch++) res[ch] = r[ch] + 0.5f;
}

__device__ __forceinline__ void sh_to_rgb(int deg, int M, const float3 pos, const float* __restrict__ campos,
                                          const float* __restrict__ sh, float* rgb, uint8_t& clamp_bits)
{
	float dx = pos.x - campos[0], dy = pos.y - campos[1], dz = pos.z - campos[2];
	const float len = sqrtf((dx * dx + dy * dy) + dz * dz);
	dx = dx / len; dy = dy / len; dz = dz / len;
	float raw[3];
	if (deg <= 0) {
		float c[3];
		load_sh<1>(sh, M, c);
		sh_eval<0>(c, dx, dy, dz, raw);
	} else if (deg == 1) {
		float c[12];
		load_sh<4>(sh, M, c);
		sh_eval<1>(c, dx, dy, dz, raw);
	} else if (deg == 2) {
		float c[27];
		load_sh<9>(sh, M, c);
		sh_eval<2>(c, dx, dy, dz, raw);
	} else {
		float c[48];
		load_sh<16>(sh, M, c);
		sh_eval<3>(c, dx, dy, dz, raw);
	}
	clamp_bits = 0;
#pragma unroll
	for (int ch = 0; ch < 3; ch++) {
		if (raw[ch] < 0) clamp_bits |= (uint8_t)(1u << ch);
		rgb[ch] = fmaxf(raw[ch], 0.0f);
	}
}

__device__ __forceinline__ void sh3_to_rgb_stream(const float3 pos, const float* __restrict__ campos,
                                                  const float* __restrict__ sh, float* rgb, uint8_t& clamp_bits)
{
	float dx = pos.x - campos[0], dy = pos.y - campos[1], dz = pos.z - campos[2];
	const float len = sqrtf((dx * dx + dy * dy) + dz * dz);
	dx = dx / len; dy = dy / len; dz = dz / len;
	float raw[3];
	sh_eval3_stream(sh, dx, dy, dz, raw);
	clamp_bits = 0;
#pragma unroll
	for (int ch = 0; ch < 3; ch++) {
		if (raw[ch] < 0) clamp_bits |= (uint8_t)(1u << ch);
		rgb[ch] = fmaxf(raw[ch], 0.0f);
	}
}

template <int DEG>
__device__ __forceinline__ void sh_coef_grad(float x, float y, float z, const float* dL_dRGB, float* dsh)
{
#define DSH(k, v)                                                    \
	do {                                                             \
		const float _v = (v);                                        \
		_Pragma("unroll") for (int ch = 0; ch < 3; ch++) dsh[(k) * 3 + ch] = _v * dL_dRGB[ch]; \
	} while (0)
	DSH(0, SH_C0);
	if (DEG > 0) {
		DSH(1, -SH_C1 * y);
		DSH(2, SH_C1 * z);
		DSH(3, -SH_C1 * x);
		if (DEG > 1) {
			const float xx = x * x, yy = y * y, zz = z * z;
			const float xy = x * y, yz = y * z, xz = x * z;
			DSH(4, SH_C2[0] * xy);
			DSH(5, SH_C2[1] * yz);
			DSH(6, SH_C2[2] * (2.f * zz - xx - yy));
			DSH(7, SH_C2[3] * xz);
			DSH(8, SH_C2[4] * (xx - yy));
			if (DEG > 2) {
				DSH(9, SH_C3[0] * y * (3.f * xx - yy));
				DSH(10, SH_C3[1] * xy * z);
				DSH(11, SH_C3[2] * y * (4.f * zz - xx - yy));
				DSH(12, SH_C3[3] * z * (2.f * zz - 3.f * xx - 3.f * yy));
				DSH(13, SH_C3[4] * x * (4.f * zz - xx - yy));
				DSH(14, SH_C3[5] * z * (xx - yy));
				DSH(15, SH_C3[6] * x * (xx - 3.f * yy));
			}
		}
	}
#undef DSH
}

template <int DEG>
__device__ __forceinline__ void sh_dir_grad(const float* c, float x, float y, float z, const float* dL_dRGB,
                                            float* dL_ddir)
{
	float dRGBdx[3] = {0, 0, 0}, dRGBdy[3] = {0, 0, 0}, dRGBdz[3] = {0, 0, 0};
#define SH(k) c[(k) * 3 + ch]
	if (DEG > 0) {
#pragma unroll
		for (int ch = 0; ch < 3; ch++) {
			dRGBdx[ch] = -SH_C1 * SH(3);
			dRGBdy[ch] = -SH_C1 * SH(1);
			dRGBdz[ch] = SH_C1 * SH(2);
		}
		if (DEG > 1) {
			const float xx = x * x, yy = y * y, zz = z * z;
			const float xy = x * y, yz = y * z, xz = x * z;
#pragma unroll
			for (int ch = 0; ch < 3; ch++) {
				dRGBdx[ch] += SH_C2[0] * y * SH(4) + SH_C2[2] * 2.f * -x * SH(6) + SH_C2[3] * z * SH(7) + SH_C2[4] * 2.f * x * SH(8);
				dRGBdy[ch] += SH_C2[0] * x * SH(4) + SH_C2[1] * z * SH(5) + SH_C2[2] * 2.f * -y * SH(6) + SH_C2[4] * 2.f * -y * SH(8);
				dRGBdz[ch] += SH_C2[1] * y * SH(5) + SH_C2[2] * 2.f * 2.f * z * SH(6) + SH_C2[3] * x * SH(7);
			}
			if (DEG > 2) {
#pragma unroll
				for (int ch = 0; ch < 3; ch++) {
					dRGBdx[ch] += (SH_C3[0] * SH(9) * 3.f * 2.f * xy + SH_C3[1] * SH(10) * yz +
					               SH_C3[2] * SH(11) * -2.f * xy + SH_C3[3] * SH(12) * -3.f * 2.f * xz +
					               SH_C3[4] * SH(13) * (-3.f * xx + 4.f * zz - yy) + SH_C3[5] * SH(14) * 2.f * xz +
					               SH_C3[6] * SH(15) * 3.f * (xx - yy));
					dRGBdy[ch] += (SH_C3[0] * SH(9) * 3.f * (xx - yy) + SH_C3[1] * SH(10) * xz +
					               SH_C3[2] * SH(11) * (-3.f * yy + 4.f * zz - xx) + SH_C3[3] * SH(12) * -3.f * 2.f * yz +
					               SH_C3[4] * SH(13) * -2.f * xy + SH_C3[5] * SH(14) * -2.f * yz +
					               SH_C3[6] * SH(15) * -3.f * 2.f * xy);
					dRGBdz[ch] += (SH_C3[1] * SH(10) * xy + SH_C3[2] * SH(11) * 4.f * 2.f * yz +
					               SH_C3[3] * SH(12) * 3.f * (2.f * zz - xx - yy) + SH_C3[4] * SH(13) * 4.f * 2.f * xz +
					               SH_C3[5] * SH(14) * (xx - yy));
				}
			}
		}
	}
#undef SH
	dL_ddir[0] = (dRGBdx[0] * dL_dRGB[0] + dRGBdx[1] * dL_dRGB[1]) + dRGBdx[2] * dL_dRGB[2];
	dL_ddir[1] = (dRGBdy[0] * dL_dRGB[0] + dRGBdy[1] * dL_dRGB[1]) + dRGBdy[2] * dL_dRGB[2];
	dL_ddir[2] = (dRGBdz[0] * dL_dRGB[0] + dRGBdz[1] * dL_dRGB[1]) + dRGBdz[2] * dL_dRGB[2];
}

template <int DEG>
__device__ __forceinline__ void sh_coef_basis(float x, float y, float z, float* b)
{
	b[0] = SH_C0;
	if (DEG > 0) {
		b[1] = -SH_C1 * y;
		b[2] = SH_C1 * z;
		b[3] = -SH_C1 * x;
		if (DEG > 1) {
			const float xx = x * x, yy = y * y, zz = z * z;
			const float xy = x * y, yz = y * z, xz = x * z;
			b[4] = SH_C2[0] * xy;
			b[5] = SH_C2[1] * yz;
			b[6] = SH_C2[2] * (2.f * zz - xx - yy);
			b[7] = SH_C2[3] * xz;
			b[8] = SH_C2[4] * (xx - yy);
			if (DEG > 2) {
				b[9] = SH_C3[0] * y * (3.f * xx - yy);
				b[10] = SH_C3[1] * xy * z;
				b[11] = SH_C3[2] * y * (4.f * zz - xx - yy);
				b[12] = SH_C3[3] * z * (2.f * zz - 3.f * xx - 3.f * yy);
				b[13] = SH_C3[4] * x * (4.f * zz - xx - yy);
				b[14] = SH_C3[5] * z * (xx - yy);
				b[15] = SH_C3[6] * x * (xx - 3.f * yy);
			}
		}
	}
}

template <int DEG, int CH>
__device__ __forceinline__ void sh_dir_grad_channel(const float* c, float x, float y, float z, float& dRGBdx, float& dRGBdy,
                                                    float& dRGBdz)
{
	dRGBdx = 0.f; dRGBdy = 0.f; dRGBdz = 0.f;
#define SH(k) c[(k) * 3 + CH]
	if (DEG > 0) {
		dRGBdx = -SH_C1 * SH(3);
		dRGBdy = -SH_C1 * SH(1);
		dRGBdz = SH_C1 * SH(2);
		if (DEG > 1) {
			const float xx = x * x, yy = y * y, zz = z * z;
			const float xy = x * y, yz = y * z, xz = x * z;
			dRGBdx += SH_C2[0] * y * SH(4) + SH_C2[2] * 2.f * -x * SH(6) + SH_C2[3] * z * SH(7) + SH_C2[4] * 2.f * x * SH(8);
			dRGBdy += SH_C2[0] * x * SH(4) + SH_C2[1] * z * SH(5) + SH_C2[2] * 2.f * -y * SH(6) + SH_C2[4] * 2.f * -y * SH(8);
			dRGBdz += SH_C2[1] * y * SH(5) + SH_C2[2] * 2.f * 2.f * z * SH(6) + SH_C2[3] * x * SH(7);
			if (DEG > 2) {
				dRGBdx += (SH_C3[0] * SH(9) * 3.f * 2.f * xy + SH_C3[1] * SH(10) * yz +
				           SH_C3[2] * SH(11) * -2.f * xy + SH_C3[3] * SH(12) * -3.f * 2.f * xz +
				           SH_C3[4] * SH(13) * (-3.f * xx + 4.f * zz - yy) + SH_C3[5] * SH(14) * 2.f * xz +
				           SH_C3[6] * SH(15) * 3.f * (xx - yy));
				dRGBdy += (SH_C3[0] * SH(9) * 3.f * (xx - yy) + SH_C3[1] * SH(10) * xz +
				           SH_C3[2] * SH(11) * (-3.f * yy + 4.f * zz - xx) + SH_C3[3] * SH(12) * -3.f * 2.f * yz +
				           SH_C3[4] * SH(13) * -2.f * xy + SH_C3[5] * SH(14) * -2.f * yz +
				           SH_C3[6] * SH(15) * -3.f * 2.f * xy);
				dRGBdz += (SH_C3[1] * SH(10) * xy + SH_C3[2] * SH(11) * 4.f * 2.f * yz +
				           SH_C3[3] * SH(12) * 3.f * (2.f * zz - xx - yy) + SH_C3[4] * SH(13) * 4.f * 2.f * xz +
				           SH_C3[5] * SH(14) * (xx - yy));
			}
		}
	}
#undef SH
}

template <int ROW_F4, int ROWS = 64>
// ... 39 lines not shown
```

### bloomscene_amd/rasterizer.py

```python
from __future__ import annotations

import ctypes as C
from typing import NamedTuple

import torch
import torch.nn as nn

from . import _capi
from .numerics import FLAG_EXACT_EXP, FLAG_EXACT_GRAD, numerics, resolve_flags

FLAG_NO_READBACK = 4


def cpu_deep_copy_tuple(input_tuple):
    copied_tensors = [item.cpu().clone() if isinstance(item, torch.Tensor) else item for item in input_tuple]
    return tuple(copied_tensors)


class GaussianRasterizationSettings(NamedTuple):
    image_height: int
    image_width: int
    tanfovx: float
    tanfovy: float
    bg: torch.Tensor
    scale_modifier: float
    viewmatrix: torch.Tensor
    projmatrix: torch.Tensor
    sh_degree: int
    campos: torch.Tensor
    prefiltered: bool
    debug: bool


def _dev_f32(t: torch.Tensor, name: str, device: torch.device):
    if t is None or t.numel() == 0:
        return None
    if t.device != device:
        raise RuntimeError(f"{name} must be on {device} (got {t.device}); bloomscene_amd has no CPU path")
    if t.dtype != torch.float32:
        t = t.float()
    return t.contiguous()


def _ptr(t):
    return None if t is None else t.data_ptr()


def _stream_handle(device):
    return C.c_void_p(torch.cuda.current_stream(device).cuda_stream)


class _Scratch:

    def __init__(self, device):
        tensor = torch.empty(0, dtype=torch.uint8, device=device)
        self.tensor = tensor

        def _resize(_user, nbytes):
            tensor.resize_(int(nbytes))
            return tensor.data_ptr()

        self.callback = _capi.ALLOC_FN(_resize)


def _check_means3D(means3D):
    if means3D.dim() != 2 or means3D.size(1) != 3:
        raise RuntimeError("means3D must have dimensions (num_points, 3)")


def _rasterize_gaussians_native(bg, means3D, colors, opacity, scales, rotations, scale_modifier, cov3D_precomp,
                                viewmatrix, projmatrix, tan_fovx, tan_fovy, image_height, image_width, sh, degree,
                                campos, prefiltered, debug, flags=None, capacity=None):
    flags = resolve_flags() if flags is None else int(flags)
    if capacity is not None:
        if int(capacity) <= 0:
            raise RuntimeError("capacity must be a positive number of tile instances")
        flags |= FLAG_NO_READBACK
    _check_means3D(means3D)
    if not means3D.is_cuda:
        raise RuntimeError("means3D must be a GPU tensor; bloomscene_amd has no CPU path")
    dev = means3D.device
    P, H, W = means3D.size(0), int(image_height), int(image_width)
    out_color = torch.empty((3, H, W), dtype=torch.float32, device=dev)
    out_depth = torch.empty((1, H, W), dtype=torch.float32, device=dev)
    radii = torch.empty((P,), dtype=torch.int32, device=dev)
    geom, binning, img = _Scratch(dev), _Scratch(dev), _Scratch(dev)
    M = sh.size(1) if (sh is not None and sh.numel() != 0) else 0
    t = dict(bg=_dev_f32(bg, "bg", dev), means3D=_dev_f32(means3D, "means3D", dev),
             colors=_dev_f32(colors, "colors_precomp", dev), opacity=_dev_f32(opacity, "opacities", dev),
             scales=_dev_f32(scales, "scales", dev), rotations=_dev_f32(rotations, "rotations", dev),
             cov3D=_dev_f32(cov3D_precomp, "cov3D_precomp", dev), view=_dev_f32(viewmatrix, "viewmatrix", dev),
             proj=_dev_f32(projmatrix, "projmatrix", dev), sh=_dev_f32(sh, "shs", dev),
             campos=_dev_f32(campos, "campos", dev))
    num_rendered = C.c_int(int(capacity) if capacity is not None else 0)
    with torch.cuda.device(dev):
        rc = _capi.lib().bsr_forward_ex(
            geom.callback, None, binning.callback, None, img.callback, None,
            P, int(degree), int(M), _ptr(t["bg"]), W, H, _ptr(t["means3D"]), _ptr(t["sh"]), _ptr(t["colors"]),
            _ptr(t["opacity"]), _ptr(t["scales"]), float(scale_modifier), _ptr(t["rotations"]), _ptr(t["cov3D"]),
            _ptr(t["view"]), _ptr(t["proj"]), _ptr(t["campos"]), float(tan_fovx), float(tan_fovy),
            int(bool(prefiltered)), out_color.data_ptr(), out_depth.data_ptr(), radii.data_ptr() if P else None,
            int(bool(debug)), _stream_handle(dev), C.byref(num_rendered), int(flags))
    _capi.check(rc, "rasterize_gaussians")
    return num_rendered.value, out_color, out_depth, radii, geom.tensor, binning.tensor, img.tensor


def _rasterize_gaussians_views_native(bg, means3D, colors, opacity, scales, rotations, scale_modifier, cov3D_precomp,
                                      viewmatrices, projmatrices, tan_fovx, tan_fovy, image_height, image_width, sh,
                                      degree, camposes, prefiltered, debug, flags=None):
    flags = resolve_flags() if flags is None else int(flags)
    _check_means3D(means3D)
    if not means3D.is_cuda:
        raise RuntimeError("means3D must be a GPU tensor; bloomscene_amd has no CPU path")
    dev = means3D.device
    P, H, W = means3D.size(0), int(image_height), int(image_width)
    view = _dev_f32(viewmatrices, "viewmatrices", dev)
    proj = _dev_f32(projmatrices, "projmatrices", dev)
    campos = _dev_f32(camposes, "camposes", dev)
    if view.dim() != 3 or tuple(view.shape[1:]) != (4, 4) or proj.shape != view.shape:
        raise RuntimeError("viewmatrices / projmatrices must have dimensions (num_views, 4, 4)")
    V = view.size(0)
    if campos is None or tuple(campos.shape) != (V, 3):
        raise RuntimeError("camposes must have dimensions (num_views, 3)")
    out_color = torch.empty((V, 3, H, W), dtype=torch.float32, device=dev)
    out_depth = torch.empty((V, 1, H, W), dtype=torch.float32, device=dev)
    radii = torch.empty((V, P), dtype=torch.int32, device=dev)
    geom, binning, img = _Scratch(dev), _Scratch(dev), _Scratch(dev)
    M = sh.size(1) if (sh is not None and sh.numel() != 0) else 0
    t = dict(bg=_dev_f32(bg, "bg", dev), means3D=_dev_f32(means3D, "means3D", dev),
             colors=_dev_f32(colors, "colors_precomp", dev), opacity=_dev_f32(opacity, "opacities", dev),
             scales=_dev_f32(scales, "scales", dev), rotations=_dev_f32(rotations, "rotations", dev),
             cov3D=_dev_f32(cov3D_precomp, "cov3D_precomp", dev), sh=_dev_f32(sh, "shs", dev))
    num_rendered = C.c_int(0)
    with torch.cuda.device(dev):
        rc = _capi.lib().bsr_forward_views(
            geom.callback, None, binning.callback, None, img.callback, None,
            P, int(degree), int(M), int(V), _ptr(t["bg"]), W, H, _ptr(t["means3D"]), _ptr(t["sh"]), _ptr(t["colors"]),
            _ptr(t["opacity"]), _ptr(t["scales"]), float(scale_modifier), _ptr(t["rotations"]), _ptr(t["cov3D"]),
            _ptr(view), _ptr(proj), _ptr(campos), float(tan_fovx), float(tan_fovy),
            int(bool(prefiltered)), out_color.data_ptr(), out_depth.data_ptr(), radii.data_ptr() if P and V else None,
            int(bool(debug)), _stream_handle(dev), C.byref(num_rendered), int(flags))
    _capi.check(rc, "rasterize_gaussians_views")
    return num_rendered.value, out_color, out_depth, radii


def _rasterize_gaussians_backward_native(bg, means3D, radii, colors, scales, rotations, scale_modifier,
                                         cov3D_precomp, viewmatrix, projmatrix, tan_fovx, tan_fovy, dL_dout_color,
                                         dL_dout_depth, sh, degree, campos, geomBuffer, R, binningBuffer,
                                         imageBuffer, debug, out_depth=None, all_outputs=False, flags=None):
    flags = resolve_flags() if flags is None else int(flags)
    dev = means3D.device
    P = means3D.size(0)
    H, W = dL_dout_color.size(1), dL_dout_color.size(2)
    M = sh.size(1) if (sh is not None and sh.numel() != 0) else 0
    o = dict(device=dev, dtype=torch.float32)
    dL_dmeans3D = torch.empty((P, 3), **o)
    dL_dmeans2D = torch.empty((P, 3), **o)
    has_colors = colors is not None and colors.numel() != 0
    has_cov = cov3D_precomp is not None and cov3D_precomp.numel() != 0
    dL_dcolors = torch.empty((P, 3), **o) if (all_outputs or has_colors) else None
    dL_dconic = torch.empty((P, 2, 2), **o) if all_outputs else None
    dL_dopacity = torch.empty((P, 1), **o)
    dL_dcov3D = torch.empty((P, 6), **o) if (all_outputs or has_cov) else None
    dL_dsh = torch.empty((P, M, 3), **o)
    has_sr = scales is not None and scales.numel() != 0
    dL_dscales = torch.empty((P, 3), **o) if has_sr else torch.zeros((P, 3), **o)
    dL_drotations = torch.empty((P, 4), **o) if has_sr else torch.zeros((P, 4), **o)
    if P != 0:
        t = dict(bg=_dev_f32(bg, "bg", dev), means3D=_dev_f32(means3D, "means3D", dev),
                 colors=_dev_f32(colors, "colors_precomp", dev), scales=_dev_f32(scales, "scales", dev),
                 rotations=_dev_f32(rotations, "rotations", dev), cov3D=_dev_f32(cov3D_precomp, "cov3D_precomp", dev),
                 view=_dev_f32(viewmatrix, "viewmatrix", dev), proj=_dev_f32(projmatrix, "projmatrix", dev),
                 sh=_dev_f32(sh, "shs", dev), campos=_dev_f32(campos, "campos", dev),
                 gcol=_dev_f32(dL_dout_color, "dL_dout_color", dev), gdep=_dev_f32(dL_dout_depth, "dL_dout_depth", dev))
        radii_c = radii.contiguous()
        head = (P, int(degree), int(M), int(R), _ptr(t["bg"]), W, H, _ptr(t["means3D"]), _ptr(t["sh"]),
                _ptr(t["colors"]), _ptr(t["scales"]), float(scale_modifier), _ptr(t["rotations"]), _ptr(t["cov3D"]),
                _ptr(t["view"]), _ptr(t["proj"]), _ptr(t["campos"]), float(tan_fovx), float(tan_fovy),
                radii_c.data_ptr(), geomBuffer.data_ptr(), binningBuffer.data_ptr() if binningBuffer.numel() else None,
                imageBuffer.data_ptr())
        tail = (_ptr(t["gcol"]), _ptr(t["gdep"]), dL_dmeans2D.data_ptr(),
                _ptr(dL_dconic), dL_dopacity.data_ptr(), _ptr(dL_dcolors), dL_dmeans3D.data_ptr(),
                _ptr(dL_dcov3D), dL_dsh.data_ptr() if M else None, dL_dscales.data_ptr(),
                dL_drotations.data_ptr(), int(bool(debug)), _stream_handle(dev))
        od = None if out_depth is None else _dev_f32(out_depth, "out_depth", dev)
        with torch.cuda.device(dev):
            rc = _capi.lib().bsr_backward_ex(*head, _ptr(od), *tail, int(flags))
        _capi.check(rc, "rasterize_gaussians_backward")
    return dL_dmeans2D, dL_dcolors, dL_dopacity, dL_dmeans3D, dL_dcov3D, dL_dsh, dL_dscales, dL_drotations


def _mark_visible_native(means3D, viewmatrix, projmatrix):
    dev = means3D.device
    if not means3D.is_cuda:
        raise RuntimeError("positions must be a GPU tensor; bloomscene_amd has no CPU path")
    P = means3D.size(0)
    present = torch.full((P,), False, dtype=torch.bool, device=dev)
    if P != 0:
        m, v, p = _dev_f32(means3D, "means3D", dev), _dev_f32(viewmatrix, "viewmatrix", dev), _dev_f32(projmatrix, "projmatrix", dev)
        with torch.cuda.device(dev):
            rc = _capi.lib().bsr_mark_visible(P, m.data_ptr(), v.data_ptr(), p.data_ptr(), present.data_ptr(),
                                              _stream_handle(dev))
        _capi.check(rc, "mark_visible")
    return present


def _rasterize_gaussians_filter_native(means3D, scales, rotations, scale_modifier, cov3D_precomp, viewmatrix,
                                       projmatrix, tan_fovx, tan_fovy, image_height, image_width, prefiltered, debug):
    _check_means3D(means3D)
    if not means3D.is_cuda:
        raise RuntimeError("means3D must be a GPU tensor; bloomscene_amd has no CPU path")
    dev = means3D.device
    P = means3D.size(0)
    radii = torch.empty((P,), dtype=torch.int32, device=dev)
    if P != 0:
        m = _dev_f32(means3D, "means3D", dev)
        s, r = _dev_f32(scales, "scales", dev), _dev_f32(rotations, "rotations", dev)
        c = _dev_f32(cov3D_precomp, "cov3D_precomp", dev)
        v, p = _dev_f32(viewmatrix, "viewmatrix", dev), _dev_f32(projmatrix, "projmatrix", dev)
        with torch.cuda.device(dev):
            rc = _capi.lib().bsr_visible_filter(
                P, 0, int(image_width), int(image_height), m.data_ptr(), _ptr(s), float(scale_modifier), _ptr(r),
                _ptr(c), v.data_ptr(), p.data_ptr(), float(tan_fovx), float(tan_fovy), int(bool(prefiltered)),
                radii.data_ptr(), int(bool(debug)), _stream_handle(dev))
        _capi.check(rc, "rasterize_gaussians_filter")
    return radii


def _rasterize_gaussians_filter_indices_native(means3D, scales, rotations, scale_modifier, cov3D_precomp, viewmatrix,
                                               projmatrix, tan_fovx, tan_fovy, image_height, image_width, prefiltered,
                                               debug):
    _check_means3D(means3D)
    if not means3D.is_cuda:
        raise RuntimeError("means3D must be a GPU tensor; bloomscene_amd has no CPU path")
    dev = means3D.device
    P = means3D.size(0)
    radii = torch.empty((P,), dtype=torch.int32, device=dev)
    idx = torch.empty((P,), dtype=torch.int32, device=dev)
    n = C.c_int(0)
    if P != 0:
        lib = _capi.lib()
        m = _dev_f32(means3D, "means3D", dev)
        s, r = _dev_f32(scales, "scales", dev), _dev_f32(rotations, "rotations", dev)
        c = _dev_f32(cov3D_precomp, "cov3D_precomp", dev)
        v, p = _dev_f32(viewmatrix, "viewmatrix", dev), _dev_f32(projmatrix, "projmatrix", dev)
        scratch = torch.empty(lib.bsr_visible_scratch_bytes(P), dtype=torch.uint8, device=dev)
        with torch.cuda.device(dev):
            rc = lib.bsr_visible_filter_indices(
                P, 0, int(image_width), int(image_height), m.data_ptr(), _ptr(s), float(scale_modifier), _ptr(r),
                _ptr(c), v.data_ptr(), p.data_ptr(), float(tan_fovx), float(tan_fovy), int(bool(prefiltered)),
                radii.data_ptr(), idx.data_ptr(), scratch.data_ptr(), C.byref(n), int(bool(debug)), _stream_handle(dev))
        _capi.check(rc, "rasterize_gaussians_filter_indices")
    return radii, idx[:n.value].long()


def _rasterize_gaussians_filter_views_native(means3D, scales, rotations, scale_modifier, cov3D_precomp, viewmatrices,
                                             projmatrices, tan_fovx, tan_fovy, image_height, image_width, debug):
    _check_means3D(means3D)
    if not means3D.is_cuda:
        raise RuntimeError("means3D must be a GPU tensor; bloomscene_amd has no CPU path")
    dev = means3D.device
    P = means3D.size(0)
    if viewmatrices.dim() != 3 or tuple(viewmatrices.shape[1:]) != (4, 4) or viewmatrices.shape != projmatrices.shape:
        raise RuntimeError("viewmatrices and projmatrices must both have dimensions (num_views, 4, 4)")
    V = viewmatrices.size(0)
    radii = torch.empty((V, P), dtype=torch.int32, device=dev)
    if P != 0 and V != 0:
        m = _dev_f32(means3D, "means3D", dev)
        s, r = _dev_f32(scales, "scales", dev), _dev_f32(rotations, "rotations", dev)
        c = _dev_f32(cov3D_precomp, "cov3D_precomp", dev)
        v, p = _dev_f32(viewmatrices, "viewmatrices", dev), _dev_f32(projmatrices, "projmatrices", dev)
        with torch.cuda.device(dev):
            rc = _capi.lib().bsr_visible_filter_views(
                P, V, int(image_width), int(image_height), m.data_ptr(), _ptr(s), float(scale_modifier), _ptr(r),
                _ptr(c), v.data_ptr(), p.data_ptr(), float(tan_fovx), float(tan_fovy), radii.data_ptr(),
                int(bool(debug)), _stream_handle(dev))
        _capi.check(rc, "rasterize_gaussians_filter_views")
    return radii


def _rasterize_gaussians_filter_groups_native(means3D, scales, rotations, scale_modifier, cov3D_precomp, viewmatrices,
                                              projmatrices, tan_fovx, tan_fovy, image_height, image_width,
                                              group_of_view, n_groups, debug, return_counts=False):
    _check_means3D(means3D)
    if not means3D.is_cuda:
        raise RuntimeError("means3D must be a GPU tensor; bloomscene_amd has no CPU path")
    dev = means3D.device
    P = means3D.size(0)
    if viewmatrices.dim() != 3 or tuple(viewmatrices.shape[1:]) != (4, 4) or viewmatrices.shape != projmatrices.shape:
        raise RuntimeError("viewmatrices and projmatrices must both have dimensions (num_views, 4, 4)")
    V = viewmatrices.size(0)
    if group_of_view.numel() != V:
        raise RuntimeError("group_of_view must hold one group id per view")
    mask = torch.empty((int(n_groups), P), dtype=torch.bool, device=dev)
    counts = (torch.empty if P != 0 else torch.zeros)((int(n_groups),), dtype=torch.int32, device=dev) if return_counts else None
    if P != 0 and n_groups != 0:
        m = _dev_f32(means3D, "means3D", dev)
        s, r = _dev_f32(scales, "scales", dev), _dev_f32(rotations, "rotations", dev)
        c = _dev_f32(cov3D_precomp, "cov3D_precomp", dev)
        v, p = _dev_f32(viewmatrices, "viewmatrices", dev), _dev_f32(projmatrices, "projmatrices", dev)
        gv = group_of_view.to(device=dev, dtype=torch.int32).contiguous()
        lib = _capi.lib()
        scratch = torch.empty(lib.bsr_visible_groups_scratch_bytes(P, int(n_groups)), dtype=torch.uint8,
                              device=dev) if return_counts else None
        with torch.cuda.device(dev):
            rc = lib.bsr_visible_filter_groups(
                P, V, int(n_groups), int(image_width), int(image_height), m.data_ptr(), _ptr(s), float(scale_modifier),
                _ptr(r), _ptr(c), _ptr(v), _ptr(p), float(tan_fovx), float(tan_fovy), gv.data_ptr() if V else None,
                mask.data_ptr(), counts.data_ptr() if return_counts else None, _ptr(scratch), int(bool(debug)),
                _stream_handle(dev))
        _capi.check(rc, "rasterize_gaussians_filter_groups")
    return (mask, counts) if return_counts else mask


def _gather_rows_native(tensors, idx, idx_stride=1, rows=None, packed=True, debug=False):
    import ctypes as C
    if not 1 <= len(tensors) <= 8:
        raise RuntimeError("gather_rows takes 1..8 tensors")
    dev = tensors[0].device
    if dev.type != "cuda":
        raise RuntimeError("gather_rows needs GPU tensors; bloomscene_amd has no CPU path")
    if idx.dtype != torch.int64 or idx.device != dev or not idx.is_contiguous():
        raise RuntimeError("idx must be a contiguous int64 tensor on the tensors' device")
    idx_stride = int(idx_stride)
    R = int(rows) if rows is not None else (idx.numel() + idx_stride - 1) // idx_stride
    if R < 0 or idx_stride < 1 or (R > 0 and (R - 1) * idx_stride + 1 > idx.numel()):
        raise RuntimeError("idx holds fewer than rows elements at this stride")
    widths = [int(torch.Size(t.shape[1:]).numel()) for t in tensors]
    if any(t.shape[0] != tensors[0].shape[0] for t in tensors):
        raise RuntimeError("gather_rows: the tensors must have the same number of rows")
    srcs = [_dev_f32(t.detach(), "gather_rows source", dev) for t in tensors] if R else []
    if R and any(t is None for t in srcs):
        raise RuntimeError("gather_rows: rows requested from an empty tensor")
    if packed:
        out = torch.empty((R, sum(widths)), dtype=torch.float32, device=dev)
    else:
        out = [torch.empty((R,) + tuple(t.shape[1:]), dtype=torch.float32, device=dev) for t in tensors]
    if R:
        n = len(srcs)
        table = (C.c_void_p * n)(*[t.data_ptr() for t in srcs])
        wtab = (C.c_int * n)(*widths)
        with torch.cuda.device(dev):
            if packed:
                rc = _capi.lib().bsr_pack_rows(R, int(tensors[0].shape[0]), n, table, wtab, idx.data_ptr(), idx_stride,
                                               out.data_ptr(), int(bool(debug)), _stream_handle(dev))
            else:
                rc = _capi.lib().bsr_gather_rows(R, int(tensors[0].shape[0]), n, table, wtab, idx.data_ptr(), idx_stride,
                                                 (C.c_void_p * n)(*[t.data_ptr() for t in out]), int(bool(debug)),
                                                 _stream_handle(dev))
        _capi.check(rc, "gather_rows")
    return out


def _pack_rows_native(tensors, idx, idx_stride=1, rows=None, debug=False):
    return _gather_rows_native(tensors, idx, idx_stride, rows, True, debug)


def read_counts(image_buffer, image_height, image_width):
    kept, R = C.c_int(0), C.c_int(0)
    dev = image_buffer.device
    with torch.cuda.device(dev):
        rc = _capi.lib().bsr_read_counts(image_buffer.data_ptr(), int(image_width), int(image_height), _stream_handle(dev),
                                         C.byref(kept), C.byref(R))
    _capi.check(rc, "bsr_read_counts")
    return kept.value, R.value


def check_deferred():
    _capi.check(_capi.lib().bsr_check_deferred(), "deferred check of the previous no-readback forward")


def rasterize_gaussians(means3D, means2D, sh, colors_precomp, opacities, scales, rotations, cov3Ds_precomp,
                        raster_settings, depth_gradient=False, return_final_T=False, flags=None, capacity=None):
    out = _RasterizeGaussians.apply(means3D, means2D, sh, colors_precomp, opacities, scales, rotations,
                                    cov3Ds_precomp, raster_settings, depth_gradient, return_final_T,
                                    resolve_flags() if flags is None else int(flags), capacity)
    return out if return_final_T else out[:3]


class _RasterizeGaussians(torch.autograd.Function):

    @staticmethod
    def forward(ctx, means3D, means2D, sh, colors_precomp, opacities, scales, rotations, cov3Ds_precomp,
                raster_settings, depth_gradient=False, return_final_T=False, flags=0, capacity=None):
        args = (
            raster_settings.bg, means3D, colors_precomp, opacities, scales, rotations,
            raster_settings.scale_modifier, cov3Ds_precomp, raster_settings.viewmatrix, raster_settings.projmatrix,
            raster_settings.tanfovx, raster_settings.tanfovy, raster_settings.image_height,
            raster_settings.image_width, sh, raster_settings.sh_degree, raster_settings.campos,
            raster_settings.prefiltered, raster_settings.debug,
        )
        if raster_settings.debug:
            cpu_args = cpu_deep_copy_tuple(args)
            try:
                num_rendered, color, depth, radii, geomBuffer, binningBuffer, imgBuffer = \
                    _rasterize_gaussians_native(*args, flags=flags, capacity=capacity)
            except Exception as ex:
                torch.save(cpu_args, "snapshot_fw.dump")
                print("\nAn error occured in forward. Please forward snapshot_fw.dump for debugging.")
                raise ex
        else:
            num_rendered, color, depth, radii, geomBuffer, binningBuffer, imgBuffer = \
                _rasterize_gaussians_native(*args, flags=flags, capacity=capacity)

        if return_final_T:
            n_pix = raster_settings.image_height * raster_settings.image_width
            if imgBuffer.numel() >= 4 * n_pix:
                off = int(_capi.lib().bsr_transmittance_offset(imgBuffer.data_ptr()))
                final_T = imgBuffer[off:off + 4 * n_pix].view(torch.float32).view(
                    1, raster_settings.image_height, raster_settings.image_width)
            else:
                final_T = torch.ones((1, raster_settings.image_height, raster_settings.image_width),
                                     dtype=torch.float32, device=color.device)
        if return_final_T:
            ctx.mark_non_differentiable(radii, final_T)
        else:
            ctx.mark_non_differentiable(radii)
        ctx.set_materialize_grads(False)
        ctx.raster_settings = raster_settings
        ctx.num_rendered = num_rendered
        ctx.depth_gradient = bool(depth_gradient)
        ctx.flags = int(flags)
        ctx.save_for_backward(colors_precomp, means3D, scales, rotations, cov3Ds_precomp, radii, sh, geomBuffer,
                              binningBuffer, imgBuffer)
        if ctx.depth_gradient:
            ctx.out_depth = depth.detach().clone()
        return color, radii, depth, (final_T if return_final_T else None)

    @staticmethod
    def backward(ctx, grad_out_color, grad_radii, grad_depth, _grad_final_T=None):
        num_rendered = ctx.num_rendered
        raster_settings = ctx.raster_settings
        colors_precomp, means3D, scales, rotations, cov3Ds_precomp, radii, sh, geomBuffer, binningBuffer, imgBuffer = \
            ctx.saved_tensors
        if grad_out_color is None:
            grad_out_color = torch.zeros((3, raster_settings.image_height, raster_settings.image_width),
                                         dtype=torch.float32, device=means3D.device)
        if grad_depth is None:
            grad_depth = torch.zeros((1, raster_settings.image_height, raster_settings.image_width),
                                     dtype=torch.float32, device=means3D.device)
        args = (raster_settings.bg, means3D, radii, colors_precomp, scales, rotations,
                raster_settings.scale_modifier, cov3Ds_precomp, raster_settings.viewmatrix,
                raster_settings.projmatrix, raster_settings.tanfovx, raster_settings.tanfovy, grad_out_color,
                grad_depth, sh, raster_settings.sh_degree, raster_settings.campos, geomBuffer, num_rendered,
                binningBuffer, imgBuffer, raster_settings.debug)
        if ctx.depth_gradient:
            args = args + (ctx.out_depth,)
        kw = dict(flags=ctx.flags)
        if raster_settings.debug:
            cpu_args = cpu_deep_copy_tuple(args)
            try:
                grad_means2D, grad_colors_precomp, grad_opacities, grad_means3D, grad_cov3Ds_precomp, grad_sh, \
                    grad_scales, grad_rotations = _rasterize_gaussians_backward_native(*args, **kw)
            except Exception as ex:
                torch.save(cpu_args, "snapshot_bw.dump")
                print("\nAn error occured in backward. Writing snapshot_bw.dump for debugging.\n")
                raise ex
        else:
            grad_means2D, grad_colors_precomp, grad_opacities, grad_means3D, grad_cov3Ds_precomp, grad_sh, \
                grad_scales, grad_rotations = _rasterize_gaussians_backward_native(*args, **kw)

        def _fit(g, inp):
            return g if (inp.numel() != 0 and g is not None) else None

        grads = (
            grad_means3D,
            grad_means2D,
            _fit(grad_sh, sh),
            _fit(grad_colors_precomp, colors_precomp),
            grad_opacities,
            _fit(grad_scales, scales),
            _fit(grad_rotations, rotations),
            _fit(grad_cov3Ds_precomp, cov3Ds_precomp),
            None,
            None,
            None,
            None,
            None,
        )
        return grads


class GaussianRasterizer(nn.Module):
    def __init__(self, raster_settings, depth_gradient=False, exact_exp=None, strict_gradients=None, capacity=None):
        super().__init__()
        self.capacity = None if capacity is None else int(capacity)
        self.raster_settings = raster_settings
        self.depth_gradient = bool(depth_gradient)
        self.exact_exp = exact_exp
        self.strict_gradients = strict_gradients

    def _flags(self):
        return resolve_flags(self.exact_exp, self.strict_gradients)

    def markVisible(self, positions):
        with torch.no_grad():
            raster_settings = self.raster_settings
            visible = _mark_visible_native(positions, raster_settings.viewmatrix, raster_settings.projmatrix)
        return visible

    def forward(self, means3D, means2D, opacities, shs=None, colors_precomp=None, scales=None, rotations=None,
                cov3D_precomp=None, return_alpha=False):
        raster_settings = self.raster_settings

        if (shs is None and colors_precomp is None) or (shs is not None and colors_precomp is not None):
            raise Exception('Please provide excatly one of either SHs or precomputed colors!')

        if ((scales is None or rotations is None) and cov3D_precomp is None) or \
                ((scales is not None or rotations is not None) and cov3D_precomp is not None):
            raise Exception('Please provide exactly one of either scale/rotation pair or precomputed 3D covariance!')

        if shs is None:
            shs = torch.Tensor([])
        if colors_precomp is None:
            colors_precomp = torch.Tensor([])
        if scales is None:
            scales = torch.Tensor([])
        if rotations is None:
            rotations = torch.Tensor([])
        if cov3D_precomp is None:
            cov3D_precomp = torch.Tensor([])

        if not return_alpha:
            return rasterize_gaussians(means3D, means2D, shs, colors_precomp, opacities, scales, rotations,
                                       cov3D_precomp, raster_settings, self.depth_gradient, flags=self._flags(),
                                       capacity=self.capacity)
        color, radii, depth, final_T = rasterize_gaussians(means3D, means2D, shs, colors_precomp, opacities, scales,
                                                           rotations, cov3D_precomp, raster_settings,
                                                           self.depth_gradient, return_final_T=True,
                                                           flags=self._flags(), capacity=self.capacity)
        return color, radii, depth, (1.0 - final_T).detach()

    def visible_filter_indices(self, means3D, scales=None, rotations=None, cov3D_precomp=None):
        rs = self.raster_settings
        e = torch.Tensor([])
        with torch.no_grad():
            return _rasterize_gaussians_filter_indices_native(
                means3D, e if scales is None else scales, e if rotations is None else rotations, rs.scale_modifier,
                e if cov3D_precomp is None else cov3D_precomp, rs.viewmatrix, rs.projmatrix, rs.tanfovx, rs.tanfovy,
                rs.image_height, rs.image_width, rs.prefiltered, rs.debug)

    def visible_filter(self, means3D, scales=None, rotations=None, cov3D_precomp=None):
        raster_settings = self.raster_settings
        if scales is None:
            scales = torch.Tensor([])
        if rotations is None:
            rotations = torch.Tensor([])
        if cov3D_precomp is None:
            cov3D_precomp = torch.Tensor([])
        with torch.no_grad():
            radii = _rasterize_gaussians_filter_native(
                means3D, scales, rotations, raster_settings.scale_modifier, cov3D_precomp,
                raster_settings.viewmatrix, raster_settings.projmatrix, raster_settings.tanfovx,
                raster_settings.tanfovy, raster_settings.image_height, raster_settings.image_width,
                raster_settings.prefiltered, raster_settings.debug)
        return radii
```

### include/bloomscene_rast.h

```cpp
#ifndef BLOOMSCENE_RAST_H_INCLUDED
#define BLOOMSCENE_RAST_H_INCLUDED

#include <stddef.h>
#include <stdint.h>

#ifdef __cplusplus
extern "C" {
#endif

#define BSR_VERSION 4

#define BSR_FLAG_EXACT_EXP  1u
#define BSR_FLAG_EXACT_GRAD 2u
#define BSR_FLAG_NO_READBACK 4u
#define BSR_FLAG_TEST_SORT_INT      0x100u
#define BSR_FLAG_TEST_SMALL_GRIDS   0x200u
#define BSR_FLAG_TEST_NO_HALF_MASKS 0x400u
#define BSR_FLAG_TEST_SORT_NETWORK  0x800u
#define BSR_FLAG_TEST_MASK          0xf00u

typedef char* (*bsr_alloc_fn)(void* user, size_t bytes);

int bsr_version(void);

const char* bsr_last_error(void);

int bsr_mark_visible(int P, const float* means3D, const float* viewmatrix, const float* projmatrix,
                     uint8_t* present, void* stream);

int bsr_forward(bsr_alloc_fn geometryBuffer, void* geometry_user,
                bsr_alloc_fn binningBuffer, void* binning_user,
                bsr_alloc_fn imageBuffer, void* image_user,
                int P, int D, int M,
                const float* background,
                int width, int height,
                const float* means3D,
                const float* shs,
                const float* colors_precomp,
                const float* opacities,
                const float* scales,
                float scale_modifier,
                const float* rotations,
                const float* cov3D_precomp,
                const float* viewmatrix,
                const float* projmatrix,
                const float* cam_pos,
                float tan_fovx, float tan_fovy,
                int prefiltered,
                float* out_color,
                float* out_depth,
                int* radii,
                int debug,
                void* stream,
                int* num_rendered);

int bsr_forward_ex(bsr_alloc_fn geometryBuffer, void* geometry_user,
                   bsr_alloc_fn binningBuffer, void* binning_user,
                   bsr_alloc_fn imageBuffer, void* image_user,
                   int P, int D, int M,
                   const float* background,
                   int width, int height,
                   const float* means3D,
                   const float* shs,
                   const float* colors_precomp,
                   const float* opacities,
                   const float* scales,
                   float scale_modifier,
                   const float* rotations,
                   const float* cov3D_precomp,
                   const float* viewmatrix,
                   const float* projmatrix,
                   const float* cam_pos,
                   float tan_fovx, float tan_fovy,
                   int prefiltered,
                   float* out_color,
                   float* out_depth,
                   int* radii,
                   int debug,
                   void* stream,
                   int* num_rendered,
                   unsigned flags);

int bsr_read_counts(const char* image_buffer, int width, int height, void* stream, int* kept, int* num_rendered);

int bsr_check_deferred(void);

int bsr_visible_filter(int P, int M,
                       int width, int height,
                       const float* means3D,
                       const float* scales,
                       float scale_modifier,
                       const float* rotations,
                       const float* cov3D_precomp,
                       const float* viewmatrix,
                       const float* projmatrix,
                       float tan_fovx, float tan_fovy,
                       int prefiltered,
                       int* radii,
                       int debug,
                       void* stream);

int bsr_forward_views(bsr_alloc_fn geometryBuffer, void* geometry_user,
                      bsr_alloc_fn binningBuffer, void* binning_user,
                      bsr_alloc_fn imageBuffer, void* image_user,
                      int P, int D, int M, int n_views,
                      const float* background,
                      int width, int height,
                      const float* means3D,
                      const float* shs,
                      const float* colors_precomp,
                      const float* opacities,
                      const float* scales,
                      float scale_modifier,
                      const float* rotations,
                      const float* cov3D_precomp,
                      const float* viewmatrices,
                      const float* projmatrices,
                      const float* cam_positions,
                      float tan_fovx, float tan_fovy,
                      int prefiltered,
                      float* out_color,
                      float* out_depth,
                      int* radii,
                      int debug,
                      void* stream,
                      int* num_rendered,
                      unsigned flags);

size_t bsr_visible_scratch_bytes(int P);
int bsr_visible_filter_indices(int P, int M,
                               int width, int height,
                               const float* means3D,
                               const float* scales,
                               float scale_modifier,
                               const float* rotations,
                               const float* cov3D_precomp,
                               const float* viewmatrix,
                               const float* projmatrix,
                               float tan_fovx, float tan_fovy,
                               int prefiltered,
                               int* radii,
                               int* visible_idx,
                               void* scratch,
                               int* num_visible,
                               int debug,
                               void* stream);

int bsr_visible_filter_views(int P, int n_views,
                             int width, int height,
                             const float* means3D,
                             const float* scales,
                             float scale_modifier,
                             const float* rotations,
                             const float* cov3D_precomp,
                             const float* viewmatrices,
                             const float* projmatrices,
                             float tan_fovx, float tan_fovy,
                             int* radii,
                             int debug,
                             void* stream);

size_t bsr_visible_groups_scratch_bytes(int P, int n_groups);
int bsr_visible_filter_groups(int P, int n_views, int n_groups,
                              int width, int height,
                              const float* means3D, const float* scales, float scale_modifier,
                              const float* rotations, const float* cov3D_precomp,
                              const float* viewmatrices, const float* projmatrices,
// ... 138 lines not shown
```

Before: 1113 Msplats/s.

## Cache SH direction Jacobian in forward and reuse it in SH backward

During forward preprocessing with SH degree 3 and a single view, the kernel now also computes the 3x3 Jacobian of RGB with respect to the view direction and stores it in a new 9*P float geometry buffer. The backward SH pass reads this Jacobian, so it no longer recomputes dL/ddir through the cooperative per-wave coefficient loop. It turns on automatically when gradients are required. In exchange it adds 36 bytes per Gaussian of write traffic in forward and read traffic in backward, plus more register pressure in the preprocess kernel.

After: 1124 Msplats/s, median of 6. Within noise of the previous version (+1.0%).

```diff
diff --git a/bloomscene_amd/_capi.py b/bloomscene_amd/_capi.py
--- a/bloomscene_amd/_capi.py
+++ b/bloomscene_amd/_capi.py
@@ -131,6 +131,8 @@
 HeadsPointers = C.c_void_p * 12
 ContextPointers = C.c_void_p * 4
 
+last_forward_flags = None
+
 _lib = None
 _allow_older_abi = False
 
diff --git a/bloomscene_amd/csrc/api.hip b/bloomscene_amd/csrc/api.hip
--- a/bloomscene_amd/csrc/api.hip
+++ b/bloomscene_amd/csrc/api.hip
@@ -10,7 +10,8 @@
 
 using namespace bsr;
 
-static constexpr unsigned BSR_KNOWN_FLAGS = BSR_FLAG_EXACT_EXP | BSR_FLAG_EXACT_GRAD | BSR_FLAG_NO_READBACK | BSR_FLAG_TEST_MASK;
+static constexpr unsigned BSR_KNOWN_FLAGS = BSR_FLAG_EXACT_EXP | BSR_FLAG_EXACT_GRAD | BSR_FLAG_NO_READBACK |
+                                           BSR_FLAG_KEEP_SH_JACOBIAN | BSR_FLAG_TEST_MASK;
 
 static bool is_capturing(hipStream_t s)
 {
@@ -174,6 +175,7 @@
 	const ImgState& img = c.img;
 
 	if (prefiltered) HIP_TRY(hipMemsetAsync(img.flags, 0, sizeof(int), s));
+	const bool keep_sh_jac = (flags & BSR_FLAG_KEEP_SH_JACOBIAN) && V == 1 && shs != nullptr && D == 3 && M == 16;
 
 	{
 		PreArgs a;
@@ -188,6 +190,7 @@
 		a.gx = gx; a.gy = gy; a.prefiltered = prefiltered; a.radii = radii; a.geom = geom;
 		a.flags = img.flags;
 		a.n_views = V;
+		a.keep_sh_jac = keep_sh_jac;
 		if (V > 1)
 			HIP_TRY(hipMemsetAsync(geom.hist1, 0, BSR_RADIX_BINS_ * hist1_columns((size_t)n_wg) * sizeof(uint32_t), s));
 		{
@@ -201,7 +204,8 @@
 	const bool capturing = no_readback && is_capturing(s);
 	{
 		StageTimer t("scan_wg", s);
-		launch_scans(n_wg, geom.wg_kept, geom.wg_area, img.flags, geom.hist1, capturing ? nullptr : sc->pinned_dev, s);
+		launch_scans(n_wg, geom.wg_kept, geom.wg_area, img.flags, geom.hist1, capturing ? nullptr : sc->pinned_dev,
+		             keep_sh_jac ? 1 : 0, s);
 	}
 	STAGE_CHECK("scan_wg", debug, s);
 
@@ -524,6 +528,7 @@
 	a.geom = geom;
 	a.slab = slab; a.depth_grad = out_depth != nullptr;
 	a.kept_ptr = img.flags + 2; a.capacity = R;
+	a.sh_jac_flag = img.flags + 7;
 	a.dL_dmean2D = dL_dmean2D; a.dL_dconic = dL_dconic; a.dL_dopacity = dL_dopacity; a.dL_dcolor = dL_dcolor;
 	a.dL_dmean3D = dL_dmean3D; a.dL_dcov3D = dL_dcov3D; a.dL_dsh = dL_dsh; a.dL_dscale = dL_dscale; a.dL_drot = dL_drot;
 	{
diff --git a/bloomscene_amd/csrc/binning.hip b/bloomscene_amd/csrc/binning.hip
--- a/bloomscene_amd/csrc/binning.hip
+++ b/bloomscene_amd/csrc/binning.hip
@@ -51,7 +51,8 @@
 };
 __global__ void __launch_bounds__(1024) k_scans(int n_wg, uint32_t* __restrict__ wg_kept,
                                                 uint32_t* __restrict__ wg_area, int* __restrict__ flags,
-                                                uint32_t* __restrict__ hist1, int* __restrict__ host_counts)
+                                                uint32_t* __restrict__ hist1, int* __restrict__ host_counts,
+                                                int sh_jac_kept)
 {
 	__shared__ uint32_t s_w[32];
 	if (blockIdx.x == BSR_RADIX_BINS) {
@@ -61,7 +62,8 @@
 			flags[2] = (int)kept;
 			flags[3] = (int)area;
 			flags[1] = flags[4] = flags[5] = 0;
-			flags[6] = flags[7] = 0;
+			flags[6] = 0;
+			flags[7] = sh_jac_kept;
 			flags[BSR_POOL_FWD] = flags[BSR_POOL_BWD] = 0;
 			if (host_counts != nullptr) {
 				host_counts[0] = flags[0];
@@ -524,10 +526,10 @@
 }
 
 void launch_scans(int n_wg, uint32_t* wg_kept, uint32_t* wg_area, int* flags, uint32_t* hist1, int* host_counts,
-                  hipStream_t s)
+                  int sh_jac_kept, hipStream_t s)
 {
 	hipLaunchKernelGGL(k_scans, dim3(BSR_RADIX_BINS + 1), dim3(1024), 0, s, n_wg, wg_kept, wg_area, flags, hist1,
-	                   host_counts);
+	                   host_counts, sh_jac_kept);
 }
 
 #ifndef BSR_BUCKET_MAX_PER_TILE
diff --git a/bloomscene_amd/csrc/common.h b/bloomscene_amd/csrc/common.h
--- a/bloomscene_amd/csrc/common.h
+++ b/bloomscene_amd/csrc/common.h
@@ -21,6 +21,7 @@
 	ushort4* rect;
 	uint8_t* clamped;
 	float* depth;
+	float* sh_jac;
 	static GeomState layout(Carver& c, size_t P);
 	static size_t bytes(size_t P);
 	static GeomState carve(char* p, size_t P);
@@ -117,6 +118,7 @@
 	int n_views;
 	GeomState geom;
 	int* flags;
+	int keep_sh_jac;
 };
 
 struct BwdArgs {
@@ -136,6 +138,7 @@
 	const float4* slab;
 	int depth_grad;
 	const int* kept_ptr;
+	const int* sh_jac_flag;
 	int capacity;
 	float* dL_dmean2D;
 	float* dL_dconic;
diff --git a/bloomscene_amd/csrc/launch.h b/bloomscene_amd/csrc/launch.h
--- a/bloomscene_amd/csrc/launch.h
+++ b/bloomscene_amd/csrc/launch.h
@@ -36,7 +36,7 @@
 void launch_pack_rows(int R, int P, int n_src, const float* const* src, const int* widths, const int64_t* idx,
                       int idx_stride, float* dst_packed, float* const* dst_each, hipStream_t s);
 void launch_scans(int n_wg, uint32_t* wg_kept, uint32_t* wg_area, int* flags, uint32_t* hist1, int* host_counts,
-                  hipStream_t s);
+                  int sh_jac_kept, hipStream_t s);
 BinPlan binning_plan(int P, int T, int capacity, long long kept_hint);
 void launch_binning(const BinPlan& plan, int P, int T, int gx, const int* n_ptr, int capacity, const GeomState& geom,
                     BinElem* elems_a, BinElem* elems_b, uint32_t* hist, int hist_blocks_max, uint2* tile_range,
diff --git a/bloomscene_amd/csrc/preprocess.hip b/bloomscene_amd/csrc/preprocess.hip
--- a/bloomscene_amd/csrc/preprocess.hip
+++ b/bloomscene_amd/csrc/preprocess.hip
@@ -195,7 +195,12 @@
 		                        (unsigned short)rmax[0], (unsigned short)(rmax[1] + ty_off));
 		float rgb[3];
 		uint8_t clamp_bits = 0;
-		if (COLOR == 1) {
+		if (COLOR == 3) {
+			float jac[9];
+			sh3_to_rgb_jac_stream(p, a.cam_pos, a.shs + (size_t)gi * 48, rgb, clamp_bits, jac);
+#pragma unroll
+			for (int k = 0; k < 9; k++) a.geom.sh_jac[(size_t)k * a.P + gid] = jac[k];
+		} else if (COLOR == 1) {
 			sh3_to_rgb_stream(p, a.cam_pos + 3 * view, a.shs + (size_t)gi * 48, rgb, clamp_bits);
 		} else if (COLOR == 0 && a.colors_precomp == nullptr) {
 			sh_to_rgb(a.D, a.M, p, a.cam_pos + 3 * view, a.shs + (size_t)gi * a.M * 3, rgb, clamp_bits);
@@ -500,6 +505,8 @@
 	const int blocks = (a.P + 255) / 256;
 	if (filter_only)
 		hipLaunchKernelGGL((k_preprocess<true, 0>), dim3(blocks), dim3(256), 0, s, a);
+	else if (a.colors_precomp == nullptr && a.D == 3 && a.M == 16 && a.keep_sh_jac && a.n_views <= 1)
+		hipLaunchKernelGGL((k_preprocess<false, 3>), dim3(blocks), dim3(256), 0, s, a);
 	else if (a.colors_precomp == nullptr && a.D == 3 && a.M == 16)
 		hipLaunchKernelGGL((k_preprocess<false, 1>), dim3(blocks, a.n_views > 1 ? a.n_views : 1), dim3(256), 0, s, a);
 	else if (a.colors_precomp != nullptr)
diff --git a/bloomscene_amd/csrc/preprocess_bwd.hip b/bloomscene_amd/csrc/preprocess_bwd.hip
--- a/bloomscene_amd/csrc/preprocess_bwd.hip
+++ b/bloomscene_amd/csrc/preprocess_bwd.hip
@@ -74,7 +74,8 @@
 
 template <int DEG, int ROW_F4>
 __device__ __forceinline__ void sh_bwd_coop_half(const BwdArgs& a, int idx, bool visible, const float3 m, const float* dcolor,
-                                                 float* dmean, ShTile<ROW_F4, 32>& tile, int lane, int g0, int n_valid)
+                                                 float* dmean, ShTile<ROW_F4, 32>& tile, int lane, int g0, int n_valid,
+                                                 const float* __restrict__ jac = nullptr)
 {
 	constexpr int NC = (DEG + 1) * (DEG + 1);
 	constexpr int N = NC * 3;
@@ -119,6 +120,18 @@
 	const uint64_t vis_mask = __ballot(visible);
 	if (vis_mask == 0ull) return;
 	float dL_ddir[3] = {0.f, 0.f, 0.f};
+	if (DEG == 3 && jac != nullptr) {
+		if (visible) {
+			const float* const j = jac + idx;
+			const size_t P = (size_t)a.P;
+			const float dx0 = j[0], dx1 = j[P], dx2 = j[2 * P];
+			const float dy0 = j[3 * P], dy1 = j[4 * P], dy2 = j[5 * P];
+			const float dz0 = j[6 * P], dz1 = j[7 * P], dz2 = j[8 * P];
+			dL_ddir[0] = (dx0 * dL_dRGB[0] + dx1 * dL_dRGB[1]) + dx2 * dL_dRGB[2];
+			dL_ddir[1] = (dy0 * dL_dRGB[0] + dy1 * dL_dRGB[1]) + dy2 * dL_dRGB[2];
+			dL_ddir[2] = (dz0 * dL_dRGB[0] + dz1 * dL_dRGB[1]) + dz2 * dL_dRGB[2];
+		}
+	} else {
 #pragma unroll
 	for (int h = 0; h < 2; h++) {
 		if (((vis_mask >> (32 * h)) & 0xffffffffull) == 0ull) continue;
@@ -141,6 +154,7 @@
 		__builtin_amdgcn_fence(__ATOMIC_RELEASE, "wavefront");
 		__builtin_amdgcn_wave_barrier();
 		__builtin_amdgcn_fence(__ATOMIC_ACQUIRE, "wavefront");
+	}
 	}
 	if (visible) {
 		const float sum2 = ox * ox + oy * oy + oz * oz;
@@ -396,7 +410,11 @@
 		else if (a.D == 1) sh_bwd_coop_half<1, RF>(a, idx, visible, m, &g[6], dmean, tile, lane, g0, n_valid);
 		else if (ROW_F4 < 12) {  }
 		else if (a.D == 2) sh_bwd_coop_half<2, RF12>(a, idx, visible, m, &g[6], dmean, *reinterpret_cast<ShTile<RF12, 32>*>(&tile), lane, g0, n_valid);
-		else sh_bwd_coop_half<3, RF12>(a, idx, visible, m, &g[6], dmean, *reinterpret_cast<ShTile<RF12, 32>*>(&tile), lane, g0, n_valid);
+		else {
+			const bool has_jac = ROW_F4 == 12 && !overflow && __builtin_amdgcn_readfirstlane(*a.sh_jac_flag) != 0;
+			sh_bwd_coop_half<3, RF12>(a, idx, visible, m, &g[6], dmean, *reinterpret_cast<ShTile<RF12, 32>*>(&tile), lane, g0, n_valid,
+			                          has_jac ? a.geom.sh_jac : nullptr);
+		}
 	}
 	if (!in_range) return;
 
diff --git a/bloomscene_amd/csrc/scratch.h b/bloomscene_amd/csrc/scratch.h
--- a/bloomscene_amd/csrc/scratch.h
+++ b/bloomscene_amd/csrc/scratch.h
@@ -31,6 +31,7 @@
 	g.rect = c.take<ushort4>(P);
 	g.clamped = c.take<uint8_t>(P);
 	g.depth = c.take<float>(P);
+	g.sh_jac = c.take<float>(9 * P);
 	return g;
 }
 inline size_t GeomState::bytes(size_t P) { Carver c{nullptr}; layout(c, P); return c.off + 256; }
diff --git a/bloomscene_amd/csrc/sh.h b/bloomscene_amd/csrc/sh.h
--- a/bloomscene_amd/csrc/sh.h
+++ b/bloomscene_amd/csrc/sh.h
@@ -111,6 +111,122 @@
 			if (k == 0) r[ch] = b * v[j];
 			else if (k == 1 || k == 3) r[ch] = r[ch] - b * v[j];
 			else r[ch] = r[ch] + b * v[j];
+		}
+	}
+#pragma unroll
+	for (int ch = 0; ch < 3; ch++) res[ch] = r[ch] + 0.5f;
+}
+
+template <int AXIS>
+__device__ __forceinline__ float sh3_jac_term(int k, float c, float x, float y, float z, float xx, float yy, float zz,
+                                              float xy, float yz, float xz, bool& has)
+{
+	has = true;
+	if (AXIS == 0) {
+		switch (k) {
+		case 3: return -SH_C1 * c;
+		case 4: return SH_C2[0] * y * c;
+		case 6: return SH_C2[2] * 2.f * -x * c;
+		case 7: return SH_C2[3] * z * c;
+		case 8: return SH_C2[4] * 2.f * x * c;
+		case 9: return SH_C3[0] * c * 3.f * 2.f * xy;
+		case 10: return SH_C3[1] * c * yz;
+		case 11: return SH_C3[2] * c * -2.f * xy;
+		case 12: return SH_C3[3] * c * -3.f * 2.f * xz;
+		case 13: return SH_C3[4] * c * (-3.f * xx + 4.f * zz - yy);
+		case 14: return SH_C3[5] * c * 2.f * xz;
+		case 15: return SH_C3[6] * c * 3.f * (xx - yy);
+		default: break;
+		}
+	} else if (AXIS == 1) {
+		switch (k) {
+		case 1: return -SH_C1 * c;
+		case 4: return SH_C2[0] * x * c;
+		case 5: return SH_C2[1] * z * c;
+		case 6: return SH_C2[2] * 2.f * -y * c;
+		case 8: return SH_C2[4] * 2.f * -y * c;
+		case 9: return SH_C3[0] * c * 3.f * (xx - yy);
+		case 10: return SH_C3[1] * c * xz;
+		case 11: return SH_C3[2] * c * (-3.f * yy + 4.f * zz - xx);
+		case 12: return SH_C3[3] * c * -3.f * 2.f * yz;
+		case 13: return SH_C3[4] * c * -2.f * xy;
+		case 14: return SH_C3[5] * c * -2.f * yz;
+		case 15: return SH_C3[6] * c * -3.f * 2.f * xy;
+		default: break;
+		}
+	} else {
+		switch (k) {
+		case 2: return SH_C1 * c;
+		case 5: return SH_C2[1] * y * c;
+		case 6: return SH_C2[2] * 2.f * 2.f * z * c;
+		case 7: return SH_C2[3] * x * c;
+		case 10: return SH_C3[1] * c * xy;
+		case 11: return SH_C3[2] * c * 4.f * 2.f * yz;
+		case 12: return SH_C3[3] * c * 3.f * (2.f * zz - xx - yy);
+		case 13: return SH_C3[4] * c * 4.f * 2.f * xz;
+		case 14: return SH_C3[5] * c * (xx - yy);
+		default: break;
+		}
+	}
+	has = false;
+	return 0.f;
+}
+
+__device__ __forceinline__ void sh_eval3_jac_stream(const float* __restrict__ sh, float x, float y, float z, float* res,
+                                                    float* jac)
+{
+	const float xx = x * x, yy = y * y, zz = z * z;
+	const float xy = x * y, yz = y * z, xz = x * z;
+	const float4* s4 = reinterpret_cast<const float4*>(sh);
+	float r[3] = {0.f, 0.f, 0.f};
+	float part[9] = {0.f, 0.f, 0.f, 0.f, 0.f, 0.f, 0.f, 0.f, 0.f};
+#pragma unroll
+	for (int i = 0; i < 9; i++) jac[i] = 0.f;
+#ifndef BSR_SH_JAC_GROUP
+#define BSR_SH_JAC_GROUP 6
+#endif
+	constexpr int GS = BSR_SH_JAC_GROUP;
+	static_assert(12 % GS == 0, "twelve 16-byte loads");
+#pragma unroll
+	for (int g = 0; g < 12 / GS; g++) {
+		if (g > 0)
+			asm volatile("" : "+v"(s4), "+v"(r[0]), "+v"(r[1]), "+v"(r[2]), "+v"(part[0]), "+v"(part[1]), "+v"(part[2]),
+			             "+v"(part[3]), "+v"(part[4]), "+v"(part[5]));
+		float v[4 * GS];
+#pragma unroll
+		for (int i = 0; i < GS; i++) {
+			const float4 q = s4[GS * g + i];
+			v[4 * i + 0] = q.x; v[4 * i + 1] = q.y; v[4 * i + 2] = q.z; v[4 * i + 3] = q.w;
+		}
+#pragma unroll
+		for (int j = 0; j < 4 * GS; j++) {
+			const int p = 4 * GS * g + j, k = p / 3, ch = p % 3;
+			const float b = sh3_basis(k, x, y, z, xx, yy, zz, xy, yz, xz);
+			if (k == 0) r[ch] = b * v[j];
+			else if (k == 1 || k == 3) r[ch] = r[ch] - b * v[j];
+			else r[ch] = r[ch] + b * v[j];
+			bool has;
+			const float tx = sh3_jac_term<0>(k, v[j], x, y, z, xx, yy, zz, xy, yz, xz, has);
+			if (has) {
+				if (k == 3) jac[0 + ch] = tx;
+				else if (k == 4 || k == 9) part[0 + ch] = tx;
+				else part[0 + ch] = part[0 + ch] + tx;
+				if (k == 8 || k == 15) jac[0 + ch] += part[0 + ch];
+			}
+			const float ty = sh3_jac_term<1>(k, v[j], x, y, z, xx, yy, zz, xy, yz, xz, has);
+			if (has) {
+				if (k == 1) jac[3 + ch] = ty;
+				else if (k == 4 || k == 9) part[3 + ch] = ty;
+				else part[3 + ch] = part[3 + ch] + ty;
+				if (k == 8 || k == 15) jac[3 + ch] += part[3 + ch];
+			}
+			const float tz = sh3_jac_term<2>(k, v[j], x, y, z, xx, yy, zz, xy, yz, xz, has);
+			if (has) {
+				if (k == 2) jac[6 + ch] = tz;
+				else if (k == 5 || k == 10) part[6 + ch] = tz;
+				else part[6 + ch] = part[6 + ch] + tz;
+				if (k == 7 || k == 14) jac[6 + ch] += part[6 + ch];
+			}
 		}
 	}
 #pragma unroll
@@ -157,6 +273,23 @@
 	dx = dx / len; dy = dy / len; dz = dz / len;
 	float raw[3];
 	sh_eval3_stream(sh, dx, dy, dz, raw);
+	clamp_bits = 0;
+#pragma unroll
+	for (int ch = 0; ch < 3; ch++) {
+		if (raw[ch] < 0) clamp_bits |= (uint8_t)(1u << ch);
+		rgb[ch] = fmaxf(raw[ch], 0.0f);
+	}
+}
+
+__device__ __forceinline__ void sh3_to_rgb_jac_stream(const float3 pos, const float* __restrict__ campos,
+                                                      const float* __restrict__ sh, float* rgb, uint8_t& clamp_bits,
+                                                      float* jac)
+{
+	float dx = pos.x - campos[0], dy = pos.y - campos[1], dz = pos.z - campos[2];
+	const float len = sqrtf((dx * dx + dy * dy) + dz * dz);
+	dx = dx / len; dy = dy / len; dz = dz / len;
+	float raw[3];
+	sh_eval3_jac_stream(sh, dx, dy, dz, raw, jac);
 	clamp_bits = 0;
 #pragma unroll
 	for (int ch = 0; ch < 3; ch++) {
diff --git a/bloomscene_amd/rasterizer.py b/bloomscene_amd/rasterizer.py
--- a/bloomscene_amd/rasterizer.py
+++ b/bloomscene_amd/rasterizer.py
@@ -10,6 +10,7 @@
 from .numerics import FLAG_EXACT_EXP, FLAG_EXACT_GRAD, numerics, resolve_flags
 
 FLAG_NO_READBACK = 4
+FLAG_KEEP_SH_JACOBIAN = 8
 
 
 def cpu_deep_copy_tuple(input_tuple):
@@ -70,8 +71,10 @@
 
 def _rasterize_gaussians_native(bg, means3D, colors, opacity, scales, rotations, scale_modifier, cov3D_precomp,
                                 viewmatrix, projmatrix, tan_fovx, tan_fovy, image_height, image_width, sh, degree,
-                                campos, prefiltered, debug, flags=None, capacity=None):
+                                campos, prefiltered, debug, flags=None, capacity=None, keep_sh_jacobian=False):
     flags = resolve_flags() if flags is None else int(flags)
+    if keep_sh_jacobian:
+        flags |= FLAG_KEEP_SH_JACOBIAN
     if capacity is not None:
         if int(capacity) <= 0:
             raise RuntimeError("capacity must be a positive number of tile instances")
@@ -93,6 +96,7 @@
              proj=_dev_f32(projmatrix, "projmatrix", dev), sh=_dev_f32(sh, "shs", dev),
              campos=_dev_f32(campos, "campos", dev))
     num_rendered = C.c_int(int(capacity) if capacity is not None else 0)
+    _capi.last_forward_flags = int(flags)
     with torch.cuda.device(dev):
         rc = _capi.lib().bsr_forward_ex(
             geom.callback, None, binning.callback, None, img.callback, None,
@@ -371,10 +375,15 @@
 
 
 def rasterize_gaussians(means3D, means2D, sh, colors_precomp, opacities, scales, rotations, cov3Ds_precomp,
-                        raster_settings, depth_gradient=False, return_final_T=False, flags=None, capacity=None):
+                        raster_settings, depth_gradient=False, return_final_T=False, flags=None, capacity=None,
+                        keep_sh_jacobian=None):
+    if keep_sh_jacobian is None:
+        keep_sh_jacobian = torch.is_grad_enabled() and any(
+            isinstance(t, torch.Tensor) and t.requires_grad
+            for t in (means3D, means2D, sh, colors_precomp, opacities, scales, rotations, cov3Ds_precomp))
     out = _RasterizeGaussians.apply(means3D, means2D, sh, colors_precomp, opacities, scales, rotations,
                                     cov3Ds_precomp, raster_settings, depth_gradient, return_final_T,
-                                    resolve_flags() if flags is None else int(flags), capacity)
+                                    resolve_flags() if flags is None else int(flags), capacity, bool(keep_sh_jacobian))
     return out if return_final_T else out[:3]
 
 
@@ -382,7 +391,8 @@
 
     @staticmethod
     def forward(ctx, means3D, means2D, sh, colors_precomp, opacities, scales, rotations, cov3Ds_precomp,
-                raster_settings, depth_gradient=False, return_final_T=False, flags=0, capacity=None):
+                raster_settings, depth_gradient=False, return_final_T=False, flags=0, capacity=None,
+                keep_sh_jacobian=False):
         args = (
             raster_settings.bg, means3D, colors_precomp, opacities, scales, rotations,
             raster_settings.scale_modifier, cov3Ds_precomp, raster_settings.viewmatrix, raster_settings.projmatrix,
@@ -394,14 +404,14 @@
             cpu_args = cpu_deep_copy_tuple(args)
             try:
                 num_rendered, color, depth, radii, geomBuffer, binningBuffer, imgBuffer = \
-                    _rasterize_gaussians_native(*args, flags=flags, capacity=capacity)
+                    _rasterize_gaussians_native(*args, flags=flags, capacity=capacity, keep_sh_jacobian=keep_sh_jacobian)
             except Exception as ex:
                 torch.save(cpu_args, "snapshot_fw.dump")
                 print("\nAn error occured in forward. Please forward snapshot_fw.dump for debugging.")
                 raise ex
         else:
             num_rendered, color, depth, radii, geomBuffer, binningBuffer, imgBuffer = \
-                _rasterize_gaussians_native(*args, flags=flags, capacity=capacity)
+                _rasterize_gaussians_native(*args, flags=flags, capacity=capacity, keep_sh_jacobian=keep_sh_jacobian)
 
         if return_final_T:
             n_pix = raster_settings.image_height * raster_settings.image_width
@@ -477,13 +487,16 @@
             None,
             None,
             None,
+            None,
         )
         return grads
 
 
 class GaussianRasterizer(nn.Module):
-    def __init__(self, raster_settings, depth_gradient=False, exact_exp=None, strict_gradients=None, capacity=None):
+    def __init__(self, raster_settings, depth_gradient=False, exact_exp=None, strict_gradients=None, capacity=None,
+                 keep_sh_jacobian=None):
         super().__init__()
+        self.keep_sh_jacobian = keep_sh_jacobian
         self.capacity = None if capacity is None else int(capacity)
         self.raster_settings = raster_settings
         self.depth_gradient = bool(depth_gradient)
@@ -524,11 +537,12 @@
         if not return_alpha:
             return rasterize_gaussians(means3D, means2D, shs, colors_precomp, opacities, scales, rotations,
                                        cov3D_precomp, raster_settings, self.depth_gradient, flags=self._flags(),
-                                       capacity=self.capacity)
+                                       capacity=self.capacity, keep_sh_jacobian=self.keep_sh_jacobian)
         color, radii, depth, final_T = rasterize_gaussians(means3D, means2D, shs, colors_precomp, opacities, scales,
                                                            rotations, cov3D_precomp, raster_settings,
                                                            self.depth_gradient, return_final_T=True,
-                                                           flags=self._flags(), capacity=self.capacity)
+                                                           flags=self._flags(), capacity=self.capacity,
+                                                           keep_sh_jacobian=self.keep_sh_jacobian)
         return color, radii, depth, (1.0 - final_T).detach()
 
     def visible_filter_indices(self, means3D, scales=None, rotations=None, cov3D_precomp=None):
diff --git a/include/bloomscene_rast.h b/include/bloomscene_rast.h
--- a/include/bloomscene_rast.h
+++ b/include/bloomscene_rast.h
@@ -13,6 +13,7 @@
 #define BSR_FLAG_EXACT_EXP  1u
 #define BSR_FLAG_EXACT_GRAD 2u
 #define BSR_FLAG_NO_READBACK 4u
+#define BSR_FLAG_KEEP_SH_JACOBIAN 8u
 #define BSR_FLAG_TEST_SORT_INT      0x100u
 #define BSR_FLAG_TEST_SMALL_GRIDS   0x200u
 #define BSR_FLAG_TEST_NO_HALF_MASKS 0x400u
```
